# minh86/ModelCrowdNav

Hardware: NVIDIA B200
Metric: env-steps/s (ORCA step + SARL lookahead) (higher is better)
Workload: dtype f16

## Files before the change

modelcrowdnav_b200/csrc/capi.cu:

```cuda
#include "cn_common.cuh"

#include <math.h>
#include <stdarg.h>
#include <stdlib.h>
#include <string.h>

#include <vector>

std::atomic<int64_t> g_cn_launches{0};
static thread_local char g_err[512] = "";

void cn_set_error(const char *fmt, ...)
{
    va_list ap;
    va_start(ap, fmt);
    vsnprintf(g_err, sizeof(g_err), fmt, ap);
    va_end(ap);
}

int cn_launch_transpose_out(int E, int H, int C, const double *src, double *dst, cudaStream_t s);
int cn_launch_set_actions(cn_env *env, const double *aos_dev, cudaStream_t s);
int cn_launch_set_human_v(cn_env *env, const double *aos_dev, cudaStream_t s);
int cn_launch_pack_keep(cn_env *env, cudaStream_t s);

struct TraceRec { const char *name; cudaStream_t stream; cudaEvent_t ev; };
static std::vector<TraceRec> g_trace;
static bool g_trace_on = false;

void cn_trace_mark(const char *name, cudaStream_t s)
{
    if (!g_trace_on || g_trace.size() >= 4096) return;
    cudaEvent_t ev;
    if (cudaEventCreate(&ev) != cudaSuccess) return;
    cudaEventRecord(ev, s);
    g_trace.push_back({name, s, ev});
}

static SarlDims dims_of(const cn_sarl_cfg *c, int om_dim)
{
    SarlDims d;
    memset(&d, 0, sizeof(d));
    d.in = c->input_dim; d.self_dim = c->self_state_dim;
    for (int i = 0; i < 2; ++i) { d.m1[i] = c->mlp1_dims[i]; d.m2[i] = c->mlp2_dims[i]; }
    for (int i = 0; i < 3; ++i) d.at[i] = c->attn_dims[i];
    for (int i = 0; i < 4; ++i) d.m3[i] = c->mlp3_dims[i];
    d.net = c->network; d.lstm_h = c->network == CN_NET_LSTM_RL ? c->lstm_hidden : 0;
    for (int i = 0; i < 4; ++i) d.lm1[i] = c->network == CN_NET_LSTM_RL ? c->lstm_mlp1_dims[i] : 0;
    d.lstm_in = d.lm1[0] > 0 ? d.lm1[3] : d.in;
    d.om_dim = om_dim; d.cell_num = c->cell_num; d.om_ch = c->om_channel_size; d.cell_size = c->cell_size;
    d.no_gs = c->network == CN_NET_SARL && c->without_global_state ? 1 : 0;
    return d;
}

std::vector<LayerSpec> cn_layers(const SarlDims &d, SarlWeightsDev &w)
{
    std::vector<LayerSpec> L;
    int in = d.in;
    auto chain = [&](int n, const int *outs, LinearDev *dst) {
        for (int i = 0; i < n; ++i) { L.push_back({in, outs[i], &dst[i], nullptr}); in = outs[i]; }
    };
    if (d.net == CN_NET_CADRL) {
        chain(4, d.m3, w.m3);
    } else if (d.net == CN_NET_LSTM_RL) {
        if (d.lm1[0] > 0) chain(4, d.lm1, w.lm1);
        in = d.self_dim + d.lstm_h;
        chain(4, d.m3, w.m3);
        L.push_back({d.lstm_in, 4 * d.lstm_h, &w.lih, &w.lhh});
    } else {
        chain(2, d.m1, w.m1);
        chain(2, d.m2, w.m2);
        in = d.no_gs ? d.m1[1] : 2 * d.m1[1];
        chain(3, d.at, w.at);
        in = d.m2[1] + d.self_dim;
        chain(4, d.m3, w.m3);
    }
    return L;
}

extern "C" {

int cn_debug_trace(int on)
{
    for (auto &r : g_trace) cudaEventDestroy(r.ev);
    g_trace.clear();
    g_trace_on = on != 0;
    return CN_OK;
}

int cn_debug_trace_dump(char *buf, int64_t cap)
{
    if (!buf || cap < 1) { cn_set_error("null buffer"); return CN_EINVAL; }
    CN_CUDA_CHECK(cudaDeviceSynchronize());
    int64_t off = 0;
    buf[0] = 0;
    for (size_t i = 0; i < g_trace.size(); ++i) {
        float ms = 0.0f;
        cudaEventElapsedTime(&ms, g_trace[0].ev, g_trace[i].ev);
        const int n = snprintf(buf + off, (size_t)(cap - off), "%.4f %p %s\n", ms, (void *)g_trace[i].stream, g_trace[i].name);
        if (n < 0 || off + n >= cap) break;
        off += n;
    }
    return CN_OK;
}

const char *cn_last_error(void) { return g_err; }
int cn_version(void) { return 100; }
int64_t cn_launch_count(void) { return g_cn_launches.load(); }

int cn_device_count(void)
{
    int n = 0;
    if (cudaGetDeviceCount(&n) != cudaSuccess) { cudaGetLastError(); return 0; }
    return n;
}

void cn_env_cfg_default(cn_env_cfg *c)
{
    memset(c, 0, sizeof(*c));
    c->num_envs = 1; c->human_num = 5;
    c->time_limit = 25; c->time_step = 0.25;
    c->success_reward = 1; c->collision_penalty = -0.25; c->discomfort_dist = 0.2; c->discomfort_penalty_factor = 0.5;
    c->neighbor_dist = 10; c->max_neighbors = 10; c->time_horizon = 5; c->human_safety_space = 0;
    c->robot_visible = 0;
    c->sim_rule = CN_CIRCLE_CROSSING; c->circle_radius = 4; c->square_width = 10;
    c->human_radius = 0.3; c->human_v_pref = 1; c->robot_radius = 0.3; c->robot_v_pref = 1;
    c->seed = 0; c->env_id_offset = 0; c->auto_reset = 0; c->gamma = 0.9;
    c->randomize_attributes = 0;
    c->robot_kinematics = CN_KIN_HOLONOMIC;
}

void cn_sarl_cfg_default(cn_sarl_cfg *c)
{
    memset(c, 0, sizeof(*c));
    c->input_dim = 13; c->self_state_dim = 6;
    c->mlp1_dims[0] = 150; c->mlp1_dims[1] = 100;
    c->mlp2_dims[0] = 100; c->mlp2_dims[1] = 50;
    c->attn_dims[0] = 100; c->attn_dims[1] = 100; c->attn_dims[2] = 1;
    c->mlp3_dims[0] = 150; c->mlp3_dims[1] = 100; c->mlp3_dims[2] = 100; c->mlp3_dims[3] = 1;
    c->speed_samples = 5; c->rotation_samples = 16;
    c->gamma = 0.9; c->v_pref = 1.0; c->precision = CN_PREC_F32;
    c->kinematics = CN_KIN_HOLONOMIC;
    c->network = CN_NET_SARL; c->lstm_hidden = 50;
    c->with_om = 0; c->cell_num = 4; c->cell_size = 1.0; c->om_channel_size = 3;
}

static int use_device(int device)
{
    int n = 0;
    cudaError_t e = cudaGetDeviceCount(&n);
    if (e != cudaSuccess || n == 0) {
        cudaGetLastError();
        cn_set_error("no CUDA device available (%s); libcrowdnav_b200 has no CPU fallback",
                     e != cudaSuccess ? cudaGetErrorString(e) : "device count 0");
        return CN_ECUDA;
    }
    if (device < 0 || device >= n) { cn_set_error("device %d out of range (0..%d)", device, n - 1); return CN_EINVAL; }
    CN_CUDA_CHECK(cudaSetDevice(device));
    cudaDeviceProp prop;
    CN_CUDA_CHECK(cudaGetDeviceProperties(&prop, device));
    if (prop.major != 10) {
        cn_set_error("device %d is sm_%d%d; this library is built for sm_100a only", device, prop.major, prop.minor);
        return CN_ECUDA;
    }
    return CN_OK;
}


int cn_env_create(const cn_env_cfg *cfg, int device, cn_env **out)
{
    if (!cfg || !out) { cn_set_error("null argument"); return CN_EINVAL; }
    if (cfg->num_envs < 1 || cfg->human_num < 1 || cfg->human_num > CN_MAX_HUMANS) {
        cn_set_error("num_envs >= 1 and 1 <= human_num <= %d required", CN_MAX_HUMANS);
        return CN_EINVAL;
    }
    if (cfg->max_neighbors < 0 || cfg->max_neighbors > CN_MAX_NEIGHBORS) {
        cn_set_error("max_neighbors must be in [0, %d]", CN_MAX_NEIGHBORS);
        return CN_EINVAL;
    }
    if (!(cfg->time_step > 0)) { cn_set_error("time_step must be positive"); return CN_EINVAL; }
    int rc = use_device(device);
    if (rc) return rc;

    cn_env *env = new cn_env();
    memset(env, 0, sizeof(*env));
    env->device = device;
    EnvParams &p = env->p;
    p.d.E = cfg->num_envs; p.d.H = cfg->human_num; p.d.A1 = cfg->human_num + 1;
    p.time_limit = cfg->time_limit; p.time_step = cfg->time_step;
    p.success_reward = cfg->success_reward; p.collision_penalty = cfg->collision_penalty;
    p.discomfort_dist = cfg->discomfort_dist; p.discomfort_penalty_factor = cfg->discomfort_penalty_factor;
    p.neighbor_dist = (float)cfg->neighbor_dist; p.time_horizon = (float)cfg->time_horizon;
    p.time_step_f = (float)cfg->time_step; p.max_neighbors = cfg->max_neighbors;
    p.human_safety_space = cfg->human_safety_space; p.robot_visible = cfg->robot_visible;
    p.sim_rule = cfg->sim_rule; p.circle_radius = cfg->circle_radius; p.square_width = cfg->square_width;
    p.human_radius = cfg->human_radius; p.human_v_pref = cfg->human_v_pref;
    p.robot_radius = cfg->robot_radius; p.robot_v_pref = cfg->robot_v_pref;
    p.seed = cfg->seed; p.env_id_offset = cfg->env_id_offset; p.auto_reset = cfg->auto_reset;
    p.gamma = cfg->gamma;
    p.randomize_attributes = cfg->randomize_attributes;
    p.kinematics = cfg->robot_kinematics;

    const size_t E = p.d.E, H = p.d.H, A1 = p.d.A1;
#define CN_ALLOC(ptr, bytes)                                                     \
    do {                                                                         \
        cudaError_t _e = cudaMalloc((void **)&(ptr), (bytes));                   \
        if (_e != cudaSuccess) {                                                 \
            cn_set_error("cudaMalloc(%zu) failed: %s", (size_t)(bytes), cudaGetErrorString(_e)); \
            cn_env_destroy(env);                                                 \
            return CN_ENOMEM;                                                    \
        }                                                                        \
        cudaMemset((ptr), 0, (bytes));                                           \
    } while (0)
    CN_ALLOC(env->state, sizeof(double) * F_COUNT * A1 * E);
    CN_ALLOC(env->time, sizeof(double) * E);
    CN_ALLOC(env->human_v, sizeof(double) * 2 * H * E);
    CN_ALLOC(env->action_xy, sizeof(double) * 2 * E);
    CN_ALLOC(env->action_idx, sizeof(int32_t) * E);
    CN_ALLOC(env->reward, sizeof(double) * E);
    CN_ALLOC(env->done, E);
    CN_ALLOC(env->info, E);
    CN_ALLOC(env->dmin, sizeof(double) * E);
    CN_ALLOC(env->next_obs, sizeof(double) * 5 * H * E);
    CN_ALLOC(env->frozen, E);
    CN_ALLOC(env->stage, sizeof(double) * F_COUNT * A1 * E);
    CN_ALLOC(env->step_ctr, sizeof(uint32_t) * E);
    CN_ALLOC(env->theta, sizeof(double) * E);
    const size_t acc_bytes = E * (6 * 8 + 6 * 8 + 4 + 4);
    CN_ALLOC(env->accum_block, acc_bytes);
#undef CN_ALLOC
    char *b = (char *)env->accum_block;
    EnvAccum &a = env->acc;
    a.episodes = (int64_t *)b; b += 8 * E;
    a.success = (int64_t *)b; b += 8 * E;
    a.collision = (int64_t *)b; b += 8 * E;
    a.timeout = (int64_t *)b; b += 8 * E;
    a.steps = (int64_t *)b; b += 8 * E;
    a.too_close = (int64_t *)b; b += 8 * E;
    a.sum_min_dist = (double *)b; b += 8 * E;
    a.sum_success_time = (double *)b; b += 8 * E;
    a.sum_collision_time = (double *)b; b += 8 * E;
    a.sum_timeout_time = (double *)b; b += 8 * E;
    a.sum_return = (double *)b; b += 8 * E;
    a.ep_return = (double *)b; b += 8 * E;
    a.ep_steps = (int32_t *)b; b += 4 * E;
    a.episode_ctr = (uint32_t *)b; b += 4 * E;
    *out = env;
    return CN_OK;
}

int cn_env_destroy(cn_env *env)
{
    if (!env) return CN_OK;
    cudaSetDevice(env->device);
    void *ptrs[] = {env->state, env->time, env->human_v, env->action_xy, env->action_idx, env->reward, env->done,
                    env->info, env->dmin, env->next_obs, env->frozen, env->stage, env->step_ctr, env->accum_block, env->theta};
    for (void *q : ptrs) if (q) cudaFree(q);
    if (env->io_block) cudaFree(env->io_block);
    if (env->side_stream) cudaStreamDestroy(env->side_stream);
    if (env->ev_fork) cudaEventDestroy(env->ev_fork);
    if (env->ev_join) cudaEventDestroy(env->ev_join);
    if (env->tail_stream) cudaStreamDestroy(env->tail_stream);
    if (env->ev_rows) cudaEventDestroy(env->ev_rows);
    if (env->ev_tail) cudaEventDestroy(env->ev_tail);
    if (env->active_dev) cudaFree(env->active_dev);
    if (env->active_host) cudaFreeHost(env->active_host);
    for (cudaEvent_t ev : env->ev_active) if (ev) cudaEventDestroy(ev);
    delete env;
    return CN_OK;
}

#define CN_ENV_ENTER(env)                                              \
    if (!(env)) { cn_set_error("null env handle"); return CN_EINVAL; } \
    CN_CUDA_CHECK(cudaSetDevice((env)->device));                       \
    cudaStream_t s = (cudaStream_t)stream

int cn_env_set_theta(cn_env *env, const double *theta_host, void *stream)
{
    CN_ENV_ENTER(env);
    if (!theta_host) { cn_set_error("theta_host is null"); return CN_EINVAL; }
    CN_CUDA_CHECK(cudaMemcpyAsync(env->theta, theta_host, sizeof(double) * env->p.d.E, cudaMemcpyHostToDevice, s));
    CN_CUDA_CHECK(cudaStreamSynchronize(s));
    return CN_OK;
}

int cn_env_get_theta(cn_env *env, double *theta_host, void *stream)
{
    CN_ENV_ENTER(env);
    if (!theta_host) { cn_set_error("theta_host is null"); return CN_EINVAL; }
    CN_CUDA_CHECK(cudaMemcpyAsync(theta_host, env->theta, sizeof(double) * env->p.d.E, cudaMemcpyDeviceToHost, s));
    CN_CUDA_CHECK(cudaStreamSynchronize(s));
    return CN_OK;
}

int cn_env_set_state(cn_env *env, const double *agents_host, const double *times_host, void *stream)
{
    CN_ENV_ENTER(env);
    if (!agents_host) { cn_set_error("agents_host is null"); return CN_EINVAL; }
    const size_t E = env->p.d.E, A1 = env->p.d.A1;
    CN_CUDA_CHECK(cudaMemcpyAsync(env->stage, agents_host, sizeof(double) * E * A1 * F_COUNT, cudaMemcpyHostToDevice, s));
    int rc = cn_launch_pack(env, 1, s);
    if (rc) return rc;
    if (times_host) CN_CUDA_CHECK(cudaMemcpyAsync(env->time, times_host, sizeof(double) * E, cudaMemcpyHostToDevice, s));
    else CN_CUDA_CHECK(cudaMemsetAsync(env->time, 0, sizeof(double) * E, s));
    return CN_OK;
}

int cn_env_get_state(cn_env *env, double *agents_host, double *times_host, void *stream)
{
    CN_ENV_ENTER(env);
    const size_t E = env->p.d.E, A1 = env->p.d.A1;
    if (agents_host) {
        int rc = cn_launch_pack(env, 0, s);
        if (rc) return rc;
        CN_CUDA_CHECK(cudaMemcpyAsync(agents_host, env->stage, sizeof(double) * E * A1 * F_COUNT, cudaMemcpyDeviceToHost, s));
    }
    if (times_host) CN_CUDA_CHECK(cudaMemcpyAsync(times_host, env->time, sizeof(double) * E, cudaMemcpyDeviceToHost, s));
    CN_CUDA_CHECK(cudaStreamSynchronize(s));
    return CN_OK;
}

int cn_env_reset(cn_env *env, void *stream)
{
    CN_ENV_ENTER(env);
    return cn_launch_reset(env, 0, s);
}

int cn_env_orca(cn_env *env, void *stream)
{
    CN_ENV_ENTER(env);
    return cn_launch_orca(env, s);
}

int cn_env_robot_orca(cn_env *env, double safety_space, void *stream)
{
    CN_ENV_ENTER(env);
    return cn_launch_robot_orca(env, safety_space, s);
}

int cn_env_step(cn_env *env, const double *action_xy_dev, int update, void *stream)
{
    CN_ENV_ENTER(env);
    if (!env->orca_valid) {
        cn_set_error("cn_env_step: call cn_env_orca for the current state first");
        return CN_EINVAL;
    }
    int rc = cn_launch_step(env, action_xy_dev, update, s);
    if (rc) return rc;
    if (update && env->p.auto_reset) rc = cn_launch_reset(env, 1, s);
    return rc;
}

int cn_env_get_views(cn_env *env, cn_env_views *out)
{
    if (!env || !out) { cn_set_error("null argument"); return CN_EINVAL; }
    out->reward = env->reward; out->done = env->done; out->info = env->info; out->dmin = env->dmin;
    out->human_v = env->human_v; out->next_obs = env->next_obs; out->state = env->state; out->time = env->time;
    out->action_idx = env->action_idx; out->action_xy = env->action_xy;
    return CN_OK;
}

int cn_env_read_outputs(cn_env *env, double *reward, uint8_t *done, uint8_t *info, double *dmin, void *stream)
{
    CN_ENV_ENTER(env);
    const size_t E = env->p.d.E;
    if (reward) CN_CUDA_CHECK(cudaMemcpyAsync(reward, env->reward, sizeof(double) * E, cudaMemcpyDeviceToHost, s));
    if (done) CN_CUDA_CHECK(cudaMemcpyAsync(done, env->done, E, cudaMemcpyDeviceToHost, s));
    if (info) CN_CUDA_CHECK(cudaMemcpyAsync(info, env->info, E, cudaMemcpyDeviceToHost, s));
    if (dmin) CN_CUDA_CHECK(cudaMemcpyAsync(dmin, env->dmin, sizeof(double) * E, cudaMemcpyDeviceToHost, s));
    CN_CUDA_CHECK(cudaStreamSynchronize(s));
    return CN_OK;
}

int cn_env_read_human_actions(cn_env *env, double *human_vxy_host, void *stream)
{
    CN_ENV_ENTER(env);
    if (!env->orca_valid) { cn_set_error("no cached ORCA result; call cn_env_orca"); return CN_EINVAL; }
    const size_t E = env->p.d.E, H = env->p.d.H;
    int rc = cn_launch_transpose_out((int)E, (int)H, 2, env->human_v, env->stage, s);
    if (rc) return rc;
    CN_CUDA_CHECK(cudaMemcpyAsync(human_vxy_host, env->stage, sizeof(double) * E * H * 2, cudaMemcpyDeviceToHost, s));
    CN_CUDA_CHECK(cudaStreamSynchronize(s));
    return CN_OK;
}

int cn_env_read_next_obs(cn_env *env, double *obs_host, void *stream)
{
    CN_ENV_ENTER(env);
    const size_t E = env->p.d.E, H = env->p.d.H;
    int rc = cn_launch_transpose_out((int)E, (int)H, 5, env->next_obs, env->stage, s);
    if (rc) return rc;
    CN_CUDA_CHECK(cudaMemcpyAsync(obs_host, env->stage, sizeof(double) * E * H * 5, cudaMemcpyDeviceToHost, s));
    CN_CUDA_CHECK(cudaStreamSynchronize(s));
    return CN_OK;
}

int cn_env_read_actions(cn_env *env, double *action_xy_host, int32_t *action_idx_host, void *stream)
{
    CN_ENV_ENTER(env);
    const size_t E = env->p.d.E;
    if (action_xy_host) {
        int rc = cn_launch_transpose_out((int)E, 1, 2, env->action_xy, env->stage, s);
        if (rc) return rc;
        CN_CUDA_CHECK(cudaMemcpyAsync(action_xy_host, env->stage, sizeof(double) * 2 * E, cudaMemcpyDeviceToHost, s));
    }
    if (action_idx_host)
        CN_CUDA_CHECK(cudaMemcpyAsync(action_idx_host, env->action_idx, sizeof(int32_t) * E, cudaMemcpyDeviceToHost, s));
    CN_CUDA_CHECK(cudaStreamSynchronize(s));
    return CN_OK;
}

int cn_env_set_actions(cn_env *env, const double *action_xy_host, void *stream)
{
    CN_ENV_ENTER(env);
    if (!action_xy_host) { cn_set_error("action_xy_host is null"); return CN_EINVAL; }
    const size_t E = env->p.d.E;
    CN_CUDA_CHECK(cudaMemcpyAsync(env->stage, action_xy_host, sizeof(double) * 2 * E, cudaMemcpyHostToDevice, s));
    return cn_launch_set_actions(env, env->stage, s);
}

int cn_env_set_human_actions(cn_env *env, const double *human_vxy_host, void *stream)
{
    CN_ENV_ENTER(env);
    if (!human_vxy_host) { cn_set_error("human_vxy_host is null"); return CN_EINVAL; }
    const size_t n = (size_t)env->p.d.E * env->p.d.H * 2;
    CN_CUDA_CHECK(cudaMemcpyAsync(env->stage, human_vxy_host, sizeof(double) * n, cudaMemcpyHostToDevice, s));
    return cn_launch_set_human_v(env, env->stage, s);
}

int cn_env_read_stats(cn_env *env, cn_stats *out, int reset, void *stream)
{
    CN_ENV_ENTER(env);
    if (!out) { cn_set_error("null stats"); return CN_EINVAL; }
    const size_t E = env->p.d.E;
    const size_t bytes = E * 8 * 11;
    std::vector<char> host(bytes);
    CN_CUDA_CHECK(cudaMemcpyAsync(host.data(), env->accum_block, bytes, cudaMemcpyDeviceToHost, s));
    CN_CUDA_CHECK(cudaStreamSynchronize(s));
    const int64_t *iv = (const int64_t *)host.data();
    const double *dv = (const double *)(host.data() + 6 * 8 * E);
    int64_t isum[6] = {0, 0, 0, 0, 0, 0};
    double dsum[5] = {0, 0, 0, 0, 0};
    for (int k = 0; k < 6; ++k) for (size_t e = 0; e < E; ++e) isum[k] += iv[k * E + e];
    for (int k = 0; k < 5; ++k) for (size_t e = 0; e < E; ++e) dsum[k] += dv[k * E + e];
    out->episodes = isum[0]; out->success = isum[1]; out->collision = isum[2]; out->timeout = isum[3];
    out->steps = isum[4]; out->too_close = isum[5];
    out->sum_min_dist = dsum[0]; out->sum_success_time = dsum[1]; out->sum_collision_time = dsum[2];
    out->sum_timeout_time = dsum[3]; out->sum_return = dsum[4];
    if (reset) CN_CUDA_CHECK(cudaMemsetAsync(env->accum_block, 0, bytes, s));
    return CN_OK;
}

int cn_env_copy_outputs(cn_env *env, double *reward_dev, uint8_t *done_dev, uint8_t *info_dev, void *stream)
{
    CN_ENV_ENTER(env);
    const size_t E = env->p.d.E;
    if (reward_dev) CN_CUDA_CHECK(cudaMemcpyAsync(reward_dev, env->reward, sizeof(double) * E, cudaMemcpyDeviceToDevice, s));
    if (done_dev) CN_CUDA_CHECK(cudaMemcpyAsync(done_dev, env->done, E, cudaMemcpyDeviceToDevice, s));
    if (info_dev) CN_CUDA_CHECK(cudaMemcpyAsync(info_dev, env->info, E, cudaMemcpyDeviceToDevice, s));
    return CN_OK;
}

int64_t cn_env_episode_table_bytes(const cn_env *env) { return env ? (int64_t)env->p.d.E * 8 * 11 : 0; }

int cn_env_read_episode_table(cn_env *env, void *table_host, uint8_t *frozen_host, void *stream)
{
    CN_ENV_ENTER(env);
    const size_t E = env->p.d.E;
    if (table_host) CN_CUDA_CHECK(cudaMemcpyAsync(table_host, env->accum_block, E * 8 * 11, cudaMemcpyDeviceToHost, s));
    if (frozen_host) CN_CUDA_CHECK(cudaMemcpyAsync(frozen_host, env->frozen, E, cudaMemcpyDeviceToHost, s));
    CN_CUDA_CHECK(cudaStreamSynchronize(s));
    return CN_OK;
}


static int pad4i(int x) { return (x + 3) & ~3; }

int64_t cn_policy_param_count(const cn_sarl_cfg *c)
{
    if (!c) return 0;
    SarlWeightsDev w;
    int64_t n = 0;
    for (const LayerSpec &l : cn_layers(dims_of(c, 0), w)) n += (int64_t)cn_layer_floats(l);
    return n;
}

static int build_action_table(const cn_sarl_cfg *c, double *out)
{
    const double E_ = 2.718281828459045;
    int n = 0;
    out[0] = 0; out[1] = 0; n = 1;
    if (c->kinematics != CN_KIN_HOLONOMIC) {
        const double PI = 3.141592653589793, start = -PI / 4, stop = PI / 4;
        const int div = c->rotation_samples - 1;
        const double step = div > 0 ? (stop - start) / div : 0.0;
        for (int r = 0; r < c->rotation_samples; ++r) {
            double rotation = start + r * step;
            if (div > 0 && r == c->rotation_samples - 1) rotation = stop;
            for (int s = 0; s < c->speed_samples; ++s) {
                out[2 * n] = (exp((double)(s + 1) / c->speed_samples) - 1) / (E_ - 1) * c->v_pref;
                out[2 * n + 1] = rotation;
                ++n;
            }
        }
        return n;
    }
    const double step = (2 * 3.141592653589793 - 0) / c->rotation_samples;
    for (int r = 0; r < c->rotation_samples; ++r) {
        const double rotation = r * step;
        for (int s = 0; s < c->speed_samples; ++s) {
            const double speed = (exp((double)(s + 1) / c->speed_samples) - 1) / (E_ - 1) * c->v_pref;
            out[2 * n] = speed * cos(rotation);
            out[2 * n + 1] = speed * sin(rotation);
            ++n;
        }
    }
    return n;
}

int cn_policy_create(const cn_sarl_cfg *cfg, int device, cn_policy **out)
{
    if (!cfg || !out) { cn_set_error("null argument"); return CN_EINVAL; }
    const int A = cfg->speed_samples * cfg->rotation_samples + 1;
    int om_dim = 0;
    if (cfg->with_om) {
        if (cfg->cell_num < 1 || cfg->cell_num > 8 || cfg->om_channel_size < 1 || cfg->om_channel_size > 3 || !(cfg->cell_size > 0)) {
            cn_set_error("with_om needs 1 <= cell_num <= 8, om_channel_size in {1, 2, 3} and cell_size > 0");
            return CN_EINVAL;
        }
        if (cfg->network == CN_NET_CADRL) { cn_set_error("CADRL has no occupancy maps (cadrl.py:60-62)"); return CN_EINVAL; }
        if (cfg->precision != CN_PREC_F32 && cfg->network != CN_NET_SARL) {
            cn_set_error("occupancy maps on the tensor-core path are built for SARL only; use CN_PREC_F32"); return CN_EUNSUPPORTED;
        }
        om_dim = cfg->cell_num * cfg->cell_num * cfg->om_channel_size;
    }
    if (cfg->input_dim != 13 + om_dim || cfg->self_state_dim < 1 || cfg->self_state_dim > 13) {
        cn_set_error("input_dim must be 13 + cell_num^2 * om_channel_size (13 without maps) and 1 <= self_state_dim <= 13");
        return CN_EUNSUPPORTED;
    }
    if (cfg->attn_dims[2] != 1 || cfg->mlp3_dims[3] != 1) { cn_set_error("attention and mlp3 must end in 1 unit"); return CN_EINVAL; }
    if (cfg->network != CN_NET_SARL && cfg->network != CN_NET_CADRL && cfg->network != CN_NET_LSTM_RL) {
        cn_set_error("unknown value network %d", cfg->network); return CN_EINVAL;
    }
    if (cfg->without_global_state && cfg->network != CN_NET_SARL) {
        cn_set_error("without_global_state is a [sarl] option; CADRL and LSTM-RL have no global state"); return CN_EINVAL;
    }
    if (cfg->network == CN_NET_LSTM_RL) {
        if (cfg->lstm_hidden < 1 || cfg->lstm_hidden > 64) { cn_set_error("1 <= lstm_hidden <= 64 required"); return CN_EINVAL; }
        if (cfg->lstm_mlp1_dims[0] > 0)
            for (int i = 0; i < 4; ++i)
                if (cfg->lstm_mlp1_dims[i] < 1 || cfg->lstm_mlp1_dims[i] > 256) { cn_set_error("layer widths must be in [1, 256]"); return CN_EINVAL; }
    }
    if (A < 1 || A > CN_MAX_ACTIONS) { cn_set_error("1 <= speed_samples*rotation_samples+1 <= %d required", CN_MAX_ACTIONS); return CN_EINVAL; }
    const int dims[] = {cfg->mlp1_dims[0], cfg->mlp1_dims[1], cfg->mlp2_dims[0], cfg->mlp2_dims[1], cfg->attn_dims[0],
                        cfg->attn_dims[1], cfg->mlp3_dims[0], cfg->mlp3_dims[1], cfg->mlp3_dims[2]};
    for (int v : dims) if (v < 1 || v > 256) { cn_set_error("layer widths must be in [1, 256]"); return CN_EINVAL; }
    if (cfg->precision != CN_PREC_F32 && cfg->precision != CN_PREC_F16_TC) { cn_set_error("unknown precision"); return CN_EINVAL; }
    int rc = use_device(device);
    if (rc) return rc;
    if ((rc = cn_f32_configure_device())) return rc;

    cn_policy *p = new cn_policy();
    memset(p, 0, sizeof(*p));
    p->device = device; p->cfg = *cfg;
    p->d = dims_of(cfg, om_dim);
    SarlDims &d = p->d;
    d.A = build_action_table(cfg, p->action_host);
    p->n_params = cn_policy_param_count(cfg);

    size_t tsize = 0;
    for (const LayerSpec &l : cn_layers(d, p->w))
        tsize += (size_t)(l.in + 1) * pad4i(l.out) + (l.dst_hh ? (size_t)(l.out / 4 + 1) * pad4i(l.out) : 0);
    cudaError_t e1 = cudaMalloc((void **)&p->action_dev, sizeof(double) * 2 * d.A);
    cudaError_t e2 = cudaMalloc((void **)&p->w_raw, sizeof(float) * p->n_params);
    cudaError_t e3 = cudaMalloc((void **)&p->w_t, sizeof(float) * tsize);
    cudaError_t e4 = cudaMalloc((void **)&p->bad_flag, 2 * sizeof(int32_t));
    if (e1 != cudaSuccess || e2 != cudaSuccess || e3 != cudaSuccess || e4 != cudaSuccess) {
        cn_set_error("cudaMalloc failed in cn_policy_create");
        cn_policy_destroy(p);
        return CN_ENOMEM;
    }
    cudaMemset(p->bad_flag, 0, 2 * sizeof(int32_t));
    CN_CUDA_CHECK(cudaMemcpy(p->action_dev, p->action_host, sizeof(double) * 2 * d.A, cudaMemcpyHostToDevice));
    if (cfg->precision == CN_PREC_F16_TC) {
        rc = cn_tc_init(p);
        if (rc) { cn_policy_destroy(p); return rc; }
    }
    *out = p;
    return CN_OK;
}

int cn_policy_destroy(cn_policy *p)
{
    if (!p) return CN_OK;
    cudaSetDevice(p->device);
    if (p->tc) cn_tc_destroy(p);
    void *ptrs[] = {p->action_dev, p->w_raw, p->w_t, p->bad_flag, p->values};
    for (void *q : ptrs) if (q) cudaFree(q);
    delete p;
    return CN_OK;
}

int cn_policy_load_weights(cn_policy *p, const float *flat, int64_t n, void *stream)
{
    if (!p || !flat) { cn_set_error("null argument"); return CN_EINVAL; }
    if (n != p->n_params) { cn_set_error("expected %lld parameters, got %lld", (long long)p->n_params, (long long)n); return CN_EINVAL; }
    CN_CUDA_CHECK(cudaSetDevice(p->device));
    cudaStream_t s = (cudaStream_t)stream;
    std::vector<float> t;
    auto put = [&](int in, int out, const float *w, const float *b, LinearDev *dst) {
        const int ld = pad4i(out);
        const size_t off = t.size();
        t.resize(off + (size_t)in * ld + ld, 0.0f);
        for (int o = 0; o < out; ++o)
            for (int k = 0; k < in; ++k) t[off + (size_t)k * ld + o] = w[(size_t)o * in + k];
        for (int o = 0; o < out; ++o) t[off + (size_t)in * ld + o] = b[o];
        dst->wt = p->w_t + off; dst->b = p->w_t + off + (size_t)in * ld;
        dst->in = in; dst->out = out; dst->ld = ld;
    };
    const float *src = flat;
    for (const LayerSpec &l : cn_layers(p->d, p->w)) {
        const float *w = src, *b = src + (size_t)l.in * l.out;
        if (l.dst_hh) {
            const int h = l.out / 4;
            const float *w_hh = b;
            b = w_hh + (size_t)l.out * h;
            put(l.in, l.out, w, b, l.dst);
            put(h, l.out, w_hh, b + l.out, l.dst_hh);
        } else {
            put(l.in, l.out, w, b, l.dst);
        }
        src += cn_layer_floats(l);
    }
    CN_CUDA_CHECK(cudaMemcpyAsync(p->w_t, t.data(), sizeof(float) * t.size(), cudaMemcpyHostToDevice, s));
    CN_CUDA_CHECK(cudaMemcpyAsync(p->w_raw, flat, sizeof(float) * n, cudaMemcpyHostToDevice, s));
    CN_CUDA_CHECK(cudaStreamSynchronize(s));
    if (p->cfg.precision == CN_PREC_F16_TC) {
        int rc = cn_tc_load_weights(p, flat, s);
        if (rc) return rc;
    }
    p->weights_loaded = 1;
    return CN_OK;
}

int cn_policy_action_table(cn_policy *p, double *out_xy_host, int32_t *n_actions)
{
    if (!p) { cn_set_error("null policy"); return CN_EINVAL; }
    if (out_xy_host) memcpy(out_xy_host, p->action_host, sizeof(double) * 2 * p->d.A);
    if (n_actions) *n_actions = p->d.A;
    return CN_OK;
}

static int check_pair(cn_policy *p, cn_env *env)
{
    if (!p || !env) { cn_set_error("null handle"); return CN_EINVAL; }
    if (p->device != env->device) { cn_set_error("policy and env live on different devices"); return CN_EINVAL; }
    if (!p->weights_loaded) { cn_set_error("cn_policy_load_weights has not been called"); return CN_EINVAL; }
    if (p->cfg.kinematics != env->p.kinematics) {
        cn_set_error("policy kinematics (%d) and env robot_kinematics (%d) differ", p->cfg.kinematics, env->p.kinematics);
        return CN_EINVAL;
    }
    return CN_OK;
}

static int lookahead(cn_policy *p, cn_env *env, int query_env, double epsilon, cudaStream_t s, cudaStream_t tail = nullptr)
{
    if (p->cfg.precision == CN_PREC_F16_TC) return cn_lookahead_tc(p, env, query_env, epsilon, s, tail);
    return cn_lookahead_f32(p, env, query_env, epsilon, s);
}

static int sync_and_check_values(cn_policy *p, cudaStream_t s)
{
    int32_t bad = 0;
    CN_CUDA_CHECK(cudaMemcpyAsync(&bad, p->bad_flag, sizeof(int32_t), cudaMemcpyDeviceToHost, s));
    CN_CUDA_CHECK(cudaStreamSynchronize(s));
    if (bad) { cn_set_error("Value network is not well trained. "); return CN_EVALUE; }
    return CN_OK;
}

int cn_policy_lookahead(cn_policy *p, cn_env *env, int query_env, double epsilon, void *stream)
{
    int rc = check_pair(p, env);
    if (rc) return rc;
    CN_CUDA_CHECK(cudaSetDevice(p->device));
    cudaStream_t s = (cudaStream_t)stream;
    if (query_env && !env->orca_valid) {
        cn_set_error("query_env lookahead needs cn_env_orca for the current state");
        return CN_EINVAL;
    }
    return lookahead(p, env, query_env, epsilon, s);
}

int cn_policy_read(cn_policy *p, cn_env *env, int32_t *best_idx, double *values, void *stream)
{
    int rc = check_pair(p, env);
    if (rc) return rc;
    CN_CUDA_CHECK(cudaSetDevice(p->device));
    cudaStream_t s = (cudaStream_t)stream;
    const size_t E = env->p.d.E;
    if (best_idx) CN_CUDA_CHECK(cudaMemcpyAsync(best_idx, env->action_idx, sizeof(int32_t) * E, cudaMemcpyDeviceToHost, s));
    if (values) {
        if (!p->values) { cn_set_error("no lookahead has been run"); return CN_EINVAL; }
        CN_CUDA_CHECK(cudaMemcpyAsync(values, p->values, sizeof(double) * E * p->d.A, cudaMemcpyDeviceToHost, s));
    }
    return sync_and_check_values(p, s);
}

int cn_policy_bad_count(cn_policy *p, int64_t *count, int reset, void *stream)
{
    if (!p || !count) { cn_set_error("null argument"); return CN_EINVAL; }
    CN_CUDA_CHECK(cudaSetDevice(p->device));
    cudaStream_t s = (cudaStream_t)stream;
    int32_t n = 0;
    CN_CUDA_CHECK(cudaMemcpyAsync(&n, p->bad_flag + 1, sizeof(int32_t), cudaMemcpyDeviceToHost, s));
    if (reset) CN_CUDA_CHECK(cudaMemsetAsync(p->bad_flag + 1, 0, sizeof(int32_t), s));
    CN_CUDA_CHECK(cudaStreamSynchronize(s));
    *count = n;
    return CN_OK;
}

int cn_policy_transform(cn_policy *p, cn_env *env, float *out_dev, void *stream)
{
    if (!p || !env || !out_dev) { cn_set_error("null argument"); return CN_EINVAL; }
    CN_CUDA_CHECK(cudaSetDevice(p->device));
    return cn_transform_f32(p, env, out_dev, 0, (cudaStream_t)stream);
}

int cn_policy_last_state(cn_policy *p, cn_env *env, float *out_dev, void *stream)
{
    if (!p || !env || !out_dev) { cn_set_error("null argument"); return CN_EINVAL; }
    CN_CUDA_CHECK(cudaSetDevice(p->device));
    return cn_transform_f32(p, env, out_dev, p->cfg.network == CN_NET_LSTM_RL ? 1 : 0, (cudaStream_t)stream);
}

int cn_policy_forward(cn_policy *p, const float *x_dev, int32_t batch, int32_t human_num, float *out_dev, void *stream)
{
    if (!p || !x_dev || !out_dev) { cn_set_error("null argument"); return CN_EINVAL; }
    if (!p->weights_loaded) { cn_set_error("cn_policy_load_weights has not been called"); return CN_EINVAL; }
    CN_CUDA_CHECK(cudaSetDevice(p->device));
    return cn_forward_f32(p, x_dev, batch, human_num, out_dev, (cudaStream_t)stream);
}


static int rollout_step_impl(cn_policy *p, cn_env *env, int query_env, double epsilon, cudaStream_t s, cudaStream_t tail,
                             cudaStream_t *cur);

int cn_rollout_step(cn_policy *p, cn_env *env, int query_env, double epsilon, void *stream)
{
    int rc = check_pair(p, env);
    if (rc) return rc;
    CN_CUDA_CHECK(cudaSetDevice(p->device));
    cudaStream_t cur;
    return rollout_step_impl(p, env, query_env, epsilon, (cudaStream_t)stream, nullptr, &cur);
}

static int ensure_tail_stream(cn_env *env)
{
    if (env->tail_stream) return CN_OK;
    int lo = 0, hi = 0;
    CN_CUDA_CHECK(cudaDeviceGetStreamPriorityRange(&lo, &hi));
    CN_CUDA_CHECK(cudaStreamCreateWithPriority(&env->tail_stream, cudaStreamNonBlocking, hi));
    CN_CUDA_CHECK(cudaEventCreateWithFlags(&env->ev_rows, cudaEventDisableTiming));
    CN_CUDA_CHECK(cudaEventCreateWithFlags(&env->ev_tail, cudaEventDisableTiming));
    return CN_OK;
}

int cn_rollout_step_sharded(cn_policy *p, cn_env *env, int query_env, double epsilon, void *stream)
{
    int rc = check_pair(p, env);
    if (rc) return rc;
    CN_CUDA_CHECK(cudaSetDevice(p->device));
    if ((rc = ensure_tail_stream(env))) return rc;
    cudaStream_t s0 = (cudaStream_t)stream, cur = s0;
    if ((rc = rollout_step_impl(p, env, query_env, epsilon, s0, env->tail_stream, &cur))) return rc;
    if (cur != s0) {
        CN_CUDA_CHECK(cudaEventRecord(env->ev_tail, cur));
        CN_CUDA_CHECK(cudaStreamWaitEvent(s0, env->ev_tail, 0));
    }
    return CN_OK;
}

static int rollout_step_impl(cn_policy *p, cn_env *env, int query_env, double epsilon, cudaStream_t s, cudaStream_t tail,
                             cudaStream_t *cur)
{
    int rc = CN_OK;
    if (p->cfg.precision != CN_PREC_F16_TC) tail = nullptr;
    const bool fork = !query_env;
    cn_trace_mark("orca", s);
    if (fork) {
        if (!env->side_stream) {
            CN_CUDA_CHECK(cudaStreamCreateWithFlags(&env->side_stream, cudaStreamNonBlocking));
            CN_CUDA_CHECK(cudaEventCreateWithFlags(&env->ev_fork, cudaEventDisableTiming));
            CN_CUDA_CHECK(cudaEventCreateWithFlags(&env->ev_join, cudaEventDisableTiming));
        }
        CN_CUDA_CHECK(cudaEventRecord(env->ev_fork, s));
        CN_CUDA_CHECK(cudaStreamWaitEvent(env->side_stream, env->ev_fork, 0));
        if ((rc = cn_launch_orca(env, env->side_stream))) return rc;
        CN_CUDA_CHECK(cudaEventRecord(env->ev_join, env->side_stream));
    } else if ((rc = cn_launch_orca(env, s))) return rc;
    if ((rc = lookahead(p, env, query_env, epsilon, s, tail))) return rc;
    if (tail) s = tail;
    *cur = s;
    if (fork) CN_CUDA_CHECK(cudaStreamWaitEvent(s, env->ev_join, 0));
    cn_trace_mark("step", s);
    if ((rc = cn_launch_step(env, nullptr, 1, s, env->p.auto_reset ? 1 : 0))) return rc;
    cn_trace_mark("step_done", s);
    return rc;
}


static __global__ void count_active_kernel(int E, const uint8_t *__restrict__ frozen, int32_t *__restrict__ out)
{
    __shared__ int total;
    if (threadIdx.x == 0) total = 0;
    __syncthreads();
    int n = 0;
    for (int e = threadIdx.x; e < E; e += blockDim.x) n += frozen[e] ? 0 : 1;
    for (int o = 16; o > 0; o >>= 1) n += __shfl_xor_sync(0xffffffffu, n, o);
    if ((threadIdx.x & 31) == 0 && n) atomicAdd(&total, n);
    __syncthreads();
    if (threadIdx.x == 0) *out = total;
}

int cn_rollout_episodes(cn_policy *p, cn_env *env, cn_world *world, int robot_mode, double safety_space, int query_env,
                        double epsilon, int32_t max_steps, int32_t check_every, const cn_rollout_record *rec,
                        int32_t *steps_run, void *stream)
{
    if (!env || !steps_run) { cn_set_error("null argument"); return CN_EINVAL; }
    if (robot_mode < CN_ROBOT_POLICY || robot_mode > CN_ROBOT_KEEP) { cn_set_error("robot_mode %d", robot_mode); return CN_EINVAL; }
    if (max_steps < 0 || check_every < 1) { cn_set_error("max_steps >= 0 and check_every >= 1"); return CN_EINVAL; }
    if (env->p.auto_reset) {
        cn_set_error("cn_rollout_episodes runs ONE episode per env: create the env with auto_reset = 0");
        return CN_EINVAL;
    }
    int rc;
    if (robot_mode == CN_ROBOT_POLICY) {
        if ((rc = check_pair(p, env))) return rc;
    }
    cn_policy *tp = rec ? rec->transform_policy : nullptr;
    if (rec && (!tp || !rec->states_dev || !rec->reward_dev || !rec->done_dev)) {
        cn_set_error("cn_rollout_record needs transform_policy, states_dev, reward_dev and done_dev");
        return CN_EINVAL;
    }
    if (tp && tp->device != env->device) { cn_set_error("transform policy and env live on different devices"); return CN_EINVAL; }
    CN_CUDA_CHECK(cudaSetDevice(env->device));
    cudaStream_t s = (cudaStream_t)stream;
    if (!env->active_dev) {
        CN_CUDA_CHECK(cudaMalloc(&env->active_dev, 2 * sizeof(int32_t)));
        CN_CUDA_CHECK(cudaMallocHost(&env->active_host, 2 * sizeof(int32_t)));
        for (cudaEvent_t &ev : env->ev_active) CN_CUDA_CHECK(cudaEventCreateWithFlags(&ev, cudaEventDisableTiming));
    }
    const size_t E = env->p.d.E;
    const size_t state_floats = tp ? E * (size_t)env->p.d.H * (size_t)tp->cfg.input_dim : 0;
    int slot = 0, pending = -1;
    *steps_run = 0;
    for (int step = 0; step < max_steps; ++step) {
        if (tp) {
            const int sorted = rec->last_state && tp->cfg.network == CN_NET_LSTM_RL;
            if ((rc = cn_transform_f32(tp, env, rec->states_dev + (size_t)step * state_floats, sorted, s))) return rc;
        }
        if (robot_mode == CN_ROBOT_POLICY && !world) {
            cudaStream_t cur;
            if ((rc = rollout_step_impl(p, env, query_env, epsilon, s, nullptr, &cur))) return rc;
        } else {
            if (world) rc = cn_world_predict(world, env, s);
            else rc = cn_launch_orca(env, s);
            if (rc) return rc;
            if (robot_mode == CN_ROBOT_POLICY)
                rc = lookahead(p, env, query_env, epsilon, s);
            else if (robot_mode == CN_ROBOT_ORCA) rc = cn_launch_robot_orca(env, safety_space, s);
            if (rc) return rc;
            if ((rc = cn_launch_step(env, nullptr, 1, s, 0))) return rc;
        }
        if (rec) {
            CN_CUDA_CHECK(cudaMemcpyAsync(rec->reward_dev + (size_t)step * E, env->reward, sizeof(double) * E, cudaMemcpyDeviceToDevice, s));
            CN_CUDA_CHECK(cudaMemcpyAsync(rec->done_dev + (size_t)step * E, env->done, E, cudaMemcpyDeviceToDevice, s));
        }
        *steps_run = step + 1;
        if ((step + 1) % check_every == 0) {
            if (pending >= 0) {
                CN_CUDA_CHECK(cudaEventSynchronize(env->ev_active[pending]));
                if (env->active_host[pending] == 0) break;
            }
            count_active_kernel<<<1, 256, 0, s>>>((int)E, env->frozen, env->active_dev + slot);
            CN_CUDA_CHECK(cudaGetLastError());
            g_cn_launches.fetch_add(1);
            CN_CUDA_CHECK(cudaMemcpyAsync(env->active_host + slot, env->active_dev + slot, sizeof(int32_t), cudaMemcpyDeviceToHost, s));
            CN_CUDA_CHECK(cudaEventRecord(env->ev_active[slot], s));
            pending = slot;
            slot ^= 1;
        }
    }
    return CN_OK;
}

int cn_rollout_step_host(cn_policy *p, cn_env *env, int query_env, double epsilon, const double *agents_in,
                         const double *times_in, double *agents_out, double *times_out, double *reward, uint8_t *done,
                         uint8_t *info, int32_t *action_idx, void *stream)
{
    int rc = check_pair(p, env);
    if (rc) return rc;
    CN_CUDA_CHECK(cudaSetDevice(p->device));
    cudaStream_t s = (cudaStream_t)stream;
    const size_t E = env->p.d.E, A1 = env->p.d.A1;
    if (agents_in) {
        CN_CUDA_CHECK(cudaMemcpyAsync(env->stage, agents_in, sizeof(double) * E * A1 * F_COUNT, cudaMemcpyHostToDevice, s));
        if ((rc = cn_launch_pack_keep(env, s))) return rc;
    }
    if (times_in) CN_CUDA_CHECK(cudaMemcpyAsync(env->time, times_in, sizeof(double) * E, cudaMemcpyHostToDevice, s));
    if ((rc = cn_rollout_step(p, env, query_env, epsilon, s))) return rc;
    if (agents_out) {
        if ((rc = cn_launch_pack(env, 0, s))) return rc;
        CN_CUDA_CHECK(cudaMemcpyAsync(agents_out, env->stage, sizeof(double) * E * A1 * F_COUNT, cudaMemcpyDeviceToHost, s));
    }
    if (times_out) CN_CUDA_CHECK(cudaMemcpyAsync(times_out, env->time, sizeof(double) * E, cudaMemcpyDeviceToHost, s));
    if (reward) CN_CUDA_CHECK(cudaMemcpyAsync(reward, env->reward, sizeof(double) * E, cudaMemcpyDeviceToHost, s));
    if (done) CN_CUDA_CHECK(cudaMemcpyAsync(done, env->done, E, cudaMemcpyDeviceToHost, s));
    if (info) CN_CUDA_CHECK(cudaMemcpyAsync(info, env->info, E, cudaMemcpyDeviceToHost, s));
    if (action_idx) CN_CUDA_CHECK(cudaMemcpyAsync(action_idx, env->action_idx, sizeof(int32_t) * E, cudaMemcpyDeviceToHost, s));
    return sync_and_check_values(p, s);
}

int64_t cn_host_step_bytes(const cn_env *env, int out)
{
    if (!env) return 0;
    const int64_t E = env->p.d.E, A1 = env->p.d.A1;
    const int64_t in = 8 * (E * A1 * F_COUNT + E);
    return out ? in + 8 * E + 4 * E + E + E : in;
}

static int rollout_step_host_packed(cn_policy *p, cn_env *env, int query_env, double epsilon, const void *host_in,
                                    void *host_out, void *stream, bool sync)
{
    int rc = check_pair(p, env);
    if (rc) return rc;
    if (!host_in || !host_out) { cn_set_error("host_in / host_out must not be null"); return CN_EINVAL; }
    CN_CUDA_CHECK(cudaSetDevice(p->device));
    cudaStream_t s = (cudaStream_t)stream;
    if (!env->io_block) CN_CUDA_CHECK(cudaMalloc((void **)&env->io_block, (size_t)cn_host_step_bytes(env, 1) + 16));
    cn_trace_mark("h2d", s);
    CN_CUDA_CHECK(cudaMemcpyAsync(env->io_block, host_in, (size_t)cn_host_step_bytes(env, 0), cudaMemcpyHostToDevice, s));
    cn_trace_mark("unpack", s);
    if ((rc = cn_launch_io(env, env->io_block, 1, s))) return rc;
    cudaStream_t tail = nullptr;
    if (!sync) {
        if ((rc = ensure_tail_stream(env))) return rc;
        tail = env->tail_stream;
    }
    cudaStream_t s0 = s;
    if ((rc = rollout_step_impl(p, env, query_env, epsilon, s, tail, &s))) return rc;
    if ((rc = cn_launch_io(env, env->io_block, 0, s))) return rc;
    cn_trace_mark("d2h", s);
    CN_CUDA_CHECK(cudaMemcpyAsync(host_out, env->io_block, (size_t)cn_host_step_bytes(env, 1), cudaMemcpyDeviceToHost, s));
    cn_trace_mark("d2h_done", s);
    if (s != s0) {
        CN_CUDA_CHECK(cudaEventRecord(env->ev_tail, s));
        CN_CUDA_CHECK(cudaStreamWaitEvent(s0, env->ev_tail, 0));
        s = s0;
    }
    return sync ? sync_and_check_values(p, s) : CN_OK;
}

int cn_rollout_step_host_packed(cn_policy *p, cn_env *env, int query_env, double epsilon, const void *host_in, void *host_out,
                                void *stream)
{
    return rollout_step_host_packed(p, env, query_env, epsilon, host_in, host_out, stream, true);
}

int cn_rollout_step_host_packed_async(cn_policy *p, cn_env *env, int query_env, double epsilon, const void *host_in,
                                      void *host_out, void *stream)
{
    return rollout_step_host_packed(p, env, query_env, epsilon, host_in, host_out, stream, false);
}

int cn_stream_sync(int device, void *stream)
{
    CN_CUDA_CHECK(cudaSetDevice(device));
    CN_CUDA_CHECK(cudaStreamSynchronize((cudaStream_t)stream));
    return CN_OK;
}

}
```

modelcrowdnav_b200/csrc/cn_common.cuh:

```cuda
#pragma once
#include <atomic>
#include <stdlib.h>
#include <utility>
#include <vector>

#include <cuda_runtime.h>
#include <stdint.h>
#include <stdio.h>

#include "../../include/crowdnav_b200.h"

enum { F_PX = 0, F_PY, F_VX, F_VY, F_GX, F_GY, F_R, F_VPREF, F_COUNT };

struct EnvDims {
    int E;
    int H;
    int A1;
};

__host__ __device__ __forceinline__ size_t st_idx(const EnvDims &d, int field, int agent, int env)
{
    return ((size_t)field * d.A1 + agent) * d.E + env;
}

struct EnvParams {
    EnvDims d;
    double time_limit, time_step;
    double success_reward, collision_penalty, discomfort_dist, discomfort_penalty_factor;
    float neighbor_dist, time_horizon, time_step_f;
    int max_neighbors;
    double human_safety_space;
    int robot_visible;
    int sim_rule;
    double circle_radius, square_width, human_radius, human_v_pref, robot_radius, robot_v_pref;
    uint64_t seed;
    int64_t env_id_offset;
    int auto_reset;
    double gamma;
    int randomize_attributes;
    int kinematics;
};

struct EnvAccum {
    int32_t *ep_steps;
    double *ep_return;
    int64_t *episodes, *success, *collision, *timeout, *steps, *too_close;
    double *sum_min_dist, *sum_success_time, *sum_collision_time, *sum_timeout_time, *sum_return;
    uint32_t *episode_ctr;
};

struct cn_env {
    int device;
    EnvParams p;
    double *state;
    double *time;
    double *human_v;
    double *action_xy;
    int32_t *action_idx;
    double *reward;
    uint8_t *done;
    uint8_t *info;
    double *dmin;
    double *next_obs;
    uint8_t *frozen;
    EnvAccum acc;
    void *accum_block;
    double *stage;
    uint32_t *step_ctr;
    double *theta;
    int orca_valid;
    cudaStream_t side_stream;
    cudaEvent_t ev_fork, ev_join;
    cudaStream_t tail_stream;
    cudaEvent_t ev_rows, ev_tail;
    double *io_block;
    int32_t *active_dev, *active_host;
    cudaEvent_t ev_active[2];
};

struct SarlDims {
    int in, self_dim;
    int m1[2], m2[2], at[3], m3[4];
    int A;
    int net;
    int lstm_h;
    int lm1[4];
    int lstm_in;
    int om_dim;
    int cell_num, om_ch;
    double cell_size;
    int no_gs;
};

template <typename Get>
__device__ __forceinline__ int occupancy_map_pair(const SarlDims &d, int i, int j, Get get, double &vxr, double &vyr)
{
    const int cn = d.cell_num;
    const double pxi = get(i, 0), pyi = get(i, 1);
    const double angle = atan2(get(i, 3), get(i, 2));
    const double opx = get(j, 0) - pxi, opy = get(j, 1) - pyi;
    const double rotation = atan2(opy, opx) - angle;
    const double distance = sqrt(opx * opx + opy * opy);
    const double xi = floor(cos(rotation) * distance / d.cell_size + cn / 2.0);
    const double yi = floor(sin(rotation) * distance / d.cell_size + cn / 2.0);
    if (xi < 0 || xi >= cn || yi < 0 || yi >= cn) return -1;
    const double vx = get(j, 2), vy = get(j, 3);
    const double vrot = atan2(vy, vx) - angle, speed = sqrt(vx * vx + vy * vy);
    vxr = cos(vrot) * speed; vyr = sin(vrot) * speed;
    return (int)(cn * yi + xi);
}

__device__ __forceinline__ void occupancy_map_store(int ch, int c, double cnt, double sx, double sy, float *__restrict__ out)
{
    const bool on = cnt > 0.0;
    if (ch == 1) out[c] = on ? 1.0f : 0.0f;
    else if (ch == 2) { out[2 * c] = on ? (float)(sx / cnt) : 0.0f; out[2 * c + 1] = on ? (float)(sy / cnt) : 0.0f; }
    else { out[3 * c] = on ? 1.0f : 0.0f; out[3 * c + 1] = on ? (float)(sx / cnt) : 0.0f; out[3 * c + 2] = on ? (float)(sy / cnt) : 0.0f; }
}

template <typename Get>
__device__ void occupancy_map_row(const SarlDims &d, int H, int i, Get get, float *__restrict__ out)
{
    int cell[CN_MAX_HUMANS];
    double vxr[CN_MAX_HUMANS], vyr[CN_MAX_HUMANS];
    for (int j = 0; j < H; ++j) {
        cell[j] = -1; vxr[j] = 0.0; vyr[j] = 0.0;
        if (j != i) cell[j] = occupancy_map_pair(d, i, j, get, vxr[j], vyr[j]);
    }
    const int cells = d.cell_num * d.cell_num;
    for (int c = 0; c < cells; ++c) {
        double cnt = 0.0, sx = 0.0, sy = 0.0;
        for (int j = 0; j < H; ++j)
            if (cell[j] == c) { cnt += 1.0; sx += vxr[j]; sy += vyr[j]; }
        occupancy_map_store(d.om_ch, c, cnt, sx, sy, out);
    }
}

struct LinearDev {
    const float *wt;
    const float *b;
    int in, out, ld;
};

struct SarlWeightsDev {
    LinearDev m1[2], m2[2], at[3], m3[4];
    LinearDev lm1[4], lih, lhh;
};

struct LayerSpec {
    int in, out;
    LinearDev *dst, *dst_hh;
};
std::vector<LayerSpec> cn_layers(const SarlDims &d, SarlWeightsDev &w);
inline size_t cn_layer_floats(const LayerSpec &l)
{
    return (size_t)l.in * l.out + l.out + (l.dst_hh ? (size_t)(l.out / 4) * l.out + l.out : 0);
}

struct cn_policy {
    int device;
    cn_sarl_cfg cfg;
    SarlDims d;
    double action_host[CN_MAX_ACTIONS * 2];
    double *action_dev;
    float *w_raw;
    float *w_t;
    SarlWeightsDev w;
    int64_t n_params;
    int weights_loaded;
    double *values;
    int32_t *bad_flag;
    size_t values_cap;
    void *tc;
};

void cn_set_error(const char *fmt, ...);
extern std::atomic<int64_t> g_cn_launches;

#define CN_CUDA_CHECK(call)                                                                     \
    do {                                                                                        \
        cudaError_t _e = (call);                                                                \
        if (_e != cudaSuccess) {                                                                \
            cn_set_error("%s failed at %s:%d: %s", #call, __FILE__, __LINE__, cudaGetErrorString(_e)); \
            return CN_ECUDA;                                                                    \
        }                                                                                       \
    } while (0)

static inline int cn_small_block() { return 32; }

void cn_trace_mark(const char *name, cudaStream_t s);

#define CN_LAUNCH_CHECK()                                                                       \
    do {                                                                                        \
        ++g_cn_launches;                                                                        \
        cudaError_t _e = cudaGetLastError();                                                    \
        if (_e != cudaSuccess) {                                                                \
            cn_set_error("kernel launch failed at %s:%d: %s", __FILE__, __LINE__, cudaGetErrorString(_e)); \
            return CN_ECUDA;                                                                    \
        }                                                                                       \
    } while (0)

template <typename... KArgs, typename... Args>
int cn_launch(void (*kern)(KArgs...), dim3 grid, dim3 block, size_t smem, cudaStream_t s, bool pdl, Args &&...args)
{
    cudaLaunchConfig_t lc = {};
    lc.gridDim = grid; lc.blockDim = block; lc.dynamicSmemBytes = smem; lc.stream = s;
    cudaLaunchAttribute at[1];
    at[0].id = cudaLaunchAttributeProgrammaticStreamSerialization;
    at[0].val.programmaticStreamSerializationAllowed = 1;
    lc.attrs = at; lc.numAttrs = pdl ? 1 : 0;
    CN_CUDA_CHECK(cudaLaunchKernelEx(&lc, kern, std::forward<Args>(args)...));
    CN_LAUNCH_CHECK();
    return CN_OK;
}

template <typename T>
int cn_grow(T *&buf, size_t &cap, size_t n, size_t item_bytes, bool zero = false, cudaStream_t s = 0)
{
    if (n <= cap) return CN_OK;
    if (buf) cudaFree(buf);
    buf = nullptr; cap = 0;
    CN_CUDA_CHECK(cudaMalloc((void **)&buf, n * item_bytes));
    if (zero) CN_CUDA_CHECK(cudaMemsetAsync(buf, 0, n * item_bytes, s));
    cap = n;
    return CN_OK;
}

struct Philox {
    uint32_t key[2];
    uint32_t ctr[4];
    __host__ __device__ static inline void mulhilo(uint32_t a, uint32_t b, uint32_t &hi, uint32_t &lo)
    {
        const uint64_t p = (uint64_t)a * b;
        hi = (uint32_t)(p >> 32);
        lo = (uint32_t)p;
    }
    __host__ __device__ inline void block(uint32_t out[4]) const
    {
        uint32_t c0 = ctr[0], c1 = ctr[1], c2 = ctr[2], c3 = ctr[3];
        uint32_t k0 = key[0], k1 = key[1];
#ifdef __CUDA_ARCH__
#pragma unroll
#endif
        for (int r = 0; r < 10; ++r) {
            uint32_t hi0, lo0, hi1, lo1;
            mulhilo(0xD2511F53u, c0, hi0, lo0);
            mulhilo(0xCD9E8D57u, c2, hi1, lo1);
            const uint32_t n0 = hi1 ^ c1 ^ k0, n1 = lo1, n2 = hi0 ^ c3 ^ k1, n3 = lo0;
            c0 = n0; c1 = n1; c2 = n2; c3 = n3;
            k0 += 0x9E3779B9u; k1 += 0xBB67AE85u;
        }
        out[0] = c0; out[1] = c1; out[2] = c2; out[3] = c3;
    }
};

struct PhiloxStream {
    Philox ph;
    uint32_t buf[4];
    int have;
    uint32_t draw;
    __host__ __device__ inline void init(uint64_t seed, uint64_t env_gid, uint32_t subseq, uint32_t domain)
    {
        ph.key[0] = (uint32_t)seed; ph.key[1] = (uint32_t)(seed >> 32);
        ph.ctr[1] = subseq; ph.ctr[2] = (uint32_t)env_gid;
        ph.ctr[3] = (uint32_t)(env_gid >> 32) ^ (domain << 24);
        have = 0; draw = 0;
    }
    __host__ __device__ inline double next()
    {
        if (have < 2) { ph.ctr[0] = draw++; ph.block(buf); have = 4; }
        const uint32_t a = buf[4 - have] >> 5, b = buf[5 - have] >> 6;
        have -= 2;
        return ((double)a * 67108864.0 + (double)b) / 9007199254740992.0;
    }
};

__device__ __forceinline__ void cn_effective_velocity(int kinematics, double theta, double a0, double a1, double &ax, double &ay)
{
    if (kinematics == CN_KIN_HOLONOMIC) { ax = a0; ay = a1; }
    else { ax = a0 * cos(a1 + theta); ay = a0 * sin(a1 + theta); }
}

__host__ __device__ __forceinline__ double norm2d(double a, double b) { return sqrt(fma(b, b, a * a)); }

int cn_launch_orca(cn_env *env, cudaStream_t s);
int cn_launch_robot_orca(cn_env *env, double safety_space, cudaStream_t s);
int cn_launch_step(cn_env *env, const double *action_xy_dev, int update, cudaStream_t s, int fuse_reset = 0);
int cn_launch_reset(cn_env *env, int only_done, cudaStream_t s);
int cn_launch_pack(cn_env *env, int to_soa, cudaStream_t s);
int cn_launch_io(cn_env *env, double *blk, int unpack, cudaStream_t s);

int cn_lookahead_f32(cn_policy *p, cn_env *env, int query_env, double epsilon, cudaStream_t s);
int cn_transform_f32(cn_policy *p, cn_env *env, float *out_dev, int sort_humans, cudaStream_t s);
int cn_forward_f32(cn_policy *p, const float *x_dev, int batch, int H, float *out_dev, cudaStream_t s);
int cn_f32_configure_device(void);

int cn_tc_init(cn_policy *p);
void cn_tc_destroy(cn_policy *p);
int cn_tc_load_weights(cn_policy *p, const float *flat_host, cudaStream_t s);
int cn_lookahead_tc(cn_policy *p, cn_env *env, int query_env, double epsilon, cudaStream_t s, cudaStream_t tail = nullptr);
```

modelcrowdnav_b200/csrc/env_math.cuh:

```cuda
#pragma once
#include "cn_common.cuh"

__device__ __forceinline__ double cn_point_to_segment_dist0(double x1, double y1, double x2, double y2)
{
    const double px = x2 - x1, py = y2 - y1;
    if (px == 0 && py == 0) return norm2d(0.0 - x1, 0.0 - y1);
    double u = ((0.0 - x1) * px + (0.0 - y1) * py) / (px * px + py * py);
    if (u > 1) u = 1;
    else if (u < 0) u = 0;
    const double x = x1 + u * px, y = y1 + u * py;
    return norm2d(x - 0.0, y - 0.0);
}

struct StepOutcome {
    double reward, dmin;
    int done, info;
};

template <typename Acc>
__device__ __forceinline__ StepOutcome cn_step_outcome(const EnvParams &p, Acc ag, int H, double t, double ax, double ay)
{
    const double rpx = ag(F_PX, 0), rpy = ag(F_PY, 0), rr = ag(F_R, 0);
    const double dt = p.time_step;
    double dmin = INFINITY;
    bool collision = false;
    for (int h = 1; h <= H; ++h) {
        const double px = ag(F_PX, h) - rpx;
        const double py = ag(F_PY, h) - rpy;
        const double vx = ag(F_VX, h) - ax;
        const double vy = ag(F_VY, h) - ay;
        const double ex = px + vx * dt;
        const double ey = py + vy * dt;
        const double closest = cn_point_to_segment_dist0(px, py, ex, ey) - ag(F_R, h) - rr;
        if (!collision) {
            if (closest < 0) collision = true;
            else if (closest < dmin) dmin = closest;
        }
    }
    const double endx = rpx + ax * dt, endy = rpy + ay * dt;
    const bool reaching_goal = norm2d(endx - ag(F_GX, 0), endy - ag(F_GY, 0)) < rr;
    StepOutcome o;
    o.dmin = dmin;
    if (t >= p.time_limit - 1) { o.reward = 0; o.done = 1; o.info = CN_TIMEOUT; }
    else if (collision) { o.reward = p.collision_penalty; o.done = 1; o.info = CN_COLLISION; }
    else if (reaching_goal) { o.reward = p.success_reward; o.done = 1; o.info = CN_REACHGOAL; }
    else if (dmin < p.discomfort_dist) {
        o.reward = (dmin - p.discomfort_dist) * p.discomfort_penalty_factor * dt;
        o.done = 0; o.info = CN_DANGER;
    } else { o.reward = 0; o.done = 0; o.info = CN_NOTHING; }
    return o;
}

__device__ __forceinline__ void cn_rotate(const float *s, float *o, int kinematics = CN_KIN_HOLONOMIC)
{
    const float dx = s[5] - s[0], dy = s[6] - s[1];
    const float rot = atan2f(dy, dx);
    float sn, c;
    sincosf(rot, &sn, &c);
    o[0] = sqrtf(dx * dx + dy * dy);
    o[1] = s[7];
    o[2] = kinematics == CN_KIN_UNICYCLE ? s[8] - rot : 0.0f;
    o[3] = s[4];
    o[4] = s[2] * c + s[3] * sn;
    o[5] = s[3] * c - s[2] * sn;
    o[6] = (s[9] - s[0]) * c + (s[10] - s[1]) * sn;
    o[7] = (s[10] - s[1]) * c - (s[9] - s[0]) * sn;
    o[8] = s[11] * c + s[12] * sn;
    o[9] = s[12] * c - s[11] * sn;
    o[10] = s[13];
    const float ax = s[0] - s[9], ay = s[1] - s[10];
    o[11] = sqrtf(ax * ax + ay * ay);
    o[12] = s[4] + s[13];
}
```

modelcrowdnav_b200/csrc/lookahead_f32.cu:

```cuda
#include "env_math.cuh"

#include <math.h>

namespace {

constexpr int kThreads = 256;
constexpr int kRowsCap = 64;
constexpr size_t kMaxDynSmem = 232448;

__host__ __device__ inline int pad4(int x) { return (x + 3) & ~3; }

struct F32Plan {
    int H, A, CA;
    int wX, wT0, wM1, wF, wJ;
    int oX, oT0, oM1, oF, oG, oJ, oS, oW, oV, oEnv, oOrd, oOm, total_floats;
};

__device__ void layer(const LinearDev L, int k_off, int K, const float *__restrict__ in, int ldin, int in_div,
                      float *__restrict__ out, int ldout, int rows, bool accum, bool add_bias, bool relu)
{
    const int N = L.out;
    const int ntc = (N + 3) >> 2, ntr = (rows + 3) >> 2;
    for (int tile = threadIdx.x; tile < ntr * ntc; tile += blockDim.x) {
        const int tr = tile / ntc, tc = tile - tr * ntc;
        const int r0 = tr * 4, n0 = tc * 4;
        const float *ip[4];
#pragma unroll
        for (int i = 0; i < 4; ++i) {
            int r = r0 + i;
            if (r >= rows) r = rows - 1;
            ip[i] = in + (size_t)(r / in_div) * ldin;
        }
        float acc[4][4];
#pragma unroll
        for (int i = 0; i < 4; ++i)
#pragma unroll
            for (int j = 0; j < 4; ++j) acc[i][j] = 0.0f;
        const float *wp = L.wt + (size_t)k_off * L.ld + n0;
#pragma unroll 4
        for (int k = 0; k < K; ++k) {
            const float4 w = __ldg(reinterpret_cast<const float4 *>(wp + (size_t)k * L.ld));
#pragma unroll
            for (int i = 0; i < 4; ++i) {
                const float a = ip[i][k];
                acc[i][0] = fmaf(a, w.x, acc[i][0]);
                acc[i][1] = fmaf(a, w.y, acc[i][1]);
                acc[i][2] = fmaf(a, w.z, acc[i][2]);
                acc[i][3] = fmaf(a, w.w, acc[i][3]);
            }
        }
#pragma unroll
        for (int i = 0; i < 4; ++i) {
            const int r = r0 + i;
            if (r >= rows) break;
#pragma unroll
            for (int j = 0; j < 4; ++j) {
                const int n = n0 + j;
                if (n >= N) break;
                float v = acc[i][j];
                if (accum) v += out[(size_t)r * ldout + n];
                if (add_bias) v += __ldg(L.b + n);
                if (relu) v = fmaxf(v, 0.0f);
                out[(size_t)r * ldout + n] = v;
            }
        }
    }
}

__device__ void head(const LinearDev L, const float *__restrict__ in, int ldin, float *__restrict__ out, int rows)
{
    for (int r = threadIdx.x; r < rows; r += blockDim.x) {
        float acc = 0.0f;
        const float *x = in + (size_t)r * ldin;
        for (int k = 0; k < L.in; ++k) acc = fmaf(x[k], __ldg(L.wt + (size_t)k * L.ld), acc);
        out[r] = acc + __ldg(L.b);
    }
}

__device__ void sarl_forward_smem(const SarlWeightsDev &W, const SarlDims &d, const F32Plan &pl, float *sm, int ng)
{
    const int H = pl.H, rows = ng * H;
    float *X = sm + pl.oX, *T0 = sm + pl.oT0, *M1 = sm + pl.oM1, *F = sm + pl.oF, *G = sm + pl.oG;
    float *J = sm + pl.oJ, *S = sm + pl.oS, *Wt = sm + pl.oW, *Vv = sm + pl.oV;
    const int G1 = d.m1[1], FD = d.m2[1];

    layer(W.m1[0], 0, d.in, X, pl.wX, 1, T0, pl.wT0, rows, false, true, true);
    __syncthreads();
    layer(W.m1[1], 0, d.m1[0], T0, pl.wT0, 1, M1, pl.wM1, rows, false, true, true);
    __syncthreads();
    if (!d.no_gs)
        for (int i = threadIdx.x; i < ng * G1; i += blockDim.x) {
            const int g = i / G1, k = i - g * G1;
            float s = 0.0f;
            for (int h = 0; h < H; ++h) s += M1[(size_t)(g * H + h) * pl.wM1 + k];
            G[(size_t)g * pl.wM1 + k] = s / (float)H;
        }
    for (int i = threadIdx.x; i < ng * d.self_dim; i += blockDim.x) {
        const int g = i / d.self_dim, k = i - g * d.self_dim;
        J[(size_t)g * pl.wJ + k] = X[(size_t)(g * H) * pl.wX + k];
    }
    layer(W.m2[0], 0, G1, M1, pl.wM1, 1, T0, pl.wT0, rows, false, true, true);
    __syncthreads();
    layer(W.m2[1], 0, d.m2[0], T0, pl.wT0, 1, F, pl.wF, rows, false, true, false);
    __syncthreads();
    if (d.no_gs) {
        layer(W.at[0], 0, G1, M1, pl.wM1, 1, T0, pl.wT0, rows, false, true, true);
    } else {
        layer(W.at[0], 0, G1, M1, pl.wM1, 1, T0, pl.wT0, rows, false, false, false);
        __syncthreads();
        layer(W.at[0], G1, G1, G, pl.wM1, H, T0, pl.wT0, rows, true, true, true);
    }
    __syncthreads();
    layer(W.at[1], 0, d.at[0], T0, pl.wT0, 1, M1, pl.wM1, rows, false, true, true);
    __syncthreads();
    head(W.at[2], M1, pl.wM1, S, rows);
    __syncthreads();
    for (int g = threadIdx.x; g < ng; g += blockDim.x) {
        float ssum = 0.0f;
        for (int h = 0; h < H; ++h) {
            const float sc = S[g * H + h];
            const float se = expf(sc) * (sc != 0.0f ? 1.0f : 0.0f);
            Wt[g * H + h] = se;
            ssum += se;
        }
        for (int h = 0; h < H; ++h) Wt[g * H + h] = Wt[g * H + h] / ssum;
    }
    __syncthreads();
    for (int i = threadIdx.x; i < ng * FD; i += blockDim.x) {
        const int g = i / FD, k = i - g * FD;
        float s = 0.0f;
        for (int h = 0; h < H; ++h) s += Wt[g * H + h] * F[(size_t)(g * H + h) * pl.wF + k];
        J[(size_t)g * pl.wJ + d.self_dim + k] = s;
    }
    __syncthreads();
    float *U0 = T0, *U1 = M1;
    layer(W.m3[0], 0, d.self_dim + FD, J, pl.wJ, 1, U0, pl.wT0, ng, false, true, true);
    __syncthreads();
    layer(W.m3[1], 0, d.m3[0], U0, pl.wT0, 1, U1, pl.wM1, ng, false, true, true);
    __syncthreads();
    layer(W.m3[2], 0, d.m3[1], U1, pl.wM1, 1, U0, pl.wT0, ng, false, true, true);
    __syncthreads();
    head(W.m3[3], U0, pl.wT0, Vv, ng);
    __syncthreads();
}

__device__ void cadrl_forward_smem(const SarlWeightsDev &W, const SarlDims &d, const F32Plan &pl, float *sm, int ng)
{
    const int H = pl.H, rows = ng * H;
    float *X = sm + pl.oX, *T0 = sm + pl.oT0, *M1 = sm + pl.oM1, *S = sm + pl.oS, *Vv = sm + pl.oV;
    layer(W.m3[0], 0, d.in, X, pl.wX, 1, T0, pl.wT0, rows, false, true, true);
    __syncthreads();
    layer(W.m3[1], 0, d.m3[0], T0, pl.wT0, 1, M1, pl.wM1, rows, false, true, true);
    __syncthreads();
    layer(W.m3[2], 0, d.m3[1], M1, pl.wM1, 1, T0, pl.wT0, rows, false, true, true);
    __syncthreads();
    head(W.m3[3], T0, pl.wT0, S, rows);
    __syncthreads();
    for (int g = threadIdx.x; g < ng; g += blockDim.x) {
        float m = S[g * H];
        for (int h = 1; h < H; ++h) m = fminf(m, S[g * H + h]);
        Vv[g] = m;
    }
    __syncthreads();
}

__device__ void lstm_forward_smem(const SarlWeightsDev &W, const SarlDims &d, const F32Plan &pl, float *sm, int ng)
{
    const int H = pl.H, rows = ng * H, Hh = d.lstm_h;
    float *X = sm + pl.oX, *T0 = sm + pl.oT0, *M1 = sm + pl.oM1, *Cc = sm + pl.oF, *Hs = sm + pl.oG;
    float *J = sm + pl.oJ, *Vv = sm + pl.oV;
    const float *in = X;
    int ldin = pl.wX;
    if (d.lm1[0] > 0) {
        layer(W.lm1[0], 0, d.in, X, pl.wX, 1, T0, pl.wT0, rows, false, true, true);
        __syncthreads();
        layer(W.lm1[1], 0, d.lm1[0], T0, pl.wT0, 1, M1, pl.wM1, rows, false, true, true);
        __syncthreads();
        layer(W.lm1[2], 0, d.lm1[1], M1, pl.wM1, 1, T0, pl.wT0, rows, false, true, true);
        __syncthreads();
        layer(W.lm1[3], 0, d.lm1[2], T0, pl.wT0, 1, M1, pl.wM1, rows, false, true, false);
        __syncthreads();
        in = M1; ldin = pl.wM1;
    }
    for (int i = threadIdx.x; i < ng * Hh; i += blockDim.x) {
        const int g = i / Hh, k = i - g * Hh;
        Hs[(size_t)g * pl.wM1 + k] = 0.0f;
        Cc[(size_t)g * pl.wF + k] = 0.0f;
    }
    for (int i = threadIdx.x; i < ng * d.self_dim; i += blockDim.x) {
        const int g = i / d.self_dim, k = i - g * d.self_dim;
        J[(size_t)g * pl.wJ + k] = X[(size_t)(g * H) * pl.wX + k];
    }
    __syncthreads();
    for (int t = 0; t < H; ++t) {
        layer(W.lih, 0, d.lstm_in, in + (size_t)t * ldin, H * ldin, 1, T0, pl.wT0, ng, false, true, false);
        __syncthreads();
        layer(W.lhh, 0, Hh, Hs, pl.wM1, 1, T0, pl.wT0, ng, true, true, false);
        __syncthreads();
        for (int i = threadIdx.x; i < ng * Hh; i += blockDim.x) {
            const int g = i / Hh, k = i - g * Hh;
            const float *gt = T0 + (size_t)g * pl.wT0;
            const float ig = 1.0f / (1.0f + expf(-gt[k])), fg = 1.0f / (1.0f + expf(-gt[Hh + k]));
            const float gg = tanhf(gt[2 * Hh + k]), og = 1.0f / (1.0f + expf(-gt[3 * Hh + k]));
            const float c = fg * Cc[(size_t)g * pl.wF + k] + ig * gg;
            Cc[(size_t)g * pl.wF + k] = c;
            Hs[(size_t)g * pl.wM1 + k] = og * tanhf(c);
        }
        __syncthreads();
    }
    for (int i = threadIdx.x; i < ng * Hh; i += blockDim.x) {
        const int g = i / Hh, k = i - g * Hh;
        J[(size_t)g * pl.wJ + d.self_dim + k] = Hs[(size_t)g * pl.wM1 + k];
    }
    __syncthreads();
    float *U0 = T0, *U1 = M1;
    layer(W.m3[0], 0, d.self_dim + Hh, J, pl.wJ, 1, U0, pl.wT0, ng, false, true, true);
    __syncthreads();
    layer(W.m3[1], 0, d.m3[0], U0, pl.wT0, 1, U1, pl.wM1, ng, false, true, true);
    __syncthreads();
    layer(W.m3[2], 0, d.m3[1], U1, pl.wM1, 1, U0, pl.wT0, ng, false, true, true);
    __syncthreads();
    head(W.m3[3], U0, pl.wT0, Vv, ng);
    __syncthreads();
}

__device__ __forceinline__ void net_forward_smem(const SarlWeightsDev &W, const SarlDims &d, const F32Plan &pl, float *sm, int ng)
{
    if (d.net == CN_NET_CADRL) cadrl_forward_smem(W, d, pl, sm, ng);
    else if (d.net == CN_NET_LSTM_RL) lstm_forward_smem(W, d, pl, sm, ng);
    else sarl_forward_smem(W, d, pl, sm, ng);
}

__global__ void __launch_bounds__(kThreads, 2)
lookahead_values_kernel(EnvParams p, SarlWeightsDev W, SarlDims d, F32Plan pl, const double *__restrict__ st,
                        const double *__restrict__ time, const double *__restrict__ human_v,
                        const uint8_t *__restrict__ frozen, const double *__restrict__ actions, int query_env,
                        double gamma, double gamma_bar_host, double v_pref_host, double *__restrict__ values,
                        const double *__restrict__ theta)
{
    extern __shared__ __align__(16) float sm[];
    const int e = blockIdx.x;
    if (frozen[e]) return;
    const EnvDims ed = p.d;
    const int H = pl.H;
    const int a0 = blockIdx.y * pl.CA;
    const int na = min(pl.CA, pl.A - a0);
    const int rows = na * H;
    double *env = reinterpret_cast<double *>(sm + pl.oEnv);
    double *hnext = env + (size_t)ed.A1 * F_COUNT;
    double *rew = hnext + (size_t)H * 4;
    float *X = sm + pl.oX;

    for (int i = threadIdx.x; i < ed.A1 * F_COUNT; i += blockDim.x) {
        const int a = i / F_COUNT, f = i - a * F_COUNT;
        env[i] = st[st_idx(ed, f, a, e)];
    }
    __syncthreads();
    auto ag = [&](int f, int a) { return env[a * F_COUNT + f]; };
    int *ord = reinterpret_cast<int *>(sm + pl.oOrd);
    if (threadIdx.x == 0) {
        for (int h = 0; h < H; ++h) ord[h] = h;
        if (d.net == CN_NET_LSTM_RL && !query_env) {
            for (int i = 1; i < H; ++i) {
                const int oi = ord[i];
                const double di = norm2d(ag(F_PX, oi + 1) - ag(F_PX, 0), ag(F_PY, oi + 1) - ag(F_PY, 0));
                int j = i - 1;
                while (j >= 0 && norm2d(ag(F_PX, ord[j] + 1) - ag(F_PX, 0), ag(F_PY, ord[j] + 1) - ag(F_PY, 0)) < di) {
                    ord[j + 1] = ord[j];
                    --j;
                }
                ord[j + 1] = oi;
            }
        }
    }
    const double dt = p.time_step;
    const int kin = p.kinematics;
    const double th = kin != CN_KIN_HOLONOMIC ? theta[e] : 0.0;
    for (int h = threadIdx.x; h < H; h += blockDim.x) {
        double hvx, hvy;
        if (query_env) { hvx = human_v[(size_t)(0 * H + h) * ed.E + e]; hvy = human_v[(size_t)(1 * H + h) * ed.E + e]; }
        else { hvx = ag(F_VX, h + 1); hvy = ag(F_VY, h + 1); }
        hnext[h * 4 + 0] = ag(F_PX, h + 1) + hvx * dt;
        hnext[h * 4 + 1] = ag(F_PY, h + 1) + hvy * dt;
        hnext[h * 4 + 2] = hvx;
        hnext[h * 4 + 3] = hvy;
    }
    __syncthreads();
    for (int i = threadIdx.x; i < na; i += blockDim.x) {
        double ax, ay;
        cn_effective_velocity(kin, th, actions[2 * (a0 + i)], actions[2 * (a0 + i) + 1], ax, ay);
        double reward;
        if (query_env) {
            reward = cn_step_outcome(p, ag, H, time[e], ax, ay).reward;
        } else {
            const double npx = ag(F_PX, 0) + ax * dt, npy = ag(F_PY, 0) + ay * dt, rr = ag(F_R, 0);
            double dmin = INFINITY;
            bool collision = false;
            for (int h = 0; h < H; ++h) {
                const double dist = norm2d(npx - hnext[h * 4 + 0], npy - hnext[h * 4 + 1]) - rr - ag(F_R, h + 1);
                if (dist < 0) { collision = true; break; }
                if (dist < dmin) dmin = dist;
            }
            const bool reaching_goal = norm2d(npx - ag(F_GX, 0), npy - ag(F_GY, 0)) < rr;
            if (collision) reward = -0.25;
            else if (reaching_goal) reward = 1;
            else if (dmin < 0.2) reward = (dmin - 0.2) * 0.5 * dt;
            else reward = 0;
        }
        rew[i] = reward;
    }
    float *OM = sm + pl.oOm;
    if (d.om_dim > 0) {
        for (int i = threadIdx.x; i < H; i += blockDim.x)
            occupancy_map_row(d, H, i, [&](int j, int f) { return hnext[ord[j] * 4 + f]; }, OM + (size_t)i * d.om_dim);
        __syncthreads();
    }
    for (int r = threadIdx.x; r < rows; r += blockDim.x) {
        const int i = r / H, h = ord[r - i * H];
        double ax, ay;
        cn_effective_velocity(kin, th, actions[2 * (a0 + i)], actions[2 * (a0 + i) + 1], ax, ay);
        float s[14], o[13];
        s[0] = (float)(ag(F_PX, 0) + ax * dt); s[1] = (float)(ag(F_PY, 0) + ay * dt);
        s[2] = (float)ax; s[3] = (float)ay; s[4] = (float)ag(F_R, 0);
        s[5] = (float)ag(F_GX, 0); s[6] = (float)ag(F_GY, 0); s[7] = (float)ag(F_VPREF, 0);
        s[8] = kin != CN_KIN_HOLONOMIC ? (float)(th + actions[2 * (a0 + i) + 1]) : 0.0f;
        s[9] = (float)hnext[h * 4 + 0]; s[10] = (float)hnext[h * 4 + 1];
        s[11] = (float)hnext[h * 4 + 2]; s[12] = (float)hnext[h * 4 + 3]; s[13] = (float)ag(F_R, h + 1);
        cn_rotate(s, o, kin);
#pragma unroll
        for (int k = 0; k < 13; ++k) X[(size_t)r * pl.wX + k] = o[k];
        for (int k = 0; k < d.om_dim; ++k) X[(size_t)r * pl.wX + 13 + k] = OM[(size_t)(r - i * H) * d.om_dim + k];
    }
    __syncthreads();
    net_forward_smem(W, d, pl, sm, na);
    const float *Vv = sm + pl.oV;
    const double vp = ag(F_VPREF, 0);
    const double gamma_bar = (vp == v_pref_host) ? gamma_bar_host : pow(gamma, dt * vp);
    for (int i = threadIdx.x; i < na; i += blockDim.x)
        values[(size_t)e * pl.A + a0 + i] = rew[i] + gamma_bar * (double)Vv[i];
}

__global__ void __launch_bounds__(128)
argmax_kernel(EnvParams p, int A, const double *__restrict__ st, const uint8_t *__restrict__ frozen,
              const double *__restrict__ values, const double *__restrict__ actions, double epsilon,
              uint32_t *__restrict__ step_ctr, double *__restrict__ action_xy,
              int32_t *__restrict__ action_idx, int32_t *__restrict__ bad_flag)
{
    const int e = (blockIdx.x * blockDim.x + threadIdx.x) >> 5, lane = threadIdx.x & 31;
    const EnvDims d = p.d;
    asm volatile("griddepcontrol.wait;" ::: "memory");
    if (e >= d.E || frozen[e]) return;
    double max_value = -INFINITY;
    int best = -1;
    for (int a = lane; a < A; a += 32) {
        const double v = values[(size_t)e * A + a];
        if (v > max_value) { max_value = v; best = a; }
    }
#pragma unroll
    for (int off = 16; off > 0; off >>= 1) {
        const double ov = __shfl_xor_sync(0xffffffffu, max_value, off);
        const int ob = __shfl_xor_sync(0xffffffffu, best, off);
        if (ob >= 0 && (best < 0 || ov > max_value || (ov == max_value && ob < best))) { max_value = ov; best = ob; }
    }
    if (lane != 0) return;
    const bool reached = norm2d(st[st_idx(d, F_PY, 0, e)] - st[st_idx(d, F_GY, 0, e)],
                                st[st_idx(d, F_PX, 0, e)] - st[st_idx(d, F_GX, 0, e)]) < st[st_idx(d, F_R, 0, e)];
    if (reached) best = 0;
    else {
        bool random_pick = false;
        if (epsilon > 0.0) {
            PhiloxStream rng;
            rng.init(p.seed, (uint64_t)(p.env_id_offset + e), step_ctr[e], 1u);
            step_ctr[e] += 1;
            if (rng.next() < epsilon) { best = min(A - 1, (int)(rng.next() * A)); random_pick = true; }
        }
        if (!random_pick && best < 0) { atomicExch(bad_flag, 1); atomicAdd(bad_flag + 1, 1); best = 0; }
    }
    action_idx[e] = best;
    action_xy[e] = actions[2 * best];
    action_xy[d.E + e] = actions[2 * best + 1];
}

__global__ void transform_kernel(EnvParams p, SarlDims nd, const double *__restrict__ st, const double *__restrict__ theta,
                                 float *__restrict__ out, int sort_humans)
{
    const int tid = blockIdx.x * blockDim.x + threadIdx.x;
    const EnvDims d = p.d;
    if (tid >= d.E * d.H) return;
    const int h = tid / d.E, e = tid - h * d.E;
    auto ag = [&](int f, int a) { return (float)st[st_idx(d, f, a, e)]; };
    float s[14], o[13];
    s[0] = ag(F_PX, 0); s[1] = ag(F_PY, 0); s[2] = ag(F_VX, 0); s[3] = ag(F_VY, 0); s[4] = ag(F_R, 0);
    s[5] = ag(F_GX, 0); s[6] = ag(F_GY, 0); s[7] = ag(F_VPREF, 0);
    s[8] = p.kinematics != CN_KIN_HOLONOMIC ? (float)theta[e] : 0.0f;
    s[9] = ag(F_PX, h + 1); s[10] = ag(F_PY, h + 1); s[11] = ag(F_VX, h + 1); s[12] = ag(F_VY, h + 1);
    s[13] = ag(F_R, h + 1);
    cn_rotate(s, o, p.kinematics);
    int pos = h;
    if (sort_humans) {
        const double rx = st[st_idx(d, F_PX, 0, e)], ry = st[st_idx(d, F_PY, 0, e)];
        const double dh = norm2d(st[st_idx(d, F_PX, h + 1, e)] - rx, st[st_idx(d, F_PY, h + 1, e)] - ry);
        pos = 0;
        for (int k = 0; k < d.H; ++k) {
            if (k == h) continue;
            const double dk = norm2d(st[st_idx(d, F_PX, k + 1, e)] - rx, st[st_idx(d, F_PY, k + 1, e)] - ry);
            pos += (dk > dh || (dk == dh && k < h)) ? 1 : 0;
        }
    }
    const int D = 13 + nd.om_dim;
    float *row = out + ((size_t)e * d.H + pos) * D;
    for (int k = 0; k < 13; ++k) row[k] = o[k];
    if (nd.om_dim > 0)
        occupancy_map_row(nd, d.H, h, [&](int j, int f) { return st[st_idx(d, f == 0 ? F_PX : f == 1 ? F_PY : f == 2 ? F_VX : F_VY, j + 1, e)]; },
                          row + 13);
}

__global__ void __launch_bounds__(kThreads, 2)
forward_kernel(SarlWeightsDev W, SarlDims d, F32Plan pl, const float *__restrict__ x, int B, float *__restrict__ out)
{
    extern __shared__ __align__(16) float sm[];
    const int b0 = blockIdx.x * pl.CA;
    const int nb = min(pl.CA, B - b0);
    const int H = pl.H;
    float *X = sm + pl.oX;
    const int D = d.in;
    for (int i = threadIdx.x; i < nb * H * D; i += blockDim.x) {
        const int r = i / D, k = i - r * D;
        X[(size_t)r * pl.wX + k] = x[(size_t)b0 * H * D + i];
    }
    __syncthreads();
    net_forward_smem(W, d, pl, sm, nb);
    const float *Vv = sm + pl.oV;
    for (int i = threadIdx.x; i < nb; i += blockDim.x) out[b0 + i] = Vv[i];
}

F32Plan make_plan(const SarlDims &d, int H, int A, int A1)
{
    F32Plan pl;
    pl.H = H; pl.A = A;
    pl.CA = kRowsCap / H;
    if (pl.CA < 1) pl.CA = 1;
    if (pl.CA > A) pl.CA = A;
    const int rows = pl.CA * H;
    auto mx = [](int a, int b) { return a > b ? a : b; };
    pl.wX = d.in <= 16 ? 16 : pad4(d.in);
    pl.wT0 = pad4(mx(mx(d.m1[0], d.m2[0]), mx(mx(d.at[0], d.m3[0]), d.m3[2])));
    pl.wM1 = pad4(mx(mx(d.m1[1], d.at[1]), d.m3[1]));
    pl.wF = pad4(d.m2[1]);
    pl.wJ = pad4(d.self_dim + d.m2[1]);
    if (d.net == CN_NET_LSTM_RL) {
        pl.wT0 = pad4(mx(pl.wT0, mx(4 * d.lstm_h, mx(d.lm1[0], d.lm1[2]))));
        pl.wM1 = pad4(mx(pl.wM1, mx(d.lstm_h, mx(d.lm1[1], d.lm1[3]))));
        pl.wF = pad4(mx(pl.wF, d.lstm_h));
        pl.wJ = pad4(d.self_dim + mx(d.m2[1], d.lstm_h));
    }
    int o = 0;
    pl.oX = o; o += rows * pl.wX;
    pl.oT0 = o; o += rows * pl.wT0;
    pl.oM1 = o; o += rows * pl.wM1;
    pl.oF = o; o += rows * pl.wF;
    pl.oG = o; o += pl.CA * pl.wM1;
    pl.oJ = o; o += pl.CA * pl.wJ;
    pl.oS = o; o += pad4(rows);
    pl.oW = o; o += pad4(rows);
    pl.oV = o; o += pad4(pl.CA);
    o = (o + 3) & ~3;
    pl.oEnv = o; o += 2 * (A1 * F_COUNT + H * 4 + pl.CA);
    pl.oOrd = o; o += pad4(H);
    pl.oOm = o; o += pad4(H * d.om_dim);
    pl.total_floats = o;
    return pl;
}

}

int cn_lookahead_argmax(cn_policy *p, cn_env *env, double epsilon, cudaStream_t s, bool pdl)
{
    return cn_launch(argmax_kernel, (env->p.d.E + 3) / 4, 128, 0, s, pdl, env->p, p->d.A, env->state, env->frozen, p->values,
                     p->action_dev, epsilon, env->step_ctr, env->action_xy, env->action_idx, p->bad_flag);
}

int cn_f32_configure_device(void)
{
    CN_CUDA_CHECK(cudaFuncSetAttribute(lookahead_values_kernel, cudaFuncAttributeMaxDynamicSharedMemorySize, (int)kMaxDynSmem));
    CN_CUDA_CHECK(cudaFuncSetAttribute(forward_kernel, cudaFuncAttributeMaxDynamicSharedMemorySize, (int)kMaxDynSmem));
    return CN_OK;
}

int cn_lookahead_prepare(cn_policy *p, cn_env *env, cudaStream_t s)
{
    int rc = cn_grow(p->values, p->values_cap, env->p.d.E, sizeof(double) * p->d.A);
    if (rc) return rc;
    CN_CUDA_CHECK(cudaMemsetAsync(p->bad_flag, 0, sizeof(int32_t), s));
    return CN_OK;
}

int cn_lookahead_f32(cn_policy *p, cn_env *env, int query_env, double epsilon, cudaStream_t s)
{
    const EnvDims ed = env->p.d;
    if (ed.H > kRowsCap) { cn_set_error("FP32 lookahead supports human_num <= %d", kRowsCap); return CN_EUNSUPPORTED; }
    int rc = cn_lookahead_prepare(p, env, s);
    if (rc) return rc;
    const F32Plan pl = make_plan(p->d, ed.H, p->d.A, ed.A1);
    const size_t smem = sizeof(float) * (size_t)pl.total_floats;
    if (smem > kMaxDynSmem) { cn_set_error("FP32 lookahead needs %zu bytes of shared memory (layer widths too large)", smem); return CN_EUNSUPPORTED; }
    const double gamma_bar = pow(p->cfg.gamma, env->p.time_step * p->cfg.v_pref);
    dim3 grid(ed.E, (p->d.A + pl.CA - 1) / pl.CA);
    lookahead_values_kernel<<<grid, kThreads, smem, s>>>(env->p, p->w, p->d, pl, env->state, env->time, env->human_v,
                                                         env->frozen, p->action_dev, query_env, p->cfg.gamma, gamma_bar,
                                                         p->cfg.v_pref, p->values, env->theta);
    CN_LAUNCH_CHECK();
    return cn_lookahead_argmax(p, env, epsilon, s, true);
}

int cn_transform_f32(cn_policy *p, cn_env *env, float *out_dev, int sort_humans, cudaStream_t s)
{
    const int n = env->p.d.E * env->p.d.H;
    EnvParams ep = env->p;
    ep.kinematics = p->cfg.kinematics;
    transform_kernel<<<(n + 127) / 128, 128, 0, s>>>(ep, p->d, env->state, env->theta, out_dev, sort_humans);
    CN_LAUNCH_CHECK();
    return CN_OK;
}

int cn_forward_f32(cn_policy *p, const float *x_dev, int batch, int H, float *out_dev, cudaStream_t s)
{
    if (H > kRowsCap || H < 1) { cn_set_error("forward supports 1 <= human_num <= %d", kRowsCap); return CN_EUNSUPPORTED; }
    if (batch <= 0) return CN_OK;
    const F32Plan pl = make_plan(p->d, H, batch, 1);
    const size_t smem = sizeof(float) * (size_t)pl.total_floats;
    if (smem > kMaxDynSmem) { cn_set_error("FP32 forward needs %zu bytes of shared memory (layer widths too large)", smem); return CN_EUNSUPPORTED; }
    forward_kernel<<<(batch + pl.CA - 1) / pl.CA, kThreads, smem, s>>>(p->w, p->d, pl, x_dev, batch, out_dev);
    CN_LAUNCH_CHECK();
    return CN_OK;
}
```

modelcrowdnav_b200/csrc/lookahead_tc.cu:

```cuda
#include "env_math.cuh"
#include "umma.cuh"

#include <cuda_fp16.h>
#include <math.h>
#include <stdlib.h>
#include <string.h>

#include <vector>

int cn_lookahead_prepare(cn_policy *p, cn_env *env, cudaStream_t s);
int cn_lookahead_argmax(cn_policy *p, cn_env *env, double epsilon, cudaStream_t s, bool pdl);

namespace {

using namespace umma;

constexpr int K_X = 32;
constexpr int N_H1 = 160;
constexpr int N_M1 = 112;
constexpr int N_F = 64;
constexpr int K_A1 = 224;
constexpr int K_J = 80;
constexpr int ROWS = 128;

__host__ __device__ constexpr uint32_t bytes_of(int rows, int K) { return (uint32_t)rows * K * 2; }
constexpr uint32_t OFF_W1 = 0;
constexpr uint32_t OFF_W2 = OFF_W1 + bytes_of(N_H1, K_X);
constexpr uint32_t OFF_W3 = OFF_W2 + bytes_of(N_M1, N_H1);
constexpr uint32_t OFF_W4 = OFF_W3 + bytes_of(N_M1, N_M1);
constexpr uint32_t OFF_WA1 = OFF_W4 + bytes_of(N_F, N_M1);
constexpr uint32_t OFF_WA2 = OFF_WA1 + bytes_of(N_M1, K_A1);
constexpr uint32_t IMG_A_BYTES = OFF_WA2 + bytes_of(N_M1, N_M1);
constexpr uint32_t TAIL_BYTES = 416;
constexpr uint32_t OFF_M1 = 0;
constexpr uint32_t OFF_M2 = OFF_M1 + bytes_of(N_H1, K_J);
constexpr uint32_t OFF_M3 = OFF_M2 + bytes_of(N_M1, N_H1);
constexpr uint32_t IMG_B_BYTES = OFF_M3 + bytes_of(N_M1, N_M1);

constexpr uint32_t J_TILE_BYTES = bytes_of(ROWS, K_J);

struct TcState {
    uint8_t *img_pair;
    long long *dbg;
    uint8_t *X;
    size_t cap_xtiles;
    uint8_t *J;
    size_t cap_jtiles;
    double *rew;
    size_t cap_rew;
    int num_sms;
    float tail_a[104];
    float tail_b[104];
    uint8_t *img_pair_b;
    float *rowv;
    size_t cap_rowv;
    uint8_t *img_lstm;
    uint8_t *XL;
    size_t cap_xl;
    int32_t *ord;
    size_t cap_ord;
    float *omP;
    size_t cap_om;
    int ktime_on;
    cudaEvent_t kev[5];
};

__device__ __forceinline__ void copy_image_to_smem(uint8_t *dst, const uint8_t *__restrict__ src, uint32_t bytes)
{
    for (uint32_t i = threadIdx.x * 16; i < bytes; i += blockDim.x * 16)
        *reinterpret_cast<uint4 *>(dst + i) = __ldg(reinterpret_cast<const uint4 *>(src + i));
}

__device__ __forceinline__ uint32_t h2(float lo, float hi) { return pack_f16x2(lo, hi); }

__device__ __forceinline__ void split_hl(float x, float &hi, float &lo)
{
    hi = __half2float(__float2half_rn(x));
    lo = x - hi;
}

#include "tc_rows_pair.cuh"
#include "tc_mlp3_pair.cuh"
#include "tc_lstm_pair.cuh"

using RowsKernel = decltype(&tc_rows_pair_kernel<0, false, true>);
constexpr RowsKernel kRowsKernels[2][2][3] = {
    {{tc_rows_pair_kernel<0, false, true>, tc_rows_pair_kernel<5, false, true>, tc_rows_pair_kernel<10, false, true>},
     {tc_rows_pair_kernel<0, true, true>, tc_rows_pair_kernel<5, true, true>, tc_rows_pair_kernel<10, true, true>}},
    {{tc_rows_pair_kernel<0, false, false>, tc_rows_pair_kernel<5, false, false>, tc_rows_pair_kernel<10, false, false>},
     {tc_rows_pair_kernel<0, true, false>, tc_rows_pair_kernel<5, true, false>, tc_rows_pair_kernel<10, true, false>}}};

__global__ void __launch_bounds__(128, 1)
umma_selftest_kernel(const uint8_t *__restrict__ a_img, const uint8_t *__restrict__ b_img, float *__restrict__ d,
                     int N, int K, int mode )
{
    extern __shared__ __align__(128) uint8_t smem[];
    const int tid = threadIdx.x, warp = tid >> 5;
    const uint32_t a_bytes = bytes_of(ROWS, K), b_bytes = mode == 1 ? bytes_of(ROWS, N) : bytes_of(N, K);
    uint8_t *sa = smem, *sb = smem + a_bytes;
    uint8_t *misc = smem + ((a_bytes + b_bytes + 15) & ~15u);
    const uint32_t mbar = smem_u32(misc);
    uint32_t *tmem_slot = reinterpret_cast<uint32_t *>(misc + 8);
    copy_image_to_smem(sa, a_img, a_bytes);
    copy_image_to_smem(sb, b_img, b_bytes);
    if (tid == 0) { mbar_init(mbar, 1); fence_mbar_init(); }
    if (warp == 0) tmem_alloc(smem_u32(tmem_slot), 512);
    fence_async_smem();
    fence_before_sync();
    __syncthreads();
    fence_after_sync();
    const uint32_t tmem = *tmem_slot;
    const uint32_t tlane = tmem + ((uint32_t)(warp * 32) << 16);
    constexpr uint32_t T_A = 256;
    if (mode == 2) {
        for (int c8 = 0; c8 < K / 16; ++c8) {
            uint32_t w[8];
            for (int j = 0; j < 8; ++j) {
                const int k = c8 * 16 + 2 * j;
                const __half2 h = *reinterpret_cast<const __half2 *>(sa + chunk_off(ROWS, tid, k >> 3) + (k & 7) * 2);
                w[j] = *reinterpret_cast<const uint32_t *>(&h);
            }
            st8(tlane + T_A + c8 * 8, w);
        }
        wait_st();
        fence_before_sync();
        __syncthreads();
        fence_after_sync();
    }
    if (tid == 0) {
        if (mode == 1) mma_layer_bmn(tmem, smem_u32(sa), ROWS, smem_u32(sb), K, N, false);
        else if (mode == 2) mma_layer_ts(tmem, tmem + T_A, smem_u32(sb), N, K, N, false);
        else mma_layer(tmem, smem_u32(sa), ROWS, smem_u32(sb), N, K, N, false);
        commit(mbar);
    }
    mbar_wait(mbar, 0);
    fence_after_sync();
    for (int c0 = 0; c0 < N; c0 += 16) {
        uint32_t v[16];
        ld16(tlane + c0, v);
        wait_ld();
        for (int k = 0; k < 16; ++k) d[(size_t)tid * N + c0 + k] = __uint_as_float(v[k]);
    }
    fence_before_sync();
    __syncthreads();
    if (warp == 0) tmem_dealloc(tmem, 512);
}

__global__ void cadrl_min_kernel(EnvParams p, const double *__restrict__ st, const float *__restrict__ rowv,
                                 const double *__restrict__ rew, int A, int NG, int G, int H, double gamma, double gamma_bar_host,
                                 double v_pref_host, double *__restrict__ values)
{
    const int g = blockIdx.x * blockDim.x + threadIdx.x;
    if (g >= NG) return;
    const size_t r0 = (size_t)(g / G) * ROWS + (size_t)(g % G) * H;
    float m = rowv[r0];
    for (int h = 1; h < H; ++h) m = fminf(m, rowv[r0 + h]);
    const double vp = st[st_idx(p.d, F_VPREF, 0, g / A)];
    const double gamma_bar = (vp == v_pref_host) ? gamma_bar_host : pow(gamma, p.time_step * vp);
    values[g] = rew[g] + gamma_bar * (double)m;
}

struct HostLinear { const float *w, *b; int in, out; };

inline void put(std::vector<uint8_t> &img, uint32_t base, int R, int r, int k, float v)
{
    const __half h = __float2half_rn(v);
    memcpy(&img[base + chunk_off(R, r, k >> 3) + (k & 7) * 2], &h, 2);
}
inline float f16r(float v) { return __half2float(__float2half_rn(v)); }

void fill_layer(std::vector<uint8_t> &img, uint32_t base, int R, const HostLinear &L, int k_in0, int n_in, int k_dst0,
                int kb, int ones_n)
{
    for (int n = 0; n < L.out; ++n) {
        for (int k = 0; k < n_in; ++k) put(img, base, R, n, k_dst0 + k, L.w[(size_t)n * L.in + k_in0 + k]);
        if (kb >= 0) {
            const float bh = f16r(L.b[n]);
            put(img, base, R, n, kb, bh);
            put(img, base, R, n, kb + 1, L.b[n] - bh);
        }
    }
    if (ones_n >= 0 && kb >= 0) { put(img, base, R, ones_n, kb, 1.0f); put(img, base, R, ones_n + 1, kb, 1.0f); }
}

void split_rows(uint8_t *dst, const uint8_t *src, int N, int K, int rank)
{
    const int hn = N / 2;
    for (int c = 0; c < K / 8; ++c)
        memcpy(dst + (size_t)c * hn * 16, src + (size_t)c * N * 16 + (size_t)rank * hn * 16, (size_t)hn * 16);
}

void fill_tail(const HostLinear &L, float *tail)
{
    memset(tail, 0, TAIL_BYTES);
    for (int k = 0; k < 100; ++k) tail[k] = L.w[k];
    tail[100] = L.b[0];
}

std::vector<uint8_t> rows_image(const HostLinear *L, bool gs, float *tail)
{
    std::vector<uint8_t> a(IMG_A_BYTES, 0);
    fill_layer(a, OFF_W1, N_H1, L[0], 0, 13, 0, 13, 150);
    fill_layer(a, OFF_W1, N_H1, L[0], 0, 13, 16, -1, -1);
    fill_layer(a, OFF_W2, N_M1, L[1], 0, 150, 0, 150, 100);
    fill_layer(a, OFF_W3, N_M1, L[2], 0, 100, 0, 100, 100);
    fill_layer(a, OFF_W4, N_F, L[3], 0, 100, 0, 100, -1);
    fill_layer(a, OFF_WA1, N_M1, L[4], 0, 100, 0, 100, 100);
    if (gs) fill_layer(a, OFF_WA1, N_M1, L[4], 100, 100, N_M1, -1, -1);
    fill_layer(a, OFF_WA2, N_M1, L[5], 0, 100, 0, 100, -1);
    fill_tail(L[6], tail);
    std::vector<uint8_t> hp(2 * IMG_H_BYTES, 0);
    for (int rank = 0; rank < 2; ++rank) {
        uint8_t *h = hp.data() + (size_t)rank * IMG_H_BYTES;
        split_rows(h + H_W1, a.data() + OFF_W1, N_H1, K_X, rank);
        split_rows(h + H_W2, a.data() + OFF_W2, N_M1, N_H1, rank);
        memcpy(h + H_W3A, rank == 0 ? a.data() + OFF_WA1 : a.data() + OFF_W3, bytes_of(N_M1, N_M1));
        if (gs) split_rows(h + H_WB, a.data() + OFF_WA1 + bytes_of(N_M1, N_M1), N_M1, N_M1, rank);
        split_rows(h + H_W4, a.data() + OFF_W4, N_F, N_M1, rank);
        split_rows(h + H_WA2, a.data() + OFF_WA2, N_M1, N_M1, rank);
        memcpy(h + H_TAIL, tail, TAIL_BYTES);
    }
    return hp;
}

std::vector<uint8_t> mlp3_image(const HostLinear *M, bool x_input, float *tail)
{
    std::vector<uint8_t> b(IMG_B_BYTES, 0);
    if (x_input) {
        fill_layer(b, OFF_M1, N_H1, M[0], 0, 13, 0, 13, 150);
        fill_layer(b, OFF_M1, N_H1, M[0], 0, 13, 16, -1, -1);
    } else {
        fill_layer(b, OFF_M1, N_H1, M[0], 6, 50, 0, -1, -1);
        fill_layer(b, OFF_M1, N_H1, M[0], 0, 6, 56, 62, 150);
        fill_layer(b, OFF_M1, N_H1, M[0], 0, 6, 64, -1, -1);
    }
    fill_layer(b, OFF_M2, N_M1, M[1], 0, 150, 0, 150, 100);
    fill_layer(b, OFF_M3, N_M1, M[2], 0, 100, 0, 100, -1);
    fill_tail(M[3], tail);
    std::vector<uint8_t> hb(2 * IMG_HM_BYTES, 0);
    for (int rank = 0; rank < 2; ++rank) {
        uint8_t *h = hb.data() + (size_t)rank * IMG_HM_BYTES;
        split_rows(h + HM_M1, b.data() + OFF_M1, N_H1, K_J, rank);
        split_rows(h + HM_M2, b.data() + OFF_M2, N_M1, N_H1, rank);
        split_rows(h + HM_M3, b.data() + OFF_M3, N_M1, N_M1, rank);
    }
    return hb;
}

std::vector<uint8_t> lstm_image(const float *src)
{
    const int G4 = 4 * L_HIDDEN;
    const float *w_ih = src, *w_hh = w_ih + (size_t)G4 * 13, *b_ih = w_hh + (size_t)G4 * L_HIDDEN, *b_hh = b_ih + G4;
    std::vector<float> wi((size_t)N_LG * 13, 0.0f), wh((size_t)N_LG * L_HIDDEN, 0.0f), bb(N_LG, 0.0f);
    for (int n = 0; n < N_LG; ++n) {
        const int half = n / 128, gate = (n % 128) / 32, cl = n % 32;
        const int ncell = half ? L_HIDDEN - L_CELLS0 : L_CELLS0;
        if (cl >= ncell) continue;
        const int r = gate * L_HIDDEN + (half ? L_CELLS0 + cl : cl);
        memcpy(&wi[(size_t)n * 13], w_ih + (size_t)r * 13, sizeof(float) * 13);
        memcpy(&wh[(size_t)n * L_HIDDEN], w_hh + (size_t)r * L_HIDDEN, sizeof(float) * L_HIDDEN);
        bb[n] = b_ih[r] + b_hh[r];
    }
    const HostLinear Li = {wi.data(), bb.data(), 13, N_LG}, Lh = {wh.data(), bb.data(), L_HIDDEN, N_LG};
    std::vector<uint8_t> li(bytes_of(N_LG, K_X), 0), lh(bytes_of(N_LG, K_LH), 0);
    fill_layer(li, 0, N_LG, Li, 0, 13, 0, 13, -1);
    fill_layer(li, 0, N_LG, Li, 0, 13, 16, -1, -1);
    fill_layer(lh, 0, N_LG, Lh, 0, L_HIDDEN, 0, -1, -1);
    fill_layer(lh, 0, N_LG, Lh, 0, L_HIDDEN, 56, -1, -1);
    std::vector<uint8_t> hl(2 * IMG_HL_BYTES, 0);
    for (int rank = 0; rank < 2; ++rank) {
        uint8_t *h = hl.data() + (size_t)rank * IMG_HL_BYTES;
        split_rows(h + HL_WIH, li.data(), N_LG, K_X, rank);
        split_rows(h + HL_WHH, lh.data(), N_LG, K_LH, rank);
    }
    return hl;
}

struct PairGrid {
    int clusters, rounds;
    size_t tiles;
};
PairGrid pair_grid(int num_sms, int ntiles)
{
    int clusters = num_sms / 2;
    const int slots_needed = (ntiles + 3) / 4;
    if (clusters > slots_needed) clusters = slots_needed;
    const int rounds = (ntiles + 4 * clusters - 1) / (4 * clusters);
    return {clusters, rounds, (size_t)rounds * 4 * clusters};
}

int stamp(TcState *t, int i, const char *name, cudaStream_t s)
{
    if (name) cn_trace_mark(name, s);
    if (t->ktime_on) CN_CUDA_CHECK(cudaEventRecord(t->kev[i], s));
    return CN_OK;
}

}

constexpr int kOmItems = 8;
__global__ void __launch_bounds__(N_H1)
tc_om_bias_kernel(EnvParams p, SarlDims d, LinearDev m10, const double *__restrict__ st, const double *__restrict__ human_v,
                  int query_env, float *__restrict__ P)
{
    __shared__ float om[kOmItems][8 * 8 * 3];
    __shared__ int cell_of[kOmItems][CN_MAX_HUMANS];
    __shared__ double vrot_of[kOmItems][CN_MAX_HUMANS][2];
    const EnvDims ed = p.d;
    const int H = ed.H, cells = d.cell_num * d.cell_num;
    const long long item0 = (long long)blockIdx.x * kOmItems, n_items = (long long)ed.E * H;
    const double dt = p.time_step;
    for (int idx = threadIdx.x; idx < kOmItems * H; idx += blockDim.x) {
        const int it = idx / H, j = idx - it * H;
        const long long item = item0 + it;
        int cell = -1;
        double vxr = 0.0, vyr = 0.0;
        if (item < n_items) {
            const int e = (int)(item / H), i = (int)(item - (long long)e * H);
            auto get = [&](int k, int f) -> double {
                const double vx = query_env ? human_v[(size_t)(0 * H + k) * ed.E + e] : st[st_idx(ed, F_VX, k + 1, e)];
                const double vy = query_env ? human_v[(size_t)(1 * H + k) * ed.E + e] : st[st_idx(ed, F_VY, k + 1, e)];
                if (f == 0) return st[st_idx(ed, F_PX, k + 1, e)] + vx * dt;
                if (f == 1) return st[st_idx(ed, F_PY, k + 1, e)] + vy * dt;
                return f == 2 ? vx : vy;
            };
            if (j != i) cell = occupancy_map_pair(d, i, j, get, vxr, vyr);
        }
        cell_of[it][j] = cell;
        vrot_of[it][j][0] = vxr; vrot_of[it][j][1] = vyr;
    }
    __syncthreads();
    for (int idx = threadIdx.x; idx < kOmItems * cells; idx += blockDim.x) {
        const int it = idx / cells, c = idx - it * cells;
        double cnt = 0.0, sx = 0.0, sy = 0.0;
        for (int j = 0; j < H; ++j)
            if (cell_of[it][j] == c) { cnt += 1.0; sx += vrot_of[it][j][0]; sy += vrot_of[it][j][1]; }
        occupancy_map_store(d.om_ch, c, cnt, sx, sy, om[it]);
    }
    __syncthreads();
    const int n = threadIdx.x;
    float acc[kOmItems];
#pragma unroll
    for (int it = 0; it < kOmItems; ++it) acc[it] = 0.0f;
    if (n < m10.out)
        for (int k = 0; k < d.om_dim; ++k) {
            const float w = m10.wt[(size_t)(13 + k) * m10.ld + n];
#pragma unroll
            for (int it = 0; it < kOmItems; ++it) acc[it] = fmaf(om[it][k], w, acc[it]);
        }
#pragma unroll
    for (int it = 0; it < kOmItems; ++it)
        if (item0 + it < n_items) P[(size_t)(item0 + it) * N_H1 + n] = acc[it];
}

int cn_tc_init(cn_policy *p)
{
    const SarlDims &d = p->d;
    if (d.net == CN_NET_CADRL) {
        if (!(d.in == 13 && d.m3[0] == 150 && d.m3[1] == 100 && d.m3[2] == 100 && d.m3[3] == 1)) {
            cn_set_error("CN_PREC_F16_TC is specialised for the default [cadrl] mlp_dims (150, 100, 100, 1); use CN_PREC_F32 "
                         "for other shapes");
            return CN_EUNSUPPORTED;
        }
    } else if (d.net == CN_NET_LSTM_RL) {
        if (!(d.in == 13 && d.self_dim == 6 && d.lstm_h == L_HIDDEN && d.lm1[0] == 0 && d.om_dim == 0 && d.m3[0] == 150 &&
              d.m3[1] == 100 && d.m3[2] == 100 && d.m3[3] == 1)) {
            cn_set_error("CN_PREC_F16_TC runs LSTM-RL's default shape only (no interaction module, no occupancy maps, "
                         "global_state_dim 50, mlp2_dims 150,100,100,1); use CN_PREC_F32 for other shapes");
            return CN_EUNSUPPORTED;
        }
    } else {
        const bool ok = d.net == CN_NET_SARL && d.in == 13 + d.om_dim && d.self_dim == 6 && d.m1[0] == 150 && d.m1[1] == 100 &&
                        d.m2[0] == 100 && d.m2[1] == 50 && d.at[0] == 100 && d.at[1] == 100 && d.at[2] == 1 &&
                        d.m3[0] == 150 && d.m3[1] == 100 && d.m3[2] == 100 && d.m3[3] == 1;
        if (!ok) {
            cn_set_error("CN_PREC_F16_TC is specialised for the default [sarl] dims (150,100 / 100,50 / 100,100,1 / "
                         "150,100,100,1) and the default [cadrl] mlp_dims; use CN_PREC_F32 for other shapes / networks");
            return CN_EUNSUPPORTED;
        }
    }
    TcState *t = new TcState();
    memset(t, 0, sizeof(*t));
    p->tc = t;
    cudaDeviceProp prop;
    CN_CUDA_CHECK(cudaGetDeviceProperties(&prop, p->device));
    t->num_sms = prop.multiProcessorCount;
    for (const auto &by_om : kRowsKernels)
        for (const auto &by_ht : by_om)
            for (RowsKernel k : by_ht) CN_CUDA_CHECK(cudaFuncSetAttribute(k, cudaFuncAttributeMaxDynamicSharedMemorySize, (int)Q_SMEM));
    CN_CUDA_CHECK(cudaFuncSetAttribute(tc_mlp3_pair_kernel<0>, cudaFuncAttributeMaxDynamicSharedMemorySize, (int)M_SMEM));
    CN_CUDA_CHECK(cudaFuncSetAttribute(tc_mlp3_pair_kernel<1>, cudaFuncAttributeMaxDynamicSharedMemorySize, (int)M_SMEM));
    CN_CUDA_CHECK(cudaFuncSetAttribute(tc_lstm_pair_kernel, cudaFuncAttributeMaxDynamicSharedMemorySize, (int)L_SMEM));
    if (cudaMalloc((void **)&t->img_pair, 2 * IMG_H_BYTES) != cudaSuccess ||
        cudaMalloc((void **)&t->img_lstm, 2 * IMG_HL_BYTES) != cudaSuccess ||
        cudaMalloc((void **)&t->img_pair_b, 2 * IMG_HM_BYTES) != cudaSuccess) {
        cn_set_error("cudaMalloc failed for the tensor-core weight images");
        return CN_ENOMEM;
    }
    return CN_OK;
}

void cn_tc_destroy(cn_policy *p)
{
    TcState *t = (TcState *)p->tc;
    if (!t) return;
    if (t->img_pair) cudaFree(t->img_pair);
    if (t->img_pair_b) cudaFree(t->img_pair_b);
    if (t->J) cudaFree(t->J);
    if (t->X) cudaFree(t->X);
    if (t->rew) cudaFree(t->rew);
    if (t->rowv) cudaFree(t->rowv);
    if (t->omP) cudaFree(t->omP);
    if (t->img_lstm) cudaFree(t->img_lstm);
    if (t->XL) cudaFree(t->XL);
    if (t->ord) cudaFree(t->ord);
    if (t->dbg) cudaFree(t->dbg);
    if (t->kev[0]) for (int i = 0; i < 5; ++i) cudaEventDestroy(t->kev[i]);
    delete t;
    p->tc = nullptr;
}

int cn_tc_load_weights(cn_policy *p, const float *flat, cudaStream_t s)
{
    TcState *t = (TcState *)p->tc;
    const SarlDims &d = p->d;
    std::vector<HostLinear> L;
    const float *lstm = nullptr, *src = flat;
    for (const LayerSpec &l : cn_layers(d, p->w)) {
        if (l.dst_hh) lstm = src;
        else L.push_back({src, src + (size_t)l.in * l.out, l.in, l.out});
        src += cn_layer_floats(l);
    }
    const std::vector<uint8_t> hb = mlp3_image(&L[L.size() - 4], d.net == CN_NET_CADRL, t->tail_b);
    std::vector<uint8_t> hp, hl;
    CN_CUDA_CHECK(cudaMemcpyAsync(t->img_pair_b, hb.data(), hb.size(), cudaMemcpyHostToDevice, s));
    if (d.net == CN_NET_SARL) {
        hp = rows_image(L.data(), !d.no_gs, t->tail_a);
        CN_CUDA_CHECK(cudaMemcpyAsync(t->img_pair, hp.data(), hp.size(), cudaMemcpyHostToDevice, s));
    } else if (d.net == CN_NET_LSTM_RL) {
        hl = lstm_image(lstm);
        CN_CUDA_CHECK(cudaMemcpyAsync(t->img_lstm, hl.data(), hl.size(), cudaMemcpyHostToDevice, s));
    }
    CN_CUDA_CHECK(cudaStreamSynchronize(s));
    return CN_OK;
}

int cn_lookahead_tc(cn_policy *p, cn_env *env, int query_env, double epsilon, cudaStream_t s, cudaStream_t tail)
{
    TcState *t = (TcState *)p->tc;
    const EnvDims ed = env->p.d;
    if (ed.H > CN_MAX_HUMANS) { cn_set_error("human_num too large"); return CN_EUNSUPPORTED; }
    int rc = cn_lookahead_prepare(p, env, s);
    if (rc) return rc;
    const bool pipelined = tail && tail != s;
    const int net = p->d.net, A = p->d.A;
    const bool om = p->d.om_dim > 0;
    const size_t NG = (size_t)ed.E * A;
    int G = ROWS / ed.H;
    if (G > 64) G = 64;
    const PairGrid ga = pair_grid(t->num_sms, (int)((NG + G - 1) / G));
    const PairGrid gb = pair_grid(t->num_sms, (int)((NG + ROWS - 1) / ROWS));
    if ((rc = cn_grow(t->J, t->cap_jtiles, (NG + ROWS - 1) / ROWS + 4 * (size_t)(t->num_sms / 2), J_TILE_BYTES, true, s))) return rc;
    if ((rc = cn_grow(t->rew, t->cap_rew, NG, sizeof(double)))) return rc;
    if ((rc = cn_grow(t->X, t->cap_xtiles, ga.tiles, X_TILE_BYTES))) return rc;
    const double gamma_bar = pow(p->cfg.gamma, env->p.time_step * p->cfg.v_pref);
    TailW twa, twb;
    memcpy(twa.w, t->tail_a, sizeof(twa.w));
    memcpy(twb.w, t->tail_b, sizeof(twb.w));
    const int ht = (ed.H == 5 && G == ROWS / 5) ? 5 : ((ed.H == 10 && G == ROWS / 10) ? 10 : 0);
    auto feat = ht == 5 ? tc_features_kernel<5> : (ht == 10 ? tc_features_kernel<10> : tc_features_kernel<0>);

    if ((rc = stamp(t, 0, "features", s))) return rc;
    feat<<<(unsigned)ga.tiles, ROWS, 0, s>>>(env->p, env->state, env->time, env->human_v, p->action_dev, A, query_env, (int)NG, G,
                                             env->theta, t->X, t->J, t->rew);
    CN_LAUNCH_CHECK();
    if ((rc = stamp(t, 1, "rows", s))) return rc;
    if (net == CN_NET_LSTM_RL) {
        if ((rc = cn_grow(t->XL, t->cap_xl, gb.tiles * ed.H, X_TILE_BYTES))) return rc;
        if ((rc = cn_grow(t->ord, t->cap_ord, (size_t)ed.E * ed.H, sizeof(int32_t)))) return rc;
        lstm_order_kernel<<<(ed.E + 127) / 128, 128, 0, s>>>(env->p, env->state, query_env, t->ord);
        CN_LAUNCH_CHECK();
        tc_features_lstm_kernel<<<(unsigned)(gb.tiles * ed.H), ROWS, 0, s>>>(env->p, env->state, env->time, env->human_v, p->action_dev,
                                                                           A, query_env, (int)NG, env->theta, t->ord, t->XL);
        CN_LAUNCH_CHECK();
        tc_lstm_pair_kernel<<<2 * gb.clusters, kThreadsL, L_SMEM, s>>>(t->img_lstm, t->XL, t->J, ed.H, gb.rounds);
        CN_LAUNCH_CHECK();
    } else if (net == CN_NET_CADRL) {
        if ((rc = cn_grow(t->rowv, t->cap_rowv, ga.tiles * ROWS, sizeof(float)))) return rc;
        if ((rc = cn_launch(tc_mlp3_pair_kernel<1>, 2 * ga.clusters, kThreadsM3, M_SMEM, s, false, env->p, env->state, t->img_pair_b,
                            t->X, t->rew, A, (int)NG, p->cfg.gamma, gamma_bar, p->cfg.v_pref, p->values, ga.rounds, twb, t->rowv)))
            return rc;
    } else {
        if (om) {
            const size_t items = (size_t)ed.E * ed.H;
            if ((rc = cn_grow(t->omP, t->cap_om, items, sizeof(float) * N_H1))) return rc;
            tc_om_bias_kernel<<<(unsigned)((items + kOmItems - 1) / kOmItems), N_H1, 0, s>>>(env->p, p->d, p->w.m1[0], env->state,
                                                                                          env->human_v, query_env, t->omP);
            CN_LAUNCH_CHECK();
        }
        const RowsKernel rows = kRowsKernels[p->d.no_gs ? 1 : 0][om ? 1 : 0][ht == 5 ? 1 : (ht == 10 ? 2 : 0)];
        if ((rc = cn_launch(rows, 2 * ga.clusters, kThreadsPair, Q_SMEM, s, !om && !pipelined, env->p, t->img_pair, t->X, t->J, (int)NG,
                            G, ga.rounds, twa, t->dbg, t->omP, A)))
            return rc;
    }
    if (pipelined) {
        CN_CUDA_CHECK(cudaEventRecord(env->ev_rows, s));
        CN_CUDA_CHECK(cudaStreamWaitEvent(tail, env->ev_rows, 0));
        s = tail;
    }
    if ((rc = stamp(t, 2, "mlp3", s))) return rc;
    if (net == CN_NET_CADRL) {
        cadrl_min_kernel<<<(unsigned)((NG + 255) / 256), 256, 0, s>>>(env->p, env->state, t->rowv, t->rew, A, (int)NG, G, ed.H,
                                                                      p->cfg.gamma, gamma_bar, p->cfg.v_pref, p->values);
        CN_LAUNCH_CHECK();
    } else if ((rc = cn_launch(tc_mlp3_pair_kernel<0>, 2 * gb.clusters, kThreadsM3, M_SMEM, s, net != CN_NET_LSTM_RL, env->p,
                                 env->state, t->img_pair_b, t->J, t->rew, A, (int)NG, p->cfg.gamma, gamma_bar, p->cfg.v_pref,
                                 p->values, gb.rounds, twb, nullptr))) {
        return rc;
    }
    if ((rc = stamp(t, 3, "argmax", s))) return rc;
    if ((rc = cn_lookahead_argmax(p, env, epsilon, s, !pipelined))) return rc;
    return stamp(t, 4, nullptr, s);
}

static int selftest_impl(int32_t N, int32_t K, const float *a_host, const float *b_host, float *d_host, int device, int mode)
{
    const int bmn = mode == 1;
    if (N < 16 || N > 256 || N % 16 || K < 16 || K % 16 || K > 256 || (bmn && K > ROWS)) {
        cn_set_error("N in [16,256] step 16, K in [16,256] step 16 (K <= 128 for the MN-major variant)");
        return CN_EINVAL;
    }
    int n = 0;
    if (cudaGetDeviceCount(&n) != cudaSuccess || n == 0) { cudaGetLastError(); cn_set_error("no CUDA device available; no CPU fallback"); return CN_ECUDA; }
    CN_CUDA_CHECK(cudaSetDevice(device));
    std::vector<uint8_t> ai(bytes_of(ROWS, K), 0), bi(bmn ? bytes_of(ROWS, N) : bytes_of(N, K), 0);
    for (int r = 0; r < ROWS; ++r) for (int k = 0; k < K; ++k) put(ai, 0, ROWS, r, k, a_host[(size_t)r * K + k]);
    for (int r = 0; r < N; ++r)
        for (int k = 0; k < K; ++k) {
            if (bmn) put(bi, 0, ROWS, k, r, b_host[(size_t)r * K + k]);
            else put(bi, 0, N, r, k, b_host[(size_t)r * K + k]);
        }
    uint8_t *da = nullptr, *db = nullptr;
    float *dd = nullptr;
    CN_CUDA_CHECK(cudaMalloc((void **)&da, ai.size()));
    CN_CUDA_CHECK(cudaMalloc((void **)&db, bi.size()));
    CN_CUDA_CHECK(cudaMalloc((void **)&dd, sizeof(float) * ROWS * N));
    CN_CUDA_CHECK(cudaMemcpy(da, ai.data(), ai.size(), cudaMemcpyHostToDevice));
    CN_CUDA_CHECK(cudaMemcpy(db, bi.data(), bi.size(), cudaMemcpyHostToDevice));
    const size_t smem = ai.size() + bi.size() + 64;
    CN_CUDA_CHECK(cudaFuncSetAttribute(umma_selftest_kernel, cudaFuncAttributeMaxDynamicSharedMemorySize, (int)smem));
    umma_selftest_kernel<<<1, 128, smem>>>(da, db, dd, N, K, mode);
    CN_LAUNCH_CHECK();
    CN_CUDA_CHECK(cudaDeviceSynchronize());
    CN_CUDA_CHECK(cudaMemcpy(d_host, dd, sizeof(float) * ROWS * N, cudaMemcpyDeviceToHost));
    cudaFree(da); cudaFree(db); cudaFree(dd);
    return CN_OK;
}

extern "C" int cn_selftest_umma(int32_t N, int32_t K, const float *a_host, const float *b_host, float *d_host, int device)
{
    return selftest_impl(N, K, a_host, b_host, d_host, device, 0);
}

extern "C" int cn_selftest_umma_bmn(int32_t N, int32_t K, const float *a_host, const float *b_host, float *d_host, int device)
{
    return selftest_impl(N, K, a_host, b_host, d_host, device, 1);
}

extern "C" int cn_selftest_umma_ts(int32_t N, int32_t K, const float *a_host, const float *b_host, float *d_host, int device)
{
    return selftest_impl(N, K, a_host, b_host, d_host, device, 2);
}

extern "C" int cn_selftest_umma_pair(int32_t N, int32_t K, const float *a_host, const float *b_host, float *d_host,
                                     int32_t reps, long long *cycles_host, int device)
{
    if (N < 32 || N > 256 || N % 16 || K < 16 || K % 16 || K > 256 || reps < 1) {
        cn_set_error("N in [32,256] step 16, K in [16,256] step 16, reps >= 1");
        return CN_EINVAL;
    }
    int n = 0;
    if (cudaGetDeviceCount(&n) != cudaSuccess || n == 0) { cudaGetLastError(); cn_set_error("no CUDA device available; no CPU fallback"); return CN_ECUDA; }
    CN_CUDA_CHECK(cudaSetDevice(device));
    const size_t a_bytes = bytes_of(ROWS, K), b_bytes = bytes_of(N / 2, K);
    std::vector<uint8_t> ai(2 * a_bytes, 0), bi(2 * b_bytes, 0);
    for (int r = 0; r < 2 * ROWS; ++r)
        for (int k = 0; k < K; ++k) put(ai, (uint32_t)((r / ROWS) * a_bytes), ROWS, r % ROWS, k, a_host[(size_t)r * K + k]);
    for (int r = 0; r < N; ++r)
        for (int k = 0; k < K; ++k) put(bi, (uint32_t)((r / (N / 2)) * b_bytes), N / 2, r % (N / 2), k, b_host[(size_t)r * K + k]);
    uint8_t *da = nullptr, *db = nullptr;
    float *dd = nullptr;
    long long *dc = nullptr;
    CN_CUDA_CHECK(cudaMalloc((void **)&da, ai.size()));
    CN_CUDA_CHECK(cudaMalloc((void **)&db, bi.size()));
    CN_CUDA_CHECK(cudaMalloc((void **)&dd, sizeof(float) * 2 * ROWS * N));
    CN_CUDA_CHECK(cudaMalloc((void **)&dc, sizeof(long long)));
    CN_CUDA_CHECK(cudaMemcpy(da, ai.data(), ai.size(), cudaMemcpyHostToDevice));
    CN_CUDA_CHECK(cudaMemcpy(db, bi.data(), bi.size(), cudaMemcpyHostToDevice));
    const size_t smem = a_bytes + b_bytes + 64;
    CN_CUDA_CHECK(cudaFuncSetAttribute(umma_pair_selftest_kernel, cudaFuncAttributeMaxDynamicSharedMemorySize, (int)smem));
    umma_pair_selftest_kernel<<<2, 160, smem>>>(da, db, dd, N, K, reps, dc);
    CN_LAUNCH_CHECK();
    CN_CUDA_CHECK(cudaDeviceSynchronize());
    CN_CUDA_CHECK(cudaMemcpy(d_host, dd, sizeof(float) * 2 * ROWS * N, cudaMemcpyDeviceToHost));
    if (cycles_host) CN_CUDA_CHECK(cudaMemcpy(cycles_host, dc, sizeof(long long), cudaMemcpyDeviceToHost));
    cudaFree(da); cudaFree(db); cudaFree(dd); cudaFree(dc);
    return CN_OK;
}

extern "C" int cn_debug_tc_timing(cn_policy *p, long long *out16)
{
    if (!p || !p->tc) { cn_set_error("policy has no tensor-core state"); return CN_EINVAL; }
    TcState *t = (TcState *)p->tc;
    CN_CUDA_CHECK(cudaSetDevice(p->device));
    if (!t->dbg) {
        CN_CUDA_CHECK(cudaMalloc((void **)&t->dbg, 256 * sizeof(long long)));
        CN_CUDA_CHECK(cudaMemset(t->dbg, 0, 256 * sizeof(long long)));
    }
    CN_CUDA_CHECK(cudaDeviceSynchronize());
    CN_CUDA_CHECK(cudaMemcpy(out16, t->dbg, 256 * sizeof(long long), cudaMemcpyDeviceToHost));
    return CN_OK;
}

extern "C" int cn_debug_kernel_ms(cn_policy *p, int on, float *out4)
{
    if (!p || !p->tc) { cn_set_error("policy has no tensor-core state"); return CN_EINVAL; }
    TcState *t = (TcState *)p->tc;
    CN_CUDA_CHECK(cudaSetDevice(p->device));
    if (out4) {
        if (!t->kev[0]) { cn_set_error("kernel timing was never enabled"); return CN_EINVAL; }
        CN_CUDA_CHECK(cudaEventSynchronize(t->kev[4]));
        for (int i = 0; i < 4; ++i) CN_CUDA_CHECK(cudaEventElapsedTime(&out4[i], t->kev[i], t->kev[i + 1]));
    }
    if (on && !t->kev[0]) for (int i = 0; i < 5; ++i) CN_CUDA_CHECK(cudaEventCreate(&t->kev[i]));
    t->ktime_on = on ? 1 : 0;
    return CN_OK;
}
```

modelcrowdnav_b200/csrc/orca_step.cu:

```cuda
#include "env_math.cuh"

#include <math.h>

#define RVO_EPSILON 0.00001f

namespace {

struct v2 { float x, y; };
struct Line { v2 point, direction; };

__device__ __forceinline__ v2 V(float x, float y) { v2 r; r.x = x; r.y = y; return r; }
__device__ __forceinline__ v2 vadd(v2 a, v2 b) { return V(a.x + b.x, a.y + b.y); }
__device__ __forceinline__ v2 vsub(v2 a, v2 b) { return V(a.x - b.x, a.y - b.y); }
__device__ __forceinline__ v2 vneg(v2 a) { return V(-a.x, -a.y); }
__device__ __forceinline__ v2 vscale(float s, v2 a) { return V(s * a.x, s * a.y); }
__device__ __forceinline__ float vdot(v2 a, v2 b) { return a.x * b.x + a.y * b.y; }
__device__ __forceinline__ float vdet(v2 a, v2 b) { return a.x * b.y - a.y * b.x; }
__device__ __forceinline__ float vabssq(v2 a) { return vdot(a, a); }
__device__ __forceinline__ float vabs(v2 a) { return sqrtf(vdot(a, a)); }
__device__ __forceinline__ v2 vdiv(v2 a, float s) { const float inv = 1.0f / s; return V(a.x * inv, a.y * inv); }
__device__ __forceinline__ v2 vnormalize(v2 a) { return vdiv(a, vabs(a)); }
__device__ __forceinline__ float sqrf(float a) { return a * a; }

__device__ bool lp1(const Line *lines, int lineNo, float radius, v2 opt, bool directionOpt, v2 &result)
{
    const Line L = lines[lineNo];
    const float dotProduct = vdot(L.point, L.direction);
    const float discriminant = sqrf(dotProduct) + sqrf(radius) - vabssq(L.point);
    if (discriminant < 0.0f) return false;

    const float sqrtDiscriminant = sqrtf(discriminant);
    float tLeft = -dotProduct - sqrtDiscriminant;
    float tRight = -dotProduct + sqrtDiscriminant;

    for (int i = 0; i < lineNo; ++i) {
        const Line Li = lines[i];
        const float denominator = vdet(L.direction, Li.direction);
        const float numerator = vdet(Li.direction, vsub(L.point, Li.point));
        if (fabsf(denominator) <= RVO_EPSILON) {
            if (numerator < 0.0f) return false;
            continue;
        }
        const float t = numerator / denominator;
        if (denominator >= 0.0f) tRight = fminf(tRight, t);
        else tLeft = fmaxf(tLeft, t);
        if (tLeft > tRight) return false;
    }

    if (directionOpt) {
        if (vdot(opt, L.direction) > 0.0f) result = vadd(L.point, vscale(tRight, L.direction));
        else result = vadd(L.point, vscale(tLeft, L.direction));
    } else {
        const float t = vdot(L.direction, vsub(opt, L.point));
        if (t < tLeft) result = vadd(L.point, vscale(tLeft, L.direction));
        else if (t > tRight) result = vadd(L.point, vscale(tRight, L.direction));
        else result = vadd(L.point, vscale(t, L.direction));
    }
    return true;
}

__device__ int lp2(const Line *lines, int n, float radius, v2 opt, bool directionOpt, v2 &result)
{
    if (directionOpt) result = vscale(radius, opt);
    else if (vabssq(opt) > sqrf(radius)) result = vscale(radius, vnormalize(opt));
    else result = opt;

    for (int i = 0; i < n; ++i) {
        if (vdet(lines[i].direction, vsub(lines[i].point, result)) > 0.0f) {
            const v2 tmp = result;
            if (!lp1(lines, i, radius, opt, directionOpt, result)) {
                result = tmp;
                return i;
            }
        }
    }
    return n;
}

__device__ void lp3(const Line *lines, int n, int beginLine, float radius, v2 &result)
{
    float distance = 0.0f;
    Line proj[CN_MAX_NEIGHBORS];
    for (int i = beginLine; i < n; ++i) {
        if (vdet(lines[i].direction, vsub(lines[i].point, result)) > distance) {
            int np = 0;
            const Line Li = lines[i];
            for (int j = 0; j < i; ++j) {
                const Line Lj = lines[j];
                Line line;
                const float determinant = vdet(Li.direction, Lj.direction);
                if (fabsf(determinant) <= RVO_EPSILON) {
                    if (vdot(Li.direction, Lj.direction) > 0.0f) continue;
                    line.point = vscale(0.5f, vadd(Li.point, Lj.point));
                } else {
                    const float t = vdet(Lj.direction, vsub(Li.point, Lj.point)) / determinant;
                    line.point = vadd(Li.point, vscale(t, Li.direction));
                }
                line.direction = vnormalize(vsub(Lj.direction, Li.direction));
                proj[np++] = line;
            }
            const v2 tmp = result;
            if (lp2(proj, np, radius, V(-Li.direction.y, Li.direction.x), true, result) < np) result = tmp;
            distance = vdet(Li.direction, vsub(Li.point, result));
        }
    }
}

__device__ void orca_solve(const EnvParams &p, const double *__restrict__ st, int e, int self,
                           const int *cand_first, int n_first, int extra_agent ,
                           double safety_space, float &out_vx, float &out_vy)
{
    const EnvDims d = p.d;
    auto ldf = [&](int field, int agent) { return (float)st[st_idx(d, field, agent, e)]; };
    const v2 pos = V(ldf(F_PX, self), ldf(F_PY, self));
    const v2 vel = V(ldf(F_VX, self), ldf(F_VY, self));
    const float radius_self = (float)(st[st_idx(d, F_R, self, e)] + 0.01 + safety_space);
    const float max_speed = (float)st[st_idx(d, F_VPREF, self, e)];
    const v2 pref = V((float)(st[st_idx(d, F_GX, self, e)] - st[st_idx(d, F_PX, self, e)]),
                      (float)(st[st_idx(d, F_GY, self, e)] - st[st_idx(d, F_PY, self, e)]));

    float nb_d2[CN_MAX_NEIGHBORS];
    int nb_id[CN_MAX_NEIGHBORS];
    int nn = 0;
    const int maxN = p.max_neighbors;
    float rangeSq = sqrf(p.neighbor_dist);
    const int n_cand = n_first + (extra_agent >= 0 ? 1 : 0);
    const double *__restrict__ pxs = st + st_idx(d, F_PX, 0, e), *__restrict__ pys = st + st_idx(d, F_PY, 0, e);
    if (maxN == 10) {
        float d0 = INFINITY, d1 = INFINITY, d2 = INFINITY, d3 = INFINITY, d4 = INFINITY, d5 = INFINITY, d6 = INFINITY,
              d7 = INFINITY, d8 = INFINITY, d9 = INFINITY;
        int i0 = 0, i1 = 0, i2 = 0, i3 = 0, i4 = 0, i5 = 0, i6 = 0, i7 = 0, i8 = 0, i9 = 0;
        const float nd2 = rangeSq;
        for (int c = 0; c < n_cand; ++c) {
            int o;
            if (c < n_first) { o = cand_first[0] + c; if (o >= self && cand_first[1]) ++o; }
            else o = extra_agent;
            const size_t oo = (size_t)o * d.E;
            const float distSq = vabssq(vsub(pos, V((float)pxs[oo], (float)pys[oo])));
            if (distSq < nd2 && distSq < d9) {
                if (nn < 10) ++nn;
#define CN_INS(hi, lo) { const bool sh = distSq < d##lo; const bool here = distSq < d##hi; \
                         i##hi = sh ? i##lo : (here ? o : i##hi); d##hi = sh ? d##lo : (here ? distSq : d##hi); }
                CN_INS(9, 8) CN_INS(8, 7) CN_INS(7, 6) CN_INS(6, 5) CN_INS(5, 4) CN_INS(4, 3) CN_INS(3, 2) CN_INS(2, 1) CN_INS(1, 0)
#undef CN_INS
                if (distSq < d0) { d0 = distSq; i0 = o; }
            }
        }
        nb_id[0] = i0; nb_id[1] = i1; nb_id[2] = i2; nb_id[3] = i3; nb_id[4] = i4;
        nb_id[5] = i5; nb_id[6] = i6; nb_id[7] = i7; nb_id[8] = i8; nb_id[9] = i9;
    } else if (maxN > 0) {
        for (int c = 0; c < n_cand; ++c) {
            int o;
            if (c < n_first) { o = cand_first[0] + c; if (o >= self && cand_first[1]) ++o; }
            else o = extra_agent;
            const float distSq = vabssq(vsub(pos, V(ldf(F_PX, o), ldf(F_PY, o))));
            if (distSq < rangeSq) {
                if (nn < maxN) { nb_d2[nn] = distSq; nb_id[nn] = o; ++nn; }
                int i = nn - 1;
                while (i != 0 && distSq < nb_d2[i - 1]) {
                    nb_d2[i] = nb_d2[i - 1]; nb_id[i] = nb_id[i - 1];
                    --i;
                }
                nb_d2[i] = distSq; nb_id[i] = o;
                if (nn == maxN) rangeSq = nb_d2[nn - 1];
            }
        }
    }

    Line lines[CN_MAX_NEIGHBORS];
    const float invTimeHorizon = 1.0f / p.time_horizon;
    for (int k = 0; k < nn; ++k) {
        const int o = nb_id[k];
        const v2 relativePosition = vsub(V(ldf(F_PX, o), ldf(F_PY, o)), pos);
        const v2 relativeVelocity = vsub(vel, V(ldf(F_VX, o), ldf(F_VY, o)));
        const float distSq = vabssq(relativePosition);
        const float radius_o = (float)(st[st_idx(d, F_R, o, e)] + 0.01 + safety_space);
        const float combinedRadius = radius_self + radius_o;
        const float combinedRadiusSq = sqrf(combinedRadius);
        Line line;
        v2 u;
        if (distSq > combinedRadiusSq) {
            const v2 w = vsub(relativeVelocity, vscale(invTimeHorizon, relativePosition));
            const float wLengthSq = vabssq(w);
            const float dotProduct1 = vdot(w, relativePosition);
            if (dotProduct1 < 0.0f && sqrf(dotProduct1) > combinedRadiusSq * wLengthSq) {
                const float wLength = sqrtf(wLengthSq);
                const v2 unitW = vdiv(w, wLength);
                line.direction = V(unitW.y, -unitW.x);
                u = vscale(combinedRadius * invTimeHorizon - wLength, unitW);
            } else {
                const float leg = sqrtf(distSq - combinedRadiusSq);
                if (vdet(relativePosition, w) > 0.0f) {
                    line.direction = vdiv(V(relativePosition.x * leg - relativePosition.y * combinedRadius,
                                            relativePosition.x * combinedRadius + relativePosition.y * leg), distSq);
                } else {
                    line.direction = vneg(vdiv(V(relativePosition.x * leg + relativePosition.y * combinedRadius,
                                                 -relativePosition.x * combinedRadius + relativePosition.y * leg), distSq));
                }
                const float dotProduct2 = vdot(relativeVelocity, line.direction);
                u = vsub(vscale(dotProduct2, line.direction), relativeVelocity);
            }
        } else {
            const float invTimeStep = 1.0f / p.time_step_f;
            const v2 w = vsub(relativeVelocity, vscale(invTimeStep, relativePosition));
            const float wLength = vabs(w);
            const v2 unitW = vdiv(w, wLength);
            line.direction = V(unitW.y, -unitW.x);
            u = vscale(combinedRadius * invTimeStep - wLength, unitW);
        }
        line.point = vadd(vel, vscale(0.5f, u));
        lines[k] = line;
    }

    v2 newV;
    const int lineFail = lp2(lines, nn, max_speed, pref, false, newV);
    if (lineFail < nn) lp3(lines, nn, lineFail, max_speed, newV);
    out_vx = newV.x;
    out_vy = newV.y;
}

__global__ void __launch_bounds__(128) orca_humans_kernel(EnvParams p, const double *__restrict__ st,
                                                          const uint8_t *__restrict__ frozen,
                                                          double *__restrict__ human_v)
{
    const int tid = blockIdx.x * blockDim.x + threadIdx.x;
    const int E = p.d.E, H = p.d.H;
    if (tid >= E * H) return;
    const int h = tid / E, e = tid - h * E;
    if (frozen[e]) return;
    const int cand[2] = {1, 1};
    float vx, vy;
    orca_solve(p, st, e, h + 1, cand, H - 1, p.robot_visible ? 0 : -1, p.human_safety_space, vx, vy);
    human_v[(size_t)(0 * H + h) * E + e] = (double)vx;
    human_v[(size_t)(1 * H + h) * E + e] = (double)vy;
}

__global__ void __launch_bounds__(128) orca_robot_kernel(EnvParams p, const double *__restrict__ st,
                                                         const uint8_t *__restrict__ frozen, double safety_space,
                                                         double *__restrict__ action_xy,
                                                         int32_t *__restrict__ action_idx)
{
    const int e = blockIdx.x * blockDim.x + threadIdx.x;
    if (e >= p.d.E || frozen[e]) return;
    const int cand[2] = {1, 0};
    float vx, vy;
    orca_solve(p, st, e, 0, cand, p.d.H, -1, safety_space, vx, vy);
    action_xy[e] = (double)vx;
    action_xy[p.d.E + e] = (double)vy;
    action_idx[e] = -1;
}

constexpr int kWarpResetHumans = 16;

__device__ void reset_env(const EnvParams &p, int e, double *__restrict__ st, double *__restrict__ time,
                          uint8_t *__restrict__ frozen, const EnvAccum &acc, double *__restrict__ theta)
{
    const EnvDims d = p.d;
    PhiloxStream rng;
    rng.init(p.seed, (uint64_t)(p.env_id_offset + e), acc.episode_ctr[e], 0u);
    acc.episode_ctr[e] += 1;
    const double PI = 3.141592653589793;
    st[st_idx(d, F_PX, 0, e)] = 0.0; st[st_idx(d, F_PY, 0, e)] = -p.circle_radius;
    st[st_idx(d, F_VX, 0, e)] = 0.0; st[st_idx(d, F_VY, 0, e)] = 0.0;
    st[st_idx(d, F_GX, 0, e)] = 0.0; st[st_idx(d, F_GY, 0, e)] = p.circle_radius;
    st[st_idx(d, F_R, 0, e)] = p.robot_radius; st[st_idx(d, F_VPREF, 0, e)] = p.robot_v_pref;
    constexpr int kLocal = 16;
    double cpx[kLocal], cpy[kLocal], cgx[kLocal], cgy[kLocal], cr[kLocal];
    cpx[0] = 0.0; cpy[0] = -p.circle_radius; cgx[0] = 0.0; cgy[0] = p.circle_radius; cr[0] = p.robot_radius;
    const bool cached = d.H < kLocal;
    auto PX = [&](int a) { return cached ? cpx[a] : st[st_idx(d, F_PX, a, e)]; };
    auto PY = [&](int a) { return cached ? cpy[a] : st[st_idx(d, F_PY, a, e)]; };
    auto GX = [&](int a) { return cached ? cgx[a] : st[st_idx(d, F_GX, a, e)]; };
    auto GY = [&](int a) { return cached ? cgy[a] : st[st_idx(d, F_GY, a, e)]; };
    auto RR = [&](int a) { return cached ? cr[a] : st[st_idx(d, F_R, a, e)]; };
    const int MAX_TRIES = 4096;
    for (int i = 1; i <= d.H; ++i) {
        double px = 0, py = 0, gx = 0, gy = 0;
        double h_radius = p.human_radius, h_v_pref = p.human_v_pref;
        if (p.randomize_attributes) {
            h_v_pref = 0.5 + (1.5 - 0.5) * rng.next();
            h_radius = 0.3 + (0.5 - 0.3) * rng.next();
        }
        if (p.sim_rule == CN_CIRCLE_CROSSING) {
            for (int tries = 0; tries < MAX_TRIES; ++tries) {
                const double angle = rng.next() * PI * 2;
                const double px_noise = (rng.next() - 0.5) * h_v_pref;
                const double py_noise = (rng.next() - 0.5) * h_v_pref;
                px = p.circle_radius * cos(angle) + px_noise;
                py = p.circle_radius * sin(angle) + py_noise;
                bool collide = false;
                for (int a = 0; a < i; ++a) {
                    const double min_dist = h_radius + RR(a) + p.discomfort_dist;
                    if (norm2d(px - PX(a), py - PY(a)) < min_dist || norm2d(px - GX(a), py - GY(a)) < min_dist) {
                        collide = true;
                        break;
                    }
                }
                if (!collide) break;
            }
            gx = -px; gy = -py;
        } else {
            const double sign = (rng.next() > 0.5) ? -1.0 : 1.0;
            for (int tries = 0; tries < MAX_TRIES; ++tries) {
                px = rng.next() * p.square_width * 0.5 * sign;
                py = (rng.next() - 0.5) * p.square_width;
                bool collide = false;
                for (int a = 0; a < i; ++a) {
                    if (norm2d(px - PX(a), py - PY(a)) < h_radius + RR(a) + p.discomfort_dist) { collide = true; break; }
                }
                if (!collide) break;
            }
            for (int tries = 0; tries < MAX_TRIES; ++tries) {
                gx = rng.next() * p.square_width * 0.5 * -sign;
                gy = (rng.next() - 0.5) * p.square_width;
                bool collide = false;
                for (int a = 0; a < i; ++a) {
                    if (norm2d(gx - GX(a), gy - GY(a)) < h_radius + RR(a) + p.discomfort_dist) { collide = true; break; }
                }
                if (!collide) break;
            }
        }
        st[st_idx(d, F_PX, i, e)] = px; st[st_idx(d, F_PY, i, e)] = py;
        st[st_idx(d, F_VX, i, e)] = 0.0; st[st_idx(d, F_VY, i, e)] = 0.0;
        st[st_idx(d, F_GX, i, e)] = gx; st[st_idx(d, F_GY, i, e)] = gy;
        st[st_idx(d, F_R, i, e)] = h_radius; st[st_idx(d, F_VPREF, i, e)] = h_v_pref;
        if (cached) { cpx[i] = px; cpy[i] = py; cgx[i] = gx; cgy[i] = gy; cr[i] = h_radius; }
    }
    time[e] = 0.0;
    theta[e] = 1.5707963267948966;
    frozen[e] = 0;
    acc.ep_steps[e] = 0; acc.ep_return[e] = 0.0;
}

__global__ void __launch_bounds__(128) step_kernel(EnvParams p, double *__restrict__ st, double *__restrict__ time,
                                                   const double *__restrict__ human_v,
                                                   const double *__restrict__ act, int act_aos, int update,
                                                   double *__restrict__ reward_o, uint8_t *__restrict__ done_o,
                                                   uint8_t *__restrict__ info_o, double *__restrict__ dmin_o,
                                                   double *__restrict__ next_obs, uint8_t *__restrict__ frozen,
                                                   EnvAccum acc, double *__restrict__ theta, int fuse_reset)
{
    const int e = blockIdx.x * blockDim.x + threadIdx.x;
    const EnvDims d = p.d;
    if (e >= d.E) return;
    if (frozen[e]) { reward_o[e] = 0.0; done_o[e] = 1; return; }
    const int E = d.E, H = d.H;
    const double a0 = act_aos ? act[2 * (size_t)e] : act[e];
    const double a1 = act_aos ? act[2 * (size_t)e + 1] : act[E + e];
    const double th = p.kinematics != CN_KIN_HOLONOMIC ? theta[e] : 0.0;
    double ax, ay;
    cn_effective_velocity(p.kinematics, th, a0, a1, ax, ay);
    const double dt = p.time_step;
    const double t = time[e];
    auto ag = [&](int f, int a) { return st[st_idx(d, f, a, e)]; };
    const StepOutcome oc = cn_step_outcome(p, ag, H, t, ax, ay);
    const double reward = oc.reward, dmin = oc.dmin;
    const int done = oc.done, info = oc.info;
    const double endx = ag(F_PX, 0) + ax * dt, endy = ag(F_PY, 0) + ay * dt;
    reward_o[e] = reward; done_o[e] = (uint8_t)done; info_o[e] = (uint8_t)info; dmin_o[e] = dmin;

    if (update) {
        st[st_idx(d, F_PX, 0, e)] = endx;
        st[st_idx(d, F_PY, 0, e)] = endy;
        if (p.kinematics == CN_KIN_HOLONOMIC) {
            st[st_idx(d, F_VX, 0, e)] = ax;
            st[st_idx(d, F_VY, 0, e)] = ay;
        } else {
            const double TWO_PI = 2 * 3.141592653589793;
            double t2 = fmod(th + a1, TWO_PI);
            if (t2 < 0) t2 += TWO_PI;
            theta[e] = t2;
            st[st_idx(d, F_VX, 0, e)] = a0 * cos(t2);
            st[st_idx(d, F_VY, 0, e)] = a0 * sin(t2);
        }
        double hvx = human_v[(size_t)(0 * H) * E + e], hvy = human_v[(size_t)(1 * H) * E + e];
        double opx = st[st_idx(d, F_PX, 1, e)], opy = st[st_idx(d, F_PY, 1, e)];
        for (int h = 1; h <= H; ++h) {
            double nvx = 0, nvy = 0, npx = 0, npy = 0;
            if (h < H) {
                nvx = human_v[(size_t)(0 * H + h) * E + e]; nvy = human_v[(size_t)(1 * H + h) * E + e];
                npx = st[st_idx(d, F_PX, h + 1, e)]; npy = st[st_idx(d, F_PY, h + 1, e)];
            }
            st[st_idx(d, F_PX, h, e)] = opx + hvx * dt;
            st[st_idx(d, F_PY, h, e)] = opy + hvy * dt;
            st[st_idx(d, F_VX, h, e)] = hvx;
            st[st_idx(d, F_VY, h, e)] = hvy;
            hvx = nvx; hvy = nvy; opx = npx; opy = npy;
        }
        const double tn = t + dt;
        time[e] = tn;
        const int k = acc.ep_steps[e];
        const double disc = pow(p.gamma, (double)k * dt * st[st_idx(d, F_VPREF, 0, e)]);
        const double ret = acc.ep_return[e] + disc * reward;
        acc.steps[e] += 1;
        if (info == CN_DANGER) { acc.too_close[e] += 1; acc.sum_min_dist[e] += dmin; }
        if (done) {
            acc.episodes[e] += 1;
            if (info == CN_REACHGOAL) { acc.success[e] += 1; acc.sum_success_time[e] += tn; }
            else if (info == CN_COLLISION) { acc.collision[e] += 1; acc.sum_collision_time[e] += tn; }
            else { acc.timeout[e] += 1; acc.sum_timeout_time[e] += p.time_limit; }
            acc.sum_return[e] += ret;
            acc.ep_return[e] = 0.0; acc.ep_steps[e] = 0;
            if (!p.auto_reset) frozen[e] = 1;
            else if (fuse_reset) reset_env(p, e, st, time, frozen, acc, theta);
        } else {
            acc.ep_return[e] = ret; acc.ep_steps[e] = k + 1;
        }
    } else {
        for (int h = 1; h <= H; ++h) {
            const double hvx = human_v[(size_t)(0 * H + h - 1) * E + e];
            const double hvy = human_v[(size_t)(1 * H + h - 1) * E + e];
            next_obs[(size_t)(0 * H + h - 1) * E + e] = st[st_idx(d, F_PX, h, e)] + hvx * dt;
            next_obs[(size_t)(1 * H + h - 1) * E + e] = st[st_idx(d, F_PY, h, e)] + hvy * dt;
            next_obs[(size_t)(2 * H + h - 1) * E + e] = hvx;
            next_obs[(size_t)(3 * H + h - 1) * E + e] = hvy;
            next_obs[(size_t)(4 * H + h - 1) * E + e] = st[st_idx(d, F_R, h, e)];
        }
    }
}

__device__ void reset_env_warp(const EnvParams &p, int e, int lane, double *__restrict__ st, double *__restrict__ time,
                               uint8_t *__restrict__ frozen, const EnvAccum &acc, double *__restrict__ theta)
{
    const EnvDims d = p.d;
    PhiloxStream rng;
    rng.init(p.seed, (uint64_t)(p.env_id_offset + e), acc.episode_ctr[e], 0u);
    __syncwarp();
    if (lane == 0) acc.episode_ctr[e] += 1;
    const double PI = 3.141592653589793;
    if (lane == 0) {
        st[st_idx(d, F_PX, 0, e)] = 0.0; st[st_idx(d, F_PY, 0, e)] = -p.circle_radius;
        st[st_idx(d, F_VX, 0, e)] = 0.0; st[st_idx(d, F_VY, 0, e)] = 0.0;
        st[st_idx(d, F_GX, 0, e)] = 0.0; st[st_idx(d, F_GY, 0, e)] = p.circle_radius;
        st[st_idx(d, F_R, 0, e)] = p.robot_radius; st[st_idx(d, F_VPREF, 0, e)] = p.robot_v_pref;
    }
    __syncwarp();
    constexpr int kSlots = (CN_MAX_HUMANS + 32) / 32;
    double cpx[kSlots], cpy[kSlots], cgx[kSlots], cgy[kSlots], cr[kSlots];
#pragma unroll
    for (int k = 0; k < kSlots; ++k) { cpx[k] = cpy[k] = cgx[k] = cgy[k] = cr[k] = 0.0; }
    if (lane == 0) { cpx[0] = 0.0; cpy[0] = -p.circle_radius; cgx[0] = 0.0; cgy[0] = p.circle_radius; cr[0] = p.robot_radius; }
    const int MAX_TRIES = 4096;
    for (int i = 1; i <= d.H; ++i) {
        double px = 0, py = 0, gx = 0, gy = 0;
        double h_radius = p.human_radius, h_v_pref = p.human_v_pref;
        if (p.randomize_attributes) {
            h_v_pref = 0.5 + (1.5 - 0.5) * rng.next();
            h_radius = 0.3 + (0.5 - 0.3) * rng.next();
        }
        if (p.sim_rule == CN_CIRCLE_CROSSING) {
            for (int tries = 0; tries < MAX_TRIES; ++tries) {
                const double angle = rng.next() * PI * 2;
                const double px_noise = (rng.next() - 0.5) * h_v_pref;
                const double py_noise = (rng.next() - 0.5) * h_v_pref;
                px = p.circle_radius * cos(angle) + px_noise;
                py = p.circle_radius * sin(angle) + py_noise;
                bool collide = false;
#pragma unroll
                for (int k = 0; k < kSlots; ++k) {
                    if (lane + 32 * k >= i) continue;
                    const double min_dist = h_radius + cr[k] + p.discomfort_dist;
                    collide = collide || norm2d(px - cpx[k], py - cpy[k]) < min_dist || norm2d(px - cgx[k], py - cgy[k]) < min_dist;
                }
                if (!__any_sync(0xffffffffu, collide)) break;
            }
            gx = -px; gy = -py;
        } else {
            const double sign = (rng.next() > 0.5) ? -1.0 : 1.0;
            for (int tries = 0; tries < MAX_TRIES; ++tries) {
                px = rng.next() * p.square_width * 0.5 * sign;
                py = (rng.next() - 0.5) * p.square_width;
                bool collide = false;
#pragma unroll
                for (int k = 0; k < kSlots; ++k)
                    if (lane + 32 * k < i)
                        collide = collide || norm2d(px - cpx[k], py - cpy[k]) < h_radius + cr[k] + p.discomfort_dist;
                if (!__any_sync(0xffffffffu, collide)) break;
            }
            for (int tries = 0; tries < MAX_TRIES; ++tries) {
                gx = rng.next() * p.square_width * 0.5 * -sign;
                gy = (rng.next() - 0.5) * p.square_width;
                bool collide = false;
#pragma unroll
                for (int k = 0; k < kSlots; ++k)
                    if (lane + 32 * k < i)
                        collide = collide || norm2d(gx - cgx[k], gy - cgy[k]) < h_radius + cr[k] + p.discomfort_dist;
                if (!__any_sync(0xffffffffu, collide)) break;
            }
        }
        if (lane == 0) {
            st[st_idx(d, F_PX, i, e)] = px; st[st_idx(d, F_PY, i, e)] = py;
            st[st_idx(d, F_VX, i, e)] = 0.0; st[st_idx(d, F_VY, i, e)] = 0.0;
            st[st_idx(d, F_GX, i, e)] = gx; st[st_idx(d, F_GY, i, e)] = gy;
            st[st_idx(d, F_R, i, e)] = h_radius; st[st_idx(d, F_VPREF, i, e)] = h_v_pref;
        }
#pragma unroll
        for (int k = 0; k < kSlots; ++k)
            if (lane + 32 * k == i) { cpx[k] = px; cpy[k] = py; cgx[k] = gx; cgy[k] = gy; cr[k] = h_radius; }
    }
    if (lane == 0) {
        time[e] = 0.0;
        theta[e] = 1.5707963267948966;
        frozen[e] = 0;
        acc.ep_steps[e] = 0; acc.ep_return[e] = 0.0;
    }
}

__global__ void __launch_bounds__(128) reset_warp_kernel(EnvParams p, double *__restrict__ st, double *__restrict__ time,
                                                         const uint8_t *__restrict__ done, int only_done,
                                                         uint8_t *__restrict__ frozen, EnvAccum acc, double *__restrict__ theta)
{
    const int e = (blockIdx.x * blockDim.x + threadIdx.x) >> 5, lane = threadIdx.x & 31;
    if (e >= p.d.E) return;
    if (only_done && !done[e]) return;
    reset_env_warp(p, e, lane, st, time, frozen, acc, theta);
}

__global__ void __launch_bounds__(128) reset_kernel(EnvParams p, double *__restrict__ st, double *__restrict__ time,
                                                    const uint8_t *__restrict__ done, int only_done,
                                                    uint8_t *__restrict__ frozen, EnvAccum acc, double *__restrict__ theta)
{
    const int e = blockIdx.x * blockDim.x + threadIdx.x;
    if (e >= p.d.E) return;
    if (only_done && !done[e]) return;
    reset_env(p, e, st, time, frozen, acc, theta);
}

__global__ void pack_kernel(EnvDims d, double *__restrict__ st, double *__restrict__ stage, int to_soa)
{
    const size_t n = (size_t)d.E * d.A1 * F_COUNT;
    for (size_t i = blockIdx.x * (size_t)blockDim.x + threadIdx.x; i < n; i += (size_t)gridDim.x * blockDim.x) {
        const int e = (int)(i % d.E);
        const size_t r = i / d.E;
        const int a = (int)(r % d.A1), f = (int)(r / d.A1);
        const size_t j = ((size_t)e * d.A1 + a) * F_COUNT + f;
        if (to_soa) st[i] = stage[j];
        else stage[j] = st[i];
    }
}

__global__ void io_unpack_kernel(EnvDims d, double *__restrict__ st, double *__restrict__ time, const double *__restrict__ blk)
{
    const size_t n = (size_t)d.E * d.A1 * F_COUNT;
    for (size_t i = blockIdx.x * (size_t)blockDim.x + threadIdx.x; i < n + d.E; i += (size_t)gridDim.x * blockDim.x) {
        if (i >= n) { time[i - n] = blk[i]; continue; }
        const int e = (int)(i % d.E);
        const size_t r = i / d.E;
        const int a = (int)(r % d.A1), f = (int)(r / d.A1);
        st[i] = blk[((size_t)e * d.A1 + a) * F_COUNT + f];
    }
}

__global__ void io_pack_kernel(EnvDims d, const double *__restrict__ st, const double *__restrict__ time,
                               const double *__restrict__ reward, const int32_t *__restrict__ action_idx,
                               const uint8_t *__restrict__ done, const uint8_t *__restrict__ info, double *__restrict__ blk)
{
    const size_t n = (size_t)d.E * d.A1 * F_COUNT;
    int32_t *b_idx = reinterpret_cast<int32_t *>(blk + n + 2 * (size_t)d.E);
    uint8_t *b_done = reinterpret_cast<uint8_t *>(b_idx + d.E), *b_info = b_done + d.E;
    for (size_t i = blockIdx.x * (size_t)blockDim.x + threadIdx.x; i < n + d.E; i += (size_t)gridDim.x * blockDim.x) {
        if (i >= n) {
            const size_t e = i - n;
            blk[n + e] = time[e];
            blk[n + d.E + e] = reward[e];
            b_idx[e] = action_idx[e]; b_done[e] = done[e]; b_info[e] = info[e];
            continue;
        }
        const int e = (int)(i % d.E);
        const size_t r = i / d.E;
        const int a = (int)(r % d.A1), f = (int)(r / d.A1);
        blk[((size_t)e * d.A1 + a) * F_COUNT + f] = st[i];
    }
}

__global__ void clear_episode_kernel(int E, uint8_t *frozen, EnvAccum acc, uint8_t *done, double *theta)
{
    const int e = blockIdx.x * blockDim.x + threadIdx.x;
    if (e >= E) return;
    frozen[e] = 0; done[e] = 0;
    theta[e] = 1.5707963267948966;
    acc.ep_steps[e] = 0; acc.ep_return[e] = 0.0;
}

__global__ void transpose_out_kernel(int E, int H, int C, const double *__restrict__ src, double *__restrict__ dst)
{
    const size_t n = (size_t)E * H * C;
    for (size_t i = blockIdx.x * (size_t)blockDim.x + threadIdx.x; i < n; i += (size_t)gridDim.x * blockDim.x) {
        const int e = (int)(i % E);
        const size_t r = i / E;
        const int h = (int)(r % H), c = (int)(r / H);
        dst[((size_t)e * H + h) * C + c] = src[i];
    }
}

__global__ void set_actions_kernel(int E, const double *__restrict__ aos, double *__restrict__ action_xy,
                                   int32_t *__restrict__ action_idx)
{
    const int e = blockIdx.x * blockDim.x + threadIdx.x;
    if (e >= E) return;
    action_xy[e] = aos[2 * (size_t)e];
    action_xy[E + e] = aos[2 * (size_t)e + 1];
    action_idx[e] = -1;
}

__global__ void set_human_v_kernel(int E, int H, const double *__restrict__ aos, double *__restrict__ human_v)
{
    const int i = blockIdx.x * blockDim.x + threadIdx.x;
    if (i >= E * H) return;
    const int h = i / E, e = i - h * E;
    human_v[(size_t)(0 * H + h) * E + e] = aos[((size_t)e * H + h) * 2];
    human_v[(size_t)(1 * H + h) * E + e] = aos[((size_t)e * H + h) * 2 + 1];
}

}

static inline int grid_for(int n, int block) { return (n + block - 1) / block; }

int cn_launch_set_human_v(cn_env *env, const double *aos_dev, cudaStream_t s)
{
    const int n = env->p.d.E * env->p.d.H;
    set_human_v_kernel<<<grid_for(n, 128), 128, 0, s>>>(env->p.d.E, env->p.d.H, aos_dev, env->human_v);
    CN_LAUNCH_CHECK();
    env->orca_valid = 1;
    return CN_OK;
}

int cn_launch_orca(cn_env *env, cudaStream_t s)
{
    const int n = env->p.d.E * env->p.d.H;
    const int bs = cn_small_block();
    orca_humans_kernel<<<grid_for(n, bs), bs, 0, s>>>(env->p, env->state, env->frozen, env->human_v);
    CN_LAUNCH_CHECK();
    env->orca_valid = 1;
    return CN_OK;
}

int cn_launch_robot_orca(cn_env *env, double safety_space, cudaStream_t s)
{
    orca_robot_kernel<<<grid_for(env->p.d.E, 128), 128, 0, s>>>(env->p, env->state, env->frozen, safety_space,
                                                                  env->action_xy, env->action_idx);
    CN_LAUNCH_CHECK();
    return CN_OK;
}

int cn_launch_step(cn_env *env, const double *action_xy_dev, int update, cudaStream_t s, int fuse_reset)
{
    const double *act = action_xy_dev ? action_xy_dev : env->action_xy;
    const int bs = cn_small_block();
    const bool split_reset = fuse_reset && update && env->p.d.H >= kWarpResetHumans;
    if (split_reset) fuse_reset = 0;
    step_kernel<<<grid_for(env->p.d.E, bs), bs, 0, s>>>(env->p, env->state, env->time, env->human_v, act,
                                                            action_xy_dev ? 1 : 0, update, env->reward, env->done,
                                                            env->info, env->dmin, env->next_obs, env->frozen,
                                                            env->acc, env->theta, fuse_reset);
    CN_LAUNCH_CHECK();
    if (update) env->orca_valid = 0;
    if (split_reset) return cn_launch_reset(env, 1, s);
    return CN_OK;
}

int cn_launch_reset(cn_env *env, int only_done, cudaStream_t s)
{
    const int bs = cn_small_block();
    if (env->p.d.H >= kWarpResetHumans)
        reset_warp_kernel<<<grid_for(env->p.d.E * 32, 128), 128, 0, s>>>(env->p, env->state, env->time, env->done, only_done,
                                                                          env->frozen, env->acc, env->theta);
    else
        reset_kernel<<<grid_for(env->p.d.E, bs), bs, 0, s>>>(env->p, env->state, env->time, env->done, only_done,
                                                             env->frozen, env->acc, env->theta);
    CN_LAUNCH_CHECK();
    env->orca_valid = 0;
    return CN_OK;
}

int cn_launch_pack(cn_env *env, int to_soa, cudaStream_t s)
{
    const size_t n = (size_t)env->p.d.E * env->p.d.A1 * F_COUNT;
    int grid = (int)((n + 255) / 256);
    if (grid > 148 * 8) grid = 148 * 8;
    pack_kernel<<<grid, 256, 0, s>>>(env->p.d, env->state, env->stage, to_soa);
    CN_LAUNCH_CHECK();
    if (to_soa) {
        clear_episode_kernel<<<grid_for(env->p.d.E, 128), 128, 0, s>>>(env->p.d.E, env->frozen, env->acc, env->done, env->theta);
        CN_LAUNCH_CHECK();
        env->orca_valid = 0;
    }
    return CN_OK;
}

int cn_launch_pack_keep(cn_env *env, cudaStream_t s)
{
    const size_t n = (size_t)env->p.d.E * env->p.d.A1 * F_COUNT;
    int grid = (int)((n + 255) / 256);
    if (grid > 148 * 8) grid = 148 * 8;
    pack_kernel<<<grid, 256, 0, s>>>(env->p.d, env->state, env->stage, 1);
    CN_LAUNCH_CHECK();
    env->orca_valid = 0;
    return CN_OK;
}

int cn_launch_io(cn_env *env, double *blk, int unpack, cudaStream_t s)
{
    const size_t n = (size_t)env->p.d.E * env->p.d.A1 * F_COUNT + env->p.d.E;
    int grid = (int)((n + 255) / 256);
    if (grid > 148 * 8) grid = 148 * 8;
    grid *= 2;
    if (unpack) {
        io_unpack_kernel<<<grid, 128, 0, s>>>(env->p.d, env->state, env->time, blk);
        env->orca_valid = 0;
    } else {
        io_pack_kernel<<<grid, 128, 0, s>>>(env->p.d, env->state, env->time, env->reward, env->action_idx, env->done, env->info, blk);
    }
    CN_LAUNCH_CHECK();
    return CN_OK;
}

int cn_launch_transpose_out(int E, int H, int C, const double *src, double *dst, cudaStream_t s)
{
    const size_t n = (size_t)E * H * C;
    int grid = (int)((n + 255) / 256);
    if (grid > 148 * 8) grid = 148 * 8;
    transpose_out_kernel<<<grid, 256, 0, s>>>(E, H, C, src, dst);
    CN_LAUNCH_CHECK();
    return CN_OK;
}

int cn_launch_set_actions(cn_env *env, const double *aos_dev, cudaStream_t s)
{
    set_actions_kernel<<<grid_for(env->p.d.E, 128), 128, 0, s>>>(env->p.d.E, aos_dev, env->action_xy,
                                                                   env->action_idx);
    CN_LAUNCH_CHECK();
    return CN_OK;
}
```

Measured before the change: 12.12 million.

## Fuse env step and auto-reset into warp-per-env kernel merged with lookahead argmax

Rewrites the environment step as a warp-per-environment kernel: lanes process humans in parallel, ballot/shuffle reductions handle collision and dmin, and an auto-reset of done environments runs inline in the same warp. The lookahead paths now take a join event and a step flag so action selection (argmax) and the env step can run in one launch, optionally with programmatic dependent launch. This removes the separate step and reset launches and the serial per-thread human loop. In exchange, small environments waste lanes, and the code path becomes more complex.

```diff
diff --git a/modelcrowdnav_b200/csrc/capi.cu b/modelcrowdnav_b200/csrc/capi.cu
--- a/modelcrowdnav_b200/csrc/capi.cu
+++ b/modelcrowdnav_b200/csrc/capi.cu
@@ -344,10 +344,7 @@
         cn_set_error("cn_env_step: call cn_env_orca for the current state first");
         return CN_EINVAL;
     }
-    int rc = cn_launch_step(env, action_xy_dev, update, s);
-    if (rc) return rc;
-    if (update && env->p.auto_reset) rc = cn_launch_reset(env, 1, s);
-    return rc;
+    return cn_launch_step(env, action_xy_dev, update, s);
 }
 
 int cn_env_get_views(cn_env *env, cn_env_views *out)
@@ -662,10 +659,11 @@
     return CN_OK;
 }
 
-static int lookahead(cn_policy *p, cn_env *env, int query_env, double epsilon, cudaStream_t s, cudaStream_t tail = nullptr)
-{
-    if (p->cfg.precision == CN_PREC_F16_TC) return cn_lookahead_tc(p, env, query_env, epsilon, s, tail);
-    return cn_lookahead_f32(p, env, query_env, epsilon, s);
+static int lookahead(cn_policy *p, cn_env *env, int query_env, double epsilon, cudaStream_t s, cudaStream_t tail = nullptr,
+                     cudaEvent_t join = nullptr, bool step = false)
+{
+    if (p->cfg.precision == CN_PREC_F16_TC) return cn_lookahead_tc(p, env, query_env, epsilon, s, tail, join, step);
+    return cn_lookahead_f32(p, env, query_env, epsilon, s, join, step);
 }
 
 static int sync_and_check_values(cn_policy *p, cudaStream_t s)
@@ -797,12 +795,9 @@
         if ((rc = cn_launch_orca(env, env->side_stream))) return rc;
         CN_CUDA_CHECK(cudaEventRecord(env->ev_join, env->side_stream));
     } else if ((rc = cn_launch_orca(env, s))) return rc;
-    if ((rc = lookahead(p, env, query_env, epsilon, s, tail))) return rc;
+    if ((rc = lookahead(p, env, query_env, epsilon, s, tail, fork ? env->ev_join : nullptr, true))) return rc;
     if (tail) s = tail;
     *cur = s;
-    if (fork) CN_CUDA_CHECK(cudaStreamWaitEvent(s, env->ev_join, 0));
-    cn_trace_mark("step", s);
-    if ((rc = cn_launch_step(env, nullptr, 1, s, env->p.auto_reset ? 1 : 0))) return rc;
     cn_trace_mark("step_done", s);
     return rc;
 }
@@ -869,7 +864,7 @@
                 rc = lookahead(p, env, query_env, epsilon, s);
             else if (robot_mode == CN_ROBOT_ORCA) rc = cn_launch_robot_orca(env, safety_space, s);
             if (rc) return rc;
-            if ((rc = cn_launch_step(env, nullptr, 1, s, 0))) return rc;
+            if ((rc = cn_launch_step(env, nullptr, 1, s))) return rc;
         }
         if (rec) {
             CN_CUDA_CHECK(cudaMemcpyAsync(rec->reward_dev + (size_t)step * E, env->reward, sizeof(double) * E, cudaMemcpyDeviceToDevice, s));
diff --git a/modelcrowdnav_b200/csrc/cn_common.cuh b/modelcrowdnav_b200/csrc/cn_common.cuh
--- a/modelcrowdnav_b200/csrc/cn_common.cuh
+++ b/modelcrowdnav_b200/csrc/cn_common.cuh
@@ -285,12 +285,15 @@
 
 int cn_launch_orca(cn_env *env, cudaStream_t s);
 int cn_launch_robot_orca(cn_env *env, double safety_space, cudaStream_t s);
-int cn_launch_step(cn_env *env, const double *action_xy_dev, int update, cudaStream_t s, int fuse_reset = 0);
+int cn_launch_step(cn_env *env, const double *action_xy_dev, int update, cudaStream_t s);
 int cn_launch_reset(cn_env *env, int only_done, cudaStream_t s);
 int cn_launch_pack(cn_env *env, int to_soa, cudaStream_t s);
 int cn_launch_io(cn_env *env, double *blk, int unpack, cudaStream_t s);
 
-int cn_lookahead_f32(cn_policy *p, cn_env *env, int query_env, double epsilon, cudaStream_t s);
+int cn_lookahead_f32(cn_policy *p, cn_env *env, int query_env, double epsilon, cudaStream_t s, cudaEvent_t join = nullptr,
+                     bool step = false);
+int cn_lookahead_argmax(cn_policy *p, cn_env *env, double epsilon, cudaStream_t s, bool pdl);
+int cn_launch_argmax_step(cn_policy *p, cn_env *env, double epsilon, cudaStream_t s, bool pdl);
 int cn_transform_f32(cn_policy *p, cn_env *env, float *out_dev, int sort_humans, cudaStream_t s);
 int cn_forward_f32(cn_policy *p, const float *x_dev, int batch, int H, float *out_dev, cudaStream_t s);
 int cn_f32_configure_device(void);
@@ -298,4 +301,5 @@
 int cn_tc_init(cn_policy *p);
 void cn_tc_destroy(cn_policy *p);
 int cn_tc_load_weights(cn_policy *p, const float *flat_host, cudaStream_t s);
-int cn_lookahead_tc(cn_policy *p, cn_env *env, int query_env, double epsilon, cudaStream_t s, cudaStream_t tail = nullptr);
+int cn_lookahead_tc(cn_policy *p, cn_env *env, int query_env, double epsilon, cudaStream_t s, cudaStream_t tail = nullptr,
+                    cudaEvent_t join = nullptr, bool step = false);
diff --git a/modelcrowdnav_b200/csrc/env_math.cuh b/modelcrowdnav_b200/csrc/env_math.cuh
--- a/modelcrowdnav_b200/csrc/env_math.cuh
+++ b/modelcrowdnav_b200/csrc/env_math.cuh
@@ -17,28 +17,9 @@
     int done, info;
 };
 
-template <typename Acc>
-__device__ __forceinline__ StepOutcome cn_step_outcome(const EnvParams &p, Acc ag, int H, double t, double ax, double ay)
-{
-    const double rpx = ag(F_PX, 0), rpy = ag(F_PY, 0), rr = ag(F_R, 0);
-    const double dt = p.time_step;
-    double dmin = INFINITY;
-    bool collision = false;
-    for (int h = 1; h <= H; ++h) {
-        const double px = ag(F_PX, h) - rpx;
-        const double py = ag(F_PY, h) - rpy;
-        const double vx = ag(F_VX, h) - ax;
-        const double vy = ag(F_VY, h) - ay;
-        const double ex = px + vx * dt;
-        const double ey = py + vy * dt;
-        const double closest = cn_point_to_segment_dist0(px, py, ex, ey) - ag(F_R, h) - rr;
-        if (!collision) {
-            if (closest < 0) collision = true;
-            else if (closest < dmin) dmin = closest;
-        }
-    }
-    const double endx = rpx + ax * dt, endy = rpy + ay * dt;
-    const bool reaching_goal = norm2d(endx - ag(F_GX, 0), endy - ag(F_GY, 0)) < rr;
+__device__ __forceinline__ StepOutcome cn_step_ladder(const EnvParams &p, double t, bool collision, double dmin, bool reaching_goal)
+{
+    const double dt = p.time_step;
     StepOutcome o;
     o.dmin = dmin;
     if (t >= p.time_limit - 1) { o.reward = 0; o.done = 1; o.info = CN_TIMEOUT; }
@@ -49,6 +30,226 @@
         o.done = 0; o.info = CN_DANGER;
     } else { o.reward = 0; o.done = 0; o.info = CN_NOTHING; }
     return o;
+}
+
+template <typename Acc>
+__device__ __forceinline__ double cn_step_clearance(const EnvParams &p, Acc ag, int h, double rpx, double rpy, double rr,
+                                                    double ax, double ay)
+{
+    const double dt = p.time_step;
+    const double px = ag(F_PX, h) - rpx;
+    const double py = ag(F_PY, h) - rpy;
+    const double vx = ag(F_VX, h) - ax;
+    const double vy = ag(F_VY, h) - ay;
+    const double ex = px + vx * dt;
+    const double ey = py + vy * dt;
+    return cn_point_to_segment_dist0(px, py, ex, ey) - ag(F_R, h) - rr;
+}
+
+template <typename Acc>
+__device__ __forceinline__ StepOutcome cn_step_outcome(const EnvParams &p, Acc ag, int H, double t, double ax, double ay)
+{
+    const double rpx = ag(F_PX, 0), rpy = ag(F_PY, 0), rr = ag(F_R, 0);
+    const double dt = p.time_step;
+    double dmin = INFINITY;
+    bool collision = false;
+    for (int h = 1; h <= H; ++h) {
+        const double closest = cn_step_clearance(p, ag, h, rpx, rpy, rr, ax, ay);
+        if (!collision) {
+            if (closest < 0) collision = true;
+            else if (closest < dmin) dmin = closest;
+        }
+    }
+    const double endx = rpx + ax * dt, endy = rpy + ay * dt;
+    return cn_step_ladder(p, t, collision, dmin, norm2d(endx - ag(F_GX, 0), endy - ag(F_GY, 0)) < rr);
+}
+
+__device__ inline void reset_env_warp(const EnvParams &p, int e, int lane, double *__restrict__ st, double *__restrict__ time,
+                                      uint8_t *__restrict__ frozen, const EnvAccum &acc, double *__restrict__ theta)
+{
+    const EnvDims d = p.d;
+    PhiloxStream rng;
+    rng.init(p.seed, (uint64_t)(p.env_id_offset + e), acc.episode_ctr[e], 0u);
+    __syncwarp();
+    if (lane == 0) acc.episode_ctr[e] += 1;
+    const double PI = 3.141592653589793;
+    if (lane == 0) {
+        st[st_idx(d, F_PX, 0, e)] = 0.0; st[st_idx(d, F_PY, 0, e)] = -p.circle_radius;
+        st[st_idx(d, F_VX, 0, e)] = 0.0; st[st_idx(d, F_VY, 0, e)] = 0.0;
+        st[st_idx(d, F_GX, 0, e)] = 0.0; st[st_idx(d, F_GY, 0, e)] = p.circle_radius;
+        st[st_idx(d, F_R, 0, e)] = p.robot_radius; st[st_idx(d, F_VPREF, 0, e)] = p.robot_v_pref;
+    }
+    __syncwarp();
+    constexpr int kSlots = (CN_MAX_HUMANS + 31) / 32;
+    double cpx[kSlots], cpy[kSlots], cgx[kSlots], cgy[kSlots], cr[kSlots];
+#pragma unroll
+    for (int k = 0; k < kSlots; ++k) { cpx[k] = cpy[k] = cgx[k] = cgy[k] = cr[k] = 0.0; }
+    if (lane == 0) { cpx[0] = 0.0; cpy[0] = -p.circle_radius; cgx[0] = 0.0; cgy[0] = p.circle_radius; cr[0] = p.robot_radius; }
+    const int MAX_TRIES = 4096;
+    for (int i = 1; i <= d.H; ++i) {
+        double px = 0, py = 0, gx = 0, gy = 0;
+        double h_radius = p.human_radius, h_v_pref = p.human_v_pref;
+        if (p.randomize_attributes) {
+            h_v_pref = 0.5 + (1.5 - 0.5) * rng.next();
+            h_radius = 0.3 + (0.5 - 0.3) * rng.next();
+        }
+        if (p.sim_rule == CN_CIRCLE_CROSSING) {
+            for (int tries = 0; tries < MAX_TRIES; ++tries) {
+                const double angle = rng.next() * PI * 2;
+                const double px_noise = (rng.next() - 0.5) * h_v_pref;
+                const double py_noise = (rng.next() - 0.5) * h_v_pref;
+                px = p.circle_radius * cos(angle) + px_noise;
+                py = p.circle_radius * sin(angle) + py_noise;
+                bool collide = false;
+#pragma unroll
+                for (int k = 0; k < kSlots; ++k) {
+                    if (lane + 32 * k >= i) continue;
+                    const double min_dist = h_radius + cr[k] + p.discomfort_dist;
+                    collide = collide || norm2d(px - cpx[k], py - cpy[k]) < min_dist || norm2d(px - cgx[k], py - cgy[k]) < min_dist;
+                }
+                if (!__any_sync(0xffffffffu, collide)) break;
+            }
+            gx = -px; gy = -py;
+        } else {
+            const double sign = (rng.next() > 0.5) ? -1.0 : 1.0;
+            for (int tries = 0; tries < MAX_TRIES; ++tries) {
+                px = rng.next() * p.square_width * 0.5 * sign;
+                py = (rng.next() - 0.5) * p.square_width;
+                bool collide = false;
+#pragma unroll
+                for (int k = 0; k < kSlots; ++k)
+                    if (lane + 32 * k < i)
+                        collide = collide || norm2d(px - cpx[k], py - cpy[k]) < h_radius + cr[k] + p.discomfort_dist;
+                if (!__any_sync(0xffffffffu, collide)) break;
+            }
+            for (int tries = 0; tries < MAX_TRIES; ++tries) {
+                gx = rng.next() * p.square_width * 0.5 * -sign;
+                gy = (rng.next() - 0.5) * p.square_width;
+                bool collide = false;
+#pragma unroll
+                for (int k = 0; k < kSlots; ++k)
+                    if (lane + 32 * k < i)
+                        collide = collide || norm2d(gx - cgx[k], gy - cgy[k]) < h_radius + cr[k] + p.discomfort_dist;
+                if (!__any_sync(0xffffffffu, collide)) break;
+            }
+        }
+        if (lane == 0) {
+            st[st_idx(d, F_PX, i, e)] = px; st[st_idx(d, F_PY, i, e)] = py;
+            st[st_idx(d, F_VX, i, e)] = 0.0; st[st_idx(d, F_VY, i, e)] = 0.0;
+            st[st_idx(d, F_GX, i, e)] = gx; st[st_idx(d, F_GY, i, e)] = gy;
+            st[st_idx(d, F_R, i, e)] = h_radius; st[st_idx(d, F_VPREF, i, e)] = h_v_pref;
+        }
+#pragma unroll
+        for (int k = 0; k < kSlots; ++k)
+            if (lane + 32 * k == i) { cpx[k] = px; cpy[k] = py; cgx[k] = gx; cgy[k] = gy; cr[k] = h_radius; }
+    }
+    if (lane == 0) {
+        time[e] = 0.0;
+        theta[e] = 1.5707963267948966;
+        frozen[e] = 0;
+        acc.ep_steps[e] = 0; acc.ep_return[e] = 0.0;
+    }
+}
+
+struct StepOut {
+    double *reward, *dmin;
+    uint8_t *done, *info;
+    double *next_obs;
+};
+inline StepOut cn_step_out(const cn_env *env) { return StepOut{env->reward, env->dmin, env->done, env->info, env->next_obs}; }
+
+__device__ __forceinline__ void cn_step_env_warp(const EnvParams &p, int e, int lane, double a0, double a1, int update,
+                                                 double *__restrict__ st, double *__restrict__ time,
+                                                 const double *__restrict__ human_v, const StepOut &out,
+                                                 uint8_t *__restrict__ frozen, const EnvAccum &acc, double *__restrict__ theta)
+{
+    const EnvDims d = p.d;
+    const int E = d.E, H = d.H;
+    const double th = p.kinematics != CN_KIN_HOLONOMIC ? theta[e] : 0.0;
+    double ax, ay;
+    cn_effective_velocity(p.kinematics, th, a0, a1, ax, ay);
+    const double dt = p.time_step;
+    auto ag = [&](int f, int a) { return st[st_idx(d, f, a, e)]; };
+    const double rpx = ag(F_PX, 0), rpy = ag(F_PY, 0), rr = ag(F_R, 0);
+    double dmin = INFINITY;
+    bool collision = false;
+    for (int h0 = 1; h0 <= H; h0 += 32) {
+        const int h = h0 + lane;
+        const bool mine = h <= H;
+        double closest = INFINITY, hpx = 0, hpy = 0, hvx = 0, hvy = 0;
+        if (mine) {
+            hpx = ag(F_PX, h); hpy = ag(F_PY, h);
+            hvx = human_v[(size_t)(0 * H + h - 1) * E + e]; hvy = human_v[(size_t)(1 * H + h - 1) * E + e];
+            closest = cn_step_clearance(p, ag, h, rpx, rpy, rr, ax, ay);
+        }
+        const unsigned hit = __ballot_sync(0xffffffffu, mine && closest < 0);
+        if (!collision) {
+            const bool before_hit = hit == 0 || lane < __ffs(hit) - 1;
+            if (mine && before_hit && closest < dmin) dmin = closest;
+            collision = hit != 0;
+        }
+        if (!mine) continue;
+        if (update) {
+            st[st_idx(d, F_PX, h, e)] = hpx + hvx * dt;
+            st[st_idx(d, F_PY, h, e)] = hpy + hvy * dt;
+            st[st_idx(d, F_VX, h, e)] = hvx;
+            st[st_idx(d, F_VY, h, e)] = hvy;
+        } else {
+            out.next_obs[(size_t)(0 * H + h - 1) * E + e] = hpx + hvx * dt;
+            out.next_obs[(size_t)(1 * H + h - 1) * E + e] = hpy + hvy * dt;
+            out.next_obs[(size_t)(2 * H + h - 1) * E + e] = hvx;
+            out.next_obs[(size_t)(3 * H + h - 1) * E + e] = hvy;
+            out.next_obs[(size_t)(4 * H + h - 1) * E + e] = ag(F_R, h);
+        }
+    }
+#pragma unroll
+    for (int off = 16; off > 0; off >>= 1) {
+        const double o = __shfl_xor_sync(0xffffffffu, dmin, off);
+        dmin = o < dmin ? o : dmin;
+    }
+    const double t = time[e];
+    const double endx = rpx + ax * dt, endy = rpy + ay * dt;
+    const StepOutcome oc = cn_step_ladder(p, t, collision, dmin, norm2d(endx - ag(F_GX, 0), endy - ag(F_GY, 0)) < rr);
+    const double reward = oc.reward;
+    const int done = oc.done, info = oc.info;
+    if (lane == 0) {
+        out.reward[e] = reward; out.done[e] = (uint8_t)done; out.info[e] = (uint8_t)info; out.dmin[e] = dmin;
+    }
+    if (!update) return;
+    if (lane == 0) {
+        const double tn = t + dt;
+        time[e] = tn;
+        const int k = acc.ep_steps[e];
+        const double disc = pow(p.gamma, (double)k * dt * ag(F_VPREF, 0));
+        const double ret = acc.ep_return[e] + disc * reward;
+        acc.steps[e] += 1;
+        if (info == CN_DANGER) { acc.too_close[e] += 1; acc.sum_min_dist[e] += dmin; }
+        if (done) {
+            acc.episodes[e] += 1;
+            if (info == CN_REACHGOAL) { acc.success[e] += 1; acc.sum_success_time[e] += tn; }
+            else if (info == CN_COLLISION) { acc.collision[e] += 1; acc.sum_collision_time[e] += tn; }
+            else { acc.timeout[e] += 1; acc.sum_timeout_time[e] += p.time_limit; }
+            acc.sum_return[e] += ret;
+            acc.ep_return[e] = 0.0; acc.ep_steps[e] = 0;
+            if (!p.auto_reset) frozen[e] = 1;
+        } else {
+            acc.ep_return[e] = ret; acc.ep_steps[e] = k + 1;
+        }
+        st[st_idx(d, F_PX, 0, e)] = endx;
+        st[st_idx(d, F_PY, 0, e)] = endy;
+        if (p.kinematics == CN_KIN_HOLONOMIC) {
+            st[st_idx(d, F_VX, 0, e)] = ax;
+            st[st_idx(d, F_VY, 0, e)] = ay;
+        } else {
+            const double TWO_PI = 2 * 3.141592653589793;
+            double t2 = fmod(th + a1, TWO_PI);
+            if (t2 < 0) t2 += TWO_PI;
+            theta[e] = t2;
+            st[st_idx(d, F_VX, 0, e)] = a0 * cos(t2);
+            st[st_idx(d, F_VY, 0, e)] = a0 * sin(t2);
+        }
+    }
+    if (done && p.auto_reset) reset_env_warp(p, e, lane, st, time, frozen, acc, theta);
 }
 
 __device__ __forceinline__ void cn_rotate(const float *s, float *o, int kinematics = CN_KIN_HOLONOMIC)
diff --git a/modelcrowdnav_b200/csrc/lookahead_f32.cu b/modelcrowdnav_b200/csrc/lookahead_f32.cu
--- a/modelcrowdnav_b200/csrc/lookahead_f32.cu
+++ b/modelcrowdnav_b200/csrc/lookahead_f32.cu
@@ -340,6 +340,45 @@
         values[(size_t)e * pl.A + a0 + i] = rew[i] + gamma_bar * (double)Vv[i];
 }
 
+__device__ __forceinline__ int argmax_env_warp(const EnvParams &p, int A, int e, int lane, const double *__restrict__ st,
+                                               const double *__restrict__ values, const double *__restrict__ actions,
+                                               double epsilon, uint32_t *__restrict__ step_ctr, double *__restrict__ action_xy,
+                                               int32_t *__restrict__ action_idx, int32_t *__restrict__ bad_flag)
+{
+    const EnvDims d = p.d;
+    double max_value = -INFINITY;
+    int best = -1;
+    for (int a = lane; a < A; a += 32) {
+        const double v = values[(size_t)e * A + a];
+        if (v > max_value) { max_value = v; best = a; }
+    }
+#pragma unroll
+    for (int off = 16; off > 0; off >>= 1) {
+        const double ov = __shfl_xor_sync(0xffffffffu, max_value, off);
+        const int ob = __shfl_xor_sync(0xffffffffu, best, off);
+        if (ob >= 0 && (best < 0 || ov > max_value || (ov == max_value && ob < best))) { max_value = ov; best = ob; }
+    }
+    if (lane == 0) {
+        const bool reached = norm2d(st[st_idx(d, F_PY, 0, e)] - st[st_idx(d, F_GY, 0, e)],
+                                    st[st_idx(d, F_PX, 0, e)] - st[st_idx(d, F_GX, 0, e)]) < st[st_idx(d, F_R, 0, e)];
+        if (reached) best = 0;
+        else {
+            bool random_pick = false;
+            if (epsilon > 0.0) {
+                PhiloxStream rng;
+                rng.init(p.seed, (uint64_t)(p.env_id_offset + e), step_ctr[e], 1u);
+                step_ctr[e] += 1;
+                if (rng.next() < epsilon) { best = min(A - 1, (int)(rng.next() * A)); random_pick = true; }
+            }
+            if (!random_pick && best < 0) { atomicExch(bad_flag, 1); atomicAdd(bad_flag + 1, 1); best = 0; }
+        }
+        action_idx[e] = best;
+        action_xy[e] = actions[2 * best];
+        action_xy[d.E + e] = actions[2 * best + 1];
+    }
+    return __shfl_sync(0xffffffffu, best, 0);
+}
+
 __global__ void __launch_bounds__(128)
 argmax_kernel(EnvParams p, int A, const double *__restrict__ st, const uint8_t *__restrict__ frozen,
               const double *__restrict__ values, const double *__restrict__ actions, double epsilon,
@@ -347,38 +386,27 @@
               int32_t *__restrict__ action_idx, int32_t *__restrict__ bad_flag)
 {
     const int e = (blockIdx.x * blockDim.x + threadIdx.x) >> 5, lane = threadIdx.x & 31;
-    const EnvDims d = p.d;
     asm volatile("griddepcontrol.wait;" ::: "memory");
-    if (e >= d.E || frozen[e]) return;
-    double max_value = -INFINITY;
-    int best = -1;
-    for (int a = lane; a < A; a += 32) {
-        const double v = values[(size_t)e * A + a];
-        if (v > max_value) { max_value = v; best = a; }
-    }
-#pragma unroll
-    for (int off = 16; off > 0; off >>= 1) {
-        const double ov = __shfl_xor_sync(0xffffffffu, max_value, off);
-        const int ob = __shfl_xor_sync(0xffffffffu, best, off);
-        if (ob >= 0 && (best < 0 || ov > max_value || (ov == max_value && ob < best))) { max_value = ov; best = ob; }
-    }
-    if (lane != 0) return;
-    const bool reached = norm2d(st[st_idx(d, F_PY, 0, e)] - st[st_idx(d, F_GY, 0, e)],
-                                st[st_idx(d, F_PX, 0, e)] - st[st_idx(d, F_GX, 0, e)]) < st[st_idx(d, F_R, 0, e)];
-    if (reached) best = 0;
-    else {
-        bool random_pick = false;
-        if (epsilon > 0.0) {
-            PhiloxStream rng;
-            rng.init(p.seed, (uint64_t)(p.env_id_offset + e), step_ctr[e], 1u);
-            step_ctr[e] += 1;
-            if (rng.next() < epsilon) { best = min(A - 1, (int)(rng.next() * A)); random_pick = true; }
-        }
-        if (!random_pick && best < 0) { atomicExch(bad_flag, 1); atomicAdd(bad_flag + 1, 1); best = 0; }
-    }
-    action_idx[e] = best;
-    action_xy[e] = actions[2 * best];
-    action_xy[d.E + e] = actions[2 * best + 1];
+    if (e >= p.d.E || frozen[e]) return;
+    argmax_env_warp(p, A, e, lane, st, values, actions, epsilon, step_ctr, action_xy, action_idx, bad_flag);
+}
+
+__global__ void __maxnreg__(72)
+argmax_step_kernel(EnvParams p, int A, double *__restrict__ st, double *__restrict__ time, const double *__restrict__ human_v,
+                   const double *__restrict__ values, const double *__restrict__ actions, double epsilon,
+                   uint32_t *__restrict__ step_ctr, double *__restrict__ action_xy, int32_t *__restrict__ action_idx,
+                   int32_t *__restrict__ bad_flag, StepOut out, uint8_t *__restrict__ frozen, EnvAccum acc,
+                   double *__restrict__ theta)
+{
+    const int e = (blockIdx.x * blockDim.x + threadIdx.x) >> 5, lane = threadIdx.x & 31;
+    asm volatile("griddepcontrol.wait;" ::: "memory");
+    if (e >= p.d.E) return;
+    if (frozen[e]) {
+        if (lane == 0) { out.reward[e] = 0.0; out.done[e] = 1; }
+        return;
+    }
+    const int best = argmax_env_warp(p, A, e, lane, st, values, actions, epsilon, step_ctr, action_xy, action_idx, bad_flag);
+    cn_step_env_warp(p, e, lane, actions[2 * best], actions[2 * best + 1], 1, st, time, human_v, out, frozen, acc, theta);
 }
 
 __global__ void transform_kernel(EnvParams p, SarlDims nd, const double *__restrict__ st, const double *__restrict__ theta,
@@ -480,6 +508,15 @@
                      p->action_dev, epsilon, env->step_ctr, env->action_xy, env->action_idx, p->bad_flag);
 }
 
+int cn_launch_argmax_step(cn_policy *p, cn_env *env, double epsilon, cudaStream_t s, bool pdl)
+{
+    int rc = cn_launch(argmax_step_kernel, (env->p.d.E + 3) / 4, 128, 0, s, pdl, env->p, p->d.A, env->state, env->time,
+                       env->human_v, p->values, p->action_dev, epsilon, env->step_ctr, env->action_xy, env->action_idx,
+                       p->bad_flag, cn_step_out(env), env->frozen, env->acc, env->theta);
+    env->orca_valid = 0;
+    return rc;
+}
+
 int cn_f32_configure_device(void)
 {
     CN_CUDA_CHECK(cudaFuncSetAttribute(lookahead_values_kernel, cudaFuncAttributeMaxDynamicSharedMemorySize, (int)kMaxDynSmem));
@@ -495,7 +532,7 @@
     return CN_OK;
 }
 
-int cn_lookahead_f32(cn_policy *p, cn_env *env, int query_env, double epsilon, cudaStream_t s)
+int cn_lookahead_f32(cn_policy *p, cn_env *env, int query_env, double epsilon, cudaStream_t s, cudaEvent_t join, bool step)
 {
     const EnvDims ed = env->p.d;
     if (ed.H > kRowsCap) { cn_set_error("FP32 lookahead supports human_num <= %d", kRowsCap); return CN_EUNSUPPORTED; }
@@ -506,11 +543,12 @@
     if (smem > kMaxDynSmem) { cn_set_error("FP32 lookahead needs %zu bytes of shared memory (layer widths too large)", smem); return CN_EUNSUPPORTED; }
     const double gamma_bar = pow(p->cfg.gamma, env->p.time_step * p->cfg.v_pref);
     dim3 grid(ed.E, (p->d.A + pl.CA - 1) / pl.CA);
+    if (join) CN_CUDA_CHECK(cudaStreamWaitEvent(s, join, 0));
     lookahead_values_kernel<<<grid, kThreads, smem, s>>>(env->p, p->w, p->d, pl, env->state, env->time, env->human_v,
                                                          env->frozen, p->action_dev, query_env, p->cfg.gamma, gamma_bar,
                                                          p->cfg.v_pref, p->values, env->theta);
     CN_LAUNCH_CHECK();
-    return cn_lookahead_argmax(p, env, epsilon, s, true);
+    return step ? cn_launch_argmax_step(p, env, epsilon, s, true) : cn_lookahead_argmax(p, env, epsilon, s, true);
 }
 
 int cn_transform_f32(cn_policy *p, cn_env *env, float *out_dev, int sort_humans, cudaStream_t s)
diff --git a/modelcrowdnav_b200/csrc/lookahead_tc.cu b/modelcrowdnav_b200/csrc/lookahead_tc.cu
--- a/modelcrowdnav_b200/csrc/lookahead_tc.cu
+++ b/modelcrowdnav_b200/csrc/lookahead_tc.cu
@@ -9,7 +9,6 @@
 #include <vector>
 
 int cn_lookahead_prepare(cn_policy *p, cn_env *env, cudaStream_t s);
-int cn_lookahead_argmax(cn_policy *p, cn_env *env, double epsilon, cudaStream_t s, bool pdl);
 
 namespace {
 
@@ -445,7 +444,8 @@
     return CN_OK;
 }
 
-int cn_lookahead_tc(cn_policy *p, cn_env *env, int query_env, double epsilon, cudaStream_t s, cudaStream_t tail)
+int cn_lookahead_tc(cn_policy *p, cn_env *env, int query_env, double epsilon, cudaStream_t s, cudaStream_t tail,
+                    cudaEvent_t join, bool step)
 {
     TcState *t = (TcState *)p->tc;
     const EnvDims ed = env->p.d;
@@ -508,6 +508,7 @@
         CN_CUDA_CHECK(cudaStreamWaitEvent(tail, env->ev_rows, 0));
         s = tail;
     }
+    if (join) CN_CUDA_CHECK(cudaStreamWaitEvent(s, join, 0));
     if ((rc = stamp(t, 2, "mlp3", s))) return rc;
     if (net == CN_NET_CADRL) {
         cadrl_min_kernel<<<(unsigned)((NG + 255) / 256), 256, 0, s>>>(env->p, env->state, t->rowv, t->rew, A, (int)NG, G, ed.H,
@@ -519,7 +520,8 @@
         return rc;
     }
     if ((rc = stamp(t, 3, "argmax", s))) return rc;
-    if ((rc = cn_lookahead_argmax(p, env, epsilon, s, !pipelined))) return rc;
+    if ((rc = step ? cn_launch_argmax_step(p, env, epsilon, s, !pipelined) : cn_lookahead_argmax(p, env, epsilon, s, !pipelined)))
+        return rc;
     return stamp(t, 4, nullptr, s);
 }
 
diff --git a/modelcrowdnav_b200/csrc/orca_step.cu b/modelcrowdnav_b200/csrc/orca_step.cu
--- a/modelcrowdnav_b200/csrc/orca_step.cu
+++ b/modelcrowdnav_b200/csrc/orca_step.cu
@@ -332,178 +332,20 @@
     acc.ep_steps[e] = 0; acc.ep_return[e] = 0.0;
 }
 
-__global__ void __launch_bounds__(128) step_kernel(EnvParams p, double *__restrict__ st, double *__restrict__ time,
-                                                   const double *__restrict__ human_v,
-                                                   const double *__restrict__ act, int act_aos, int update,
-                                                   double *__restrict__ reward_o, uint8_t *__restrict__ done_o,
-                                                   uint8_t *__restrict__ info_o, double *__restrict__ dmin_o,
-                                                   double *__restrict__ next_obs, uint8_t *__restrict__ frozen,
-                                                   EnvAccum acc, double *__restrict__ theta, int fuse_reset)
-{
-    const int e = blockIdx.x * blockDim.x + threadIdx.x;
-    const EnvDims d = p.d;
-    if (e >= d.E) return;
-    if (frozen[e]) { reward_o[e] = 0.0; done_o[e] = 1; return; }
-    const int E = d.E, H = d.H;
+__global__ void __launch_bounds__(128) step_warp_kernel(EnvParams p, double *__restrict__ st, double *__restrict__ time,
+                                                        const double *__restrict__ human_v,
+                                                        const double *__restrict__ act, int act_aos, int update, StepOut out,
+                                                        uint8_t *__restrict__ frozen, EnvAccum acc, double *__restrict__ theta)
+{
+    const int e = (blockIdx.x * blockDim.x + threadIdx.x) >> 5, lane = threadIdx.x & 31;
+    if (e >= p.d.E) return;
+    if (frozen[e]) {
+        if (lane == 0) { out.reward[e] = 0.0; out.done[e] = 1; }
+        return;
+    }
     const double a0 = act_aos ? act[2 * (size_t)e] : act[e];
-    const double a1 = act_aos ? act[2 * (size_t)e + 1] : act[E + e];
-    const double th = p.kinematics != CN_KIN_HOLONOMIC ? theta[e] : 0.0;
-    double ax, ay;
-    cn_effective_velocity(p.kinematics, th, a0, a1, ax, ay);
-    const double dt = p.time_step;
-    const double t = time[e];
-    auto ag = [&](int f, int a) { return st[st_idx(d, f, a, e)]; };
-    const StepOutcome oc = cn_step_outcome(p, ag, H, t, ax, ay);
-    const double reward = oc.reward, dmin = oc.dmin;
-    const int done = oc.done, info = oc.info;
-    const double endx = ag(F_PX, 0) + ax * dt, endy = ag(F_PY, 0) + ay * dt;
-    reward_o[e] = reward; done_o[e] = (uint8_t)done; info_o[e] = (uint8_t)info; dmin_o[e] = dmin;
-
-    if (update) {
-        st[st_idx(d, F_PX, 0, e)] = endx;
-        st[st_idx(d, F_PY, 0, e)] = endy;
-        if (p.kinematics == CN_KIN_HOLONOMIC) {
-            st[st_idx(d, F_VX, 0, e)] = ax;
-            st[st_idx(d, F_VY, 0, e)] = ay;
-        } else {
-            const double TWO_PI = 2 * 3.141592653589793;
-            double t2 = fmod(th + a1, TWO_PI);
-            if (t2 < 0) t2 += TWO_PI;
-            theta[e] = t2;
-            st[st_idx(d, F_VX, 0, e)] = a0 * cos(t2);
-            st[st_idx(d, F_VY, 0, e)] = a0 * sin(t2);
-        }
-        double hvx = human_v[(size_t)(0 * H) * E + e], hvy = human_v[(size_t)(1 * H) * E + e];
-        double opx = st[st_idx(d, F_PX, 1, e)], opy = st[st_idx(d, F_PY, 1, e)];
-        for (int h = 1; h <= H; ++h) {
-            double nvx = 0, nvy = 0, npx = 0, npy = 0;
-            if (h < H) {
-                nvx = human_v[(size_t)(0 * H + h) * E + e]; nvy = human_v[(size_t)(1 * H + h) * E + e];
-                npx = st[st_idx(d, F_PX, h + 1, e)]; npy = st[st_idx(d, F_PY, h + 1, e)];
-            }
-            st[st_idx(d, F_PX, h, e)] = opx + hvx * dt;
-            st[st_idx(d, F_PY, h, e)] = opy + hvy * dt;
-            st[st_idx(d, F_VX, h, e)] = hvx;
-            st[st_idx(d, F_VY, h, e)] = hvy;
-            hvx = nvx; hvy = nvy; opx = npx; opy = npy;
-        }
-        const double tn = t + dt;
-        time[e] = tn;
-        const int k = acc.ep_steps[e];
-        const double disc = pow(p.gamma, (double)k * dt * st[st_idx(d, F_VPREF, 0, e)]);
-        const double ret = acc.ep_return[e] + disc * reward;
-        acc.steps[e] += 1;
-        if (info == CN_DANGER) { acc.too_close[e] += 1; acc.sum_min_dist[e] += dmin; }
-        if (done) {
-            acc.episodes[e] += 1;
-            if (info == CN_REACHGOAL) { acc.success[e] += 1; acc.sum_success_time[e] += tn; }
-            else if (info == CN_COLLISION) { acc.collision[e] += 1; acc.sum_collision_time[e] += tn; }
-            else { acc.timeout[e] += 1; acc.sum_timeout_time[e] += p.time_limit; }
-            acc.sum_return[e] += ret;
-            acc.ep_return[e] = 0.0; acc.ep_steps[e] = 0;
-            if (!p.auto_reset) frozen[e] = 1;
-            else if (fuse_reset) reset_env(p, e, st, time, frozen, acc, theta);
-        } else {
-            acc.ep_return[e] = ret; acc.ep_steps[e] = k + 1;
-        }
-    } else {
-        for (int h = 1; h <= H; ++h) {
-            const double hvx = human_v[(size_t)(0 * H + h - 1) * E + e];
-            const double hvy = human_v[(size_t)(1 * H + h - 1) * E + e];
-            next_obs[(size_t)(0 * H + h - 1) * E + e] = st[st_idx(d, F_PX, h, e)] + hvx * dt;
-            next_obs[(size_t)(1 * H + h - 1) * E + e] = st[st_idx(d, F_PY, h, e)] + hvy * dt;
-            next_obs[(size_t)(2 * H + h - 1) * E + e] = hvx;
-            next_obs[(size_t)(3 * H + h - 1) * E + e] = hvy;
-            next_obs[(size_t)(4 * H + h - 1) * E + e] = st[st_idx(d, F_R, h, e)];
-        }
-    }
-}
-
-__device__ void reset_env_warp(const EnvParams &p, int e, int lane, double *__restrict__ st, double *__restrict__ time,
-                               uint8_t *__restrict__ frozen, const EnvAccum &acc, double *__restrict__ theta)
-{
-    const EnvDims d = p.d;
-    PhiloxStream rng;
-    rng.init(p.seed, (uint64_t)(p.env_id_offset + e), acc.episode_ctr[e], 0u);
-    __syncwarp();
-    if (lane == 0) acc.episode_ctr[e] += 1;
-    const double PI = 3.141592653589793;
-    if (lane == 0) {
-        st[st_idx(d, F_PX, 0, e)] = 0.0; st[st_idx(d, F_PY, 0, e)] = -p.circle_radius;
-        st[st_idx(d, F_VX, 0, e)] = 0.0; st[st_idx(d, F_VY, 0, e)] = 0.0;
-        st[st_idx(d, F_GX, 0, e)] = 0.0; st[st_idx(d, F_GY, 0, e)] = p.circle_radius;
-        st[st_idx(d, F_R, 0, e)] = p.robot_radius; st[st_idx(d, F_VPREF, 0, e)] = p.robot_v_pref;
-    }
-    __syncwarp();
-    constexpr int kSlots = (CN_MAX_HUMANS + 32) / 32;
-    double cpx[kSlots], cpy[kSlots], cgx[kSlots], cgy[kSlots], cr[kSlots];
-#pragma unroll
-    for (int k = 0; k < kSlots; ++k) { cpx[k] = cpy[k] = cgx[k] = cgy[k] = cr[k] = 0.0; }
-    if (lane == 0) { cpx[0] = 0.0; cpy[0] = -p.circle_radius; cgx[0] = 0.0; cgy[0] = p.circle_radius; cr[0] = p.robot_radius; }
-    const int MAX_TRIES = 4096;
-    for (int i = 1; i <= d.H; ++i) {
-        double px = 0, py = 0, gx = 0, gy = 0;
-        double h_radius = p.human_radius, h_v_pref = p.human_v_pref;
-        if (p.randomize_attributes) {
-            h_v_pref = 0.5 + (1.5 - 0.5) * rng.next();
-            h_radius = 0.3 + (0.5 - 0.3) * rng.next();
-        }
-        if (p.sim_rule == CN_CIRCLE_CROSSING) {
-            for (int tries = 0; tries < MAX_TRIES; ++tries) {
-                const double angle = rng.next() * PI * 2;
-                const double px_noise = (rng.next() - 0.5) * h_v_pref;
-                const double py_noise = (rng.next() - 0.5) * h_v_pref;
-                px = p.circle_radius * cos(angle) + px_noise;
-                py = p.circle_radius * sin(angle) + py_noise;
-                bool collide = false;
-#pragma unroll
-                for (int k = 0; k < kSlots; ++k) {
-                    if (lane + 32 * k >= i) continue;
-                    const double min_dist = h_radius + cr[k] + p.discomfort_dist;
-                    collide = collide || norm2d(px - cpx[k], py - cpy[k]) < min_dist || norm2d(px - cgx[k], py - cgy[k]) < min_dist;
-                }
-                if (!__any_sync(0xffffffffu, collide)) break;
-            }
-            gx = -px; gy = -py;
-        } else {
-            const double sign = (rng.next() > 0.5) ? -1.0 : 1.0;
-            for (int tries = 0; tries < MAX_TRIES; ++tries) {
-                px = rng.next() * p.square_width * 0.5 * sign;
-                py = (rng.next() - 0.5) * p.square_width;
-                bool collide = false;
-#pragma unroll
-                for (int k = 0; k < kSlots; ++k)
-                    if (lane + 32 * k < i)
-                        collide = collide || norm2d(px - cpx[k], py - cpy[k]) < h_radius + cr[k] + p.discomfort_dist;
-                if (!__any_sync(0xffffffffu, collide)) break;
-            }
-            for (int tries = 0; tries < MAX_TRIES; ++tries) {
-                gx = rng.next() * p.square_width * 0.5 * -sign;
-                gy = (rng.next() - 0.5) * p.square_width;
-                bool collide = false;
-#pragma unroll
-                for (int k = 0; k < kSlots; ++k)
-                    if (lane + 32 * k < i)
-                        collide = collide || norm2d(gx - cgx[k], gy - cgy[k]) < h_radius + cr[k] + p.discomfort_dist;
-                if (!__any_sync(0xffffffffu, collide)) break;
-            }
-        }
-        if (lane == 0) {
-            st[st_idx(d, F_PX, i, e)] = px; st[st_idx(d, F_PY, i, e)] = py;
-            st[st_idx(d, F_VX, i, e)] = 0.0; st[st_idx(d, F_VY, i, e)] = 0.0;
-            st[st_idx(d, F_GX, i, e)] = gx; st[st_idx(d, F_GY, i, e)] = gy;
-            st[st_idx(d, F_R, i, e)] = h_radius; st[st_idx(d, F_VPREF, i, e)] = h_v_pref;
-        }
-#pragma unroll
-        for (int k = 0; k < kSlots; ++k)
-            if (lane + 32 * k == i) { cpx[k] = px; cpy[k] = py; cgx[k] = gx; cgy[k] = gy; cr[k] = h_radius; }
-    }
-    if (lane == 0) {
-        time[e] = 0.0;
-        theta[e] = 1.5707963267948966;
-        frozen[e] = 0;
-        acc.ep_steps[e] = 0; acc.ep_return[e] = 0.0;
-    }
+    const double a1 = act_aos ? act[2 * (size_t)e + 1] : act[p.d.E + e];
+    cn_step_env_warp(p, e, lane, a0, a1, update, st, time, human_v, out, frozen, acc, theta);
 }
 
 __global__ void __launch_bounds__(128) reset_warp_kernel(EnvParams p, double *__restrict__ st, double *__restrict__ time,
@@ -643,19 +485,14 @@
     return CN_OK;
 }
 
-int cn_launch_step(cn_env *env, const double *action_xy_dev, int update, cudaStream_t s, int fuse_reset)
+int cn_launch_step(cn_env *env, const double *action_xy_dev, int update, cudaStream_t s)
 {
     const double *act = action_xy_dev ? action_xy_dev : env->action_xy;
-    const int bs = cn_small_block();
-    const bool split_reset = fuse_reset && update && env->p.d.H >= kWarpResetHumans;
-    if (split_reset) fuse_reset = 0;
-    step_kernel<<<grid_for(env->p.d.E, bs), bs, 0, s>>>(env->p, env->state, env->time, env->human_v, act,
-                                                            action_xy_dev ? 1 : 0, update, env->reward, env->done,
-                                                            env->info, env->dmin, env->next_obs, env->frozen,
-                                                            env->acc, env->theta, fuse_reset);
+    step_warp_kernel<<<grid_for(env->p.d.E * 32, 128), 128, 0, s>>>(env->p, env->state, env->time, env->human_v, act,
+                                                                     action_xy_dev ? 1 : 0, update, cn_step_out(env),
+                                                                     env->frozen, env->acc, env->theta);
     CN_LAUNCH_CHECK();
     if (update) env->orca_valid = 0;
-    if (split_reset) return cn_launch_reset(env, 1, s);
     return CN_OK;
 }
 
```

Result: no change. 12.11 million, median of 6 (-0.0%).
